# ehsan886/DBA_mod

Hardware: AMD Instinct MI355X
Metric: FL rounds/sec + backdoor ASR & main-task acc, ResNet-18 CIFAR-10 100 clients (higher is better)
Workload: dtype fp32

## Files before the change

csrc/kernels/xaux.hip:

```cpp
#include "common.hpp"
#include "xmfma.hpp"
#include <algorithm>

namespace {

__device__ __forceinline__ void xsplit_w_body(const float* __restrict__ w, long long sstride, long long per,
                                              const int* __restrict__ amax, int ld, uint16_t* __restrict__ out,
                                              int sl, long long e0, long long e1, long long step) {
  const int sb = hexp(amax_read(amax, ld, sl));
  const float mb = __uint_as_float((uint32_t)(sb + 127) << 23);
  const float* __restrict__ src = w + (long long)sl * sstride;
  uint16_t* __restrict__ oh = out + (long long)sl * 2 * per;
  uint16_t* __restrict__ ol = oh + per;
  for (long long e = e0 + threadIdx.x * 4LL; e < e1; e += step) {
    float v[4];
#pragma unroll
    for (int i = 0; i < 4; ++i) v[i] = e + i < per ? src[e + i] : 0.f;
    uint2 sp[2];
    split4h(v[0], v[1], v[2], v[3], mb, sp);
    const uint16_t* h = (const uint16_t*)&sp[0];
    const uint16_t* l = (const uint16_t*)&sp[1];
#pragma unroll
    for (int i = 0; i < 4; ++i)
      if (e + i < per) { oh[e + i] = h[i]; ol[e + i] = l[i]; }
  }
}
__global__ __launch_bounds__(256) void xsplit_w_kernel(const float* __restrict__ w, long long sstride, long long per,
                                                       const int* __restrict__ amax, int ld,
                                                       uint16_t* __restrict__ out) {
  xsplit_w_body(w, sstride, per, amax, ld, out, blockIdx.y, blockIdx.x * 1024LL, per, (long long)gridDim.x * 1024);
}
struct XSDesc {
  long long w, sstride, per, amax, ld, out, boff;
};
constexpr int kXSBatch = 24, kXSChunk = 4096;
struct XSBatch {
  XSDesc d[kXSBatch];
  int n;
};
__global__ __launch_bounds__(256) void xsplit_w_batch_kernel(const XSBatch b) {
  int i = 0;
  while (i + 1 < b.n && (long long)blockIdx.x >= b.d[i + 1].boff) ++i;
  const XSDesc& d = b.d[i];
  const long long e0 = ((long long)blockIdx.x - d.boff) * kXSChunk;
  const long long e1 = e0 + kXSChunk < d.per ? e0 + kXSChunk : d.per;
  xsplit_w_body((const float*)d.w, d.sstride, d.per, (const int*)d.amax, (int)d.ld, (uint16_t*)d.out, blockIdx.y, e0,
                e1, 1024);
}

struct XFDesc {
  long long planes, out, ncol, cs, boff;
};
struct XFBatch {
  XFDesc d[kXSBatch];
  int n;
};
__global__ __launch_bounds__(256) void xfrag_w_kernel(const XFBatch b) {
  int i = 0;
  while (i + 1 < b.n && (long long)blockIdx.x >= b.d[i + 1].boff) ++i;
  const XFDesc& d = b.d[i];
  const int Cs = (int)d.cs, K = 9 * Cs, NK = K / 32;
  const long long per = d.ncol * K;
  const long long idx = ((long long)blockIdx.x - d.boff) * 256 + threadIdx.x;
  if (idx >= per / 4) return;
  const int l = (int)(idx & 63), f = (int)(idx >> 6) & 3, p = f & 1, kk = f >> 1;
  const long long tt = idx >> 8;
  const int t = (int)(tt % NK), nt = (int)(tt / NK), cc = t / 9, tap = t - cc * 9;
  const long long e = (long long)(nt * 32 + (l & 31)) * K + tap * Cs + cc * 32 + (kk * 2 + (l >> 5)) * 8;
  const uint16_t* __restrict__ src = (const uint16_t*)d.planes + ((long long)blockIdx.y * 2 + p) * per;
  uint16_t* __restrict__ dst = (uint16_t*)d.out + (long long)blockIdx.y * 2 * per;
  ((uint4*)dst)[idx] = *(const uint4*)(src + e);
}

constexpr int kAmaxSegs = 64, kAmaxChunk = 4096;
struct AmaxSegs {
  long long off[kAmaxSegs];
  int len[kAmaxSegs];
  int start[kAmaxSegs + 1];
  int n;
};
__global__ __launch_bounds__(256) void amax_segments_kernel(const float* __restrict__ base, long long gstride,
                                                            const AmaxSegs segs, int ld, int* __restrict__ out) {
  const int c = blockIdx.x, g = blockIdx.y;
  int sg = 0;
  while (sg + 1 < segs.n && segs.start[sg + 1] <= c) ++sg;
  const float* __restrict__ p = base + (long long)g * gstride + segs.off[sg];
  const int n = segs.len[sg], e0 = (c - segs.start[sg]) * kAmaxChunk;
  const bool v4 = ((segs.off[sg] | gstride) & 3) == 0 && ((uintptr_t)base & 15) == 0;
  float m = 0.f;
  float4 v[4];
#pragma unroll
  for (int k = 0; k < 4; ++k) {
    const int e = e0 + (k * 256 + threadIdx.x) * 4;
    if (v4 && e + 3 < n) {
      v[k] = *(const float4*)(p + e);
    } else {
      v[k].x = e < n ? p[e] : 0.f;
      v[k].y = e + 1 < n ? p[e + 1] : 0.f;
      v[k].z = e + 2 < n ? p[e + 2] : 0.f;
      v[k].w = e + 3 < n ? p[e + 3] : 0.f;
    }
  }
#pragma unroll
  for (int k = 0; k < 4; ++k) m = fmaxf(m, fmaxf(fmaxf(fabsf(v[k].x), fabsf(v[k].y)), fmaxf(fabsf(v[k].z), fabsf(v[k].w))));
  amax_fold(out + (long long)sg * kAmaxSub * ld, ld, g, m);
}

__global__ __launch_bounds__(256) void amax_kernel(const float* __restrict__ x, long long gstride, long long n_per_g,
                                                   const int* __restrict__ nvalid, long long per_item, int vec,
                                                   int* __restrict__ out, int ld) {
  const int g = blockIdx.y;
  const long long n = nvalid ? (long long)nvalid[g] * per_item : n_per_g;
  const float* __restrict__ p = x + (long long)g * gstride;
  float m = 0.f;
  if (vec) {
    const long long n4 = n >> 2;
    for (long long e = blockIdx.x * 256LL + threadIdx.x; e < n4; e += (long long)gridDim.x * 256) {
      const float4 v = ((const float4*)p)[e];
      m = fmaxf(m, fmaxf(fmaxf(fabsf(v.x), fabsf(v.y)), fmaxf(fabsf(v.z), fabsf(v.w))));
    }
    for (long long e = n4 * 4 + blockIdx.x * 256LL + threadIdx.x; e < n; e += (long long)gridDim.x * 256)
      m = fmaxf(m, fabsf(p[e]));
  } else {
    for (long long e = blockIdx.x * 256LL + threadIdx.x; e < n; e += (long long)gridDim.x * 256) m = fmaxf(m, fabsf(p[e]));
  }
  amax_fold(out, ld, g, m);
}

}

DBA_EXPORT int dba_xsplit_w(const float* w, long long sstride, long long per, int slots, const int* amax, int ld,
                            uint16_t* out, void* stream) {
  const dim3 grid((unsigned)std::max(1LL, std::min(1024LL, (per + 1023) / 1024)), slots);
  hipLaunchKernelGGL(xsplit_w_kernel, grid, dim3(256), 0, (hipStream_t)stream, w, sstride, per, amax, ld, out);
  DBA_LAUNCH_CHECK();
}


DBA_EXPORT int dba_xsplit_w_batch(const void* desc, int n, int slots, void* stream) {
  const XSDesc* ds = (const XSDesc*)desc;
  for (int i0 = 0; i0 < n; i0 += kXSBatch) {
    XSBatch b{};
    b.n = std::min(kXSBatch, n - i0);
    long long nb = 0;
    for (int i = 0; i < b.n; ++i) {
      b.d[i] = ds[i0 + i];
      b.d[i].boff = nb;
      nb += (b.d[i].per + kXSChunk - 1) / kXSChunk;
    }
    hipLaunchKernelGGL(xsplit_w_batch_kernel, dim3((unsigned)nb, slots), dim3(256), 0, (hipStream_t)stream, b);
    const int rc = (int)hipGetLastError();
    if (rc != 0) return rc;
  }
  return 0;
}


DBA_EXPORT int dba_xfrag_w_batch(const void* desc, int n, int slots, void* stream) {
  const XFDesc* ds = (const XFDesc*)desc;
  for (int i0 = 0; i0 < n; i0 += kXSBatch) {
    XFBatch b{};
    b.n = std::min(kXSBatch, n - i0);
    long long nb = 0;
    for (int i = 0; i < b.n; ++i) {
      b.d[i] = ds[i0 + i];
      if (b.d[i].ncol <= 0 || b.d[i].cs <= 0 || b.d[i].ncol % 32 || b.d[i].cs % 32 || ((b.d[i].planes | b.d[i].out) & 15))
        return -105;
      b.d[i].boff = nb;
      nb += b.d[i].ncol * 9 * b.d[i].cs / 1024;
    }
    hipLaunchKernelGGL(xfrag_w_kernel, dim3((unsigned)nb, slots), dim3(256), 0, (hipStream_t)stream, b);
    const int rc = (int)hipGetLastError();
    if (rc != 0) return rc;
  }
  return 0;
}


DBA_EXPORT int dba_amax_segments(const float* base, long long gstride, const long long* segs, int n, int G, int* out,
                                 int ld, void* stream) {
  if (n > kAmaxSegs || n < 1) return -105;
  AmaxSegs a{};
  a.n = n;
  for (int i = 0; i < n; ++i) {
    a.off[i] = segs[2 * i];
    a.len[i] = (int)segs[2 * i + 1];
    a.start[i + 1] = a.start[i] + std::max(1, ceil_div(a.len[i], kAmaxChunk));
  }
  const dim3 grid((unsigned)a.start[n], G);
  hipLaunchKernelGGL(amax_segments_kernel, grid, dim3(256), 0, (hipStream_t)stream, base, gstride, a, ld, out);
  DBA_LAUNCH_CHECK();
}


DBA_EXPORT int dba_amax(const float* x, long long gstride, long long n_per_g, const int* nvalid, long long per_item,
                        int G, int* out, int ld, void* stream) {
  hipStream_t st = (hipStream_t)stream;
  const int vec = aligned16(x) && gstride % 4 == 0;
  const long long per = nvalid ? per_item * (n_per_g / std::max(1LL, per_item)) : n_per_g;
  const dim3 grid((unsigned)std::max(1LL, std::min(256LL, (per + 4095) / 4096)), G);
  hipLaunchKernelGGL(amax_kernel, grid, dim3(256), 0, st, x, gstride, n_per_g, nvalid, per_item, vec, out, ld);
  DBA_LAUNCH_CHECK();
}
```

csrc/kernels/xconv_fwd.hip:

```cpp
#include "xhalo.hpp"

namespace xg {
SplitPolicy& split_policy() {
  static SplitPolicy p;
  return p;
}
int& xstage_mode() {
  static int mode = 1;
  return mode;
}
}

namespace {

template <int W, int IMGS, int BN, int WM, int WN, bool PRE>
__global__ __launch_bounds__(256) void ximg_kernel(const XArgs a) {
  constexpr int P = 2, NT = 256;
  constexpr int PW = W + 2, PI = PW * PW, PP = IMGS * PI;
  constexpr int CC = 32, CH = CC / 8, Q4 = CC / 4;
  constexpr int PATCH = PP * CH;
  constexpr int BM = IMGS * W * W;
  constexpr int TM = BM / WM, TN = BN / WN, MI = TM / 32, NJ = TN / 32;
  static_assert(WM * WN == NT / 64 && MI >= 1 && NJ >= 1 && BM == 128, "tiling");
  constexpr int RPT = NT / 8;
  static_assert(BN % RPT == 0, "weight rows");
  constexpr int RB = BN / RPT, BPL = BN * 4;
  __shared__ __attribute__((aligned(16))) uint4 patch[P * PATCH];
  __shared__ __attribute__((aligned(16))) uint4 bring[2 * P * BPL];

  const int g = blockIdx.y;
  const int tn = blockIdx.x % a.tiles_n, tm = blockIdx.x / a.tiles_n;
  const int img0 = tm * IMGS, n0 = tn * BN;
  const int nv = min(valid_rows(a.nvalid, g, a.N), a.N);
  if (img0 >= nv) return;
  const int slot = a.wsel ? a.wsel[g] : g;
  const int Cs = a.Cs, K = 9 * Cs, NC = Cs / CC, NK = 9 * NC;
  const float* __restrict__ src = a.src + (long long)g * a.src_gstride;
  const int tid = threadIdx.x, lane = tid & 63, wid = tid >> 6;
  const int wm = wid / WN, wn = wid % WN;
  const int kq = tid & 7, r0 = tid >> 3;
  const int fr = lane & 31, hf = lane >> 5;

  constexpr int NE = (PP * Q4 + NT - 1) / NT;
  float4 pv[NE];
  const __amdgpu_buffer_rsrc_t rA = rsrc(src, (long long)a.N * W * W * Cs * 4);
  auto pload = [&](int cc) __attribute__((always_inline)) {
#pragma unroll
    for (int u = 0; u < NE; ++u) {
      const int e = tid + NT * u;
      const int pp = e / Q4, q = e - pp * Q4;
      const int im = pp / PI, rem = pp - im * PI;
      const int h = rem / PW - 1, w = rem % PW - 1, img = img0 + im;
      const bool ok = e < PP * Q4 && img < nv && (unsigned)h < (unsigned)W && (unsigned)w < (unsigned)W;
      pv[u] = bload4(rA, ok ? (((img * W + h) * W + w) * Cs + cc * CC + q * 4) * 4 : kOOB);
    }
  };
  HScale hs;
  auto ppiece = [&](int u, float m) __attribute__((always_inline)) {
    const int e = tid + NT * u;
    if (e >= PP * Q4) return;
    const int pp = e / Q4, q = e - pp * Q4;
    const int prow = (pp % PI) / PW;
    uint2 sp[P];
    split4h(pv[u].x, pv[u].y, pv[u].z, pv[u].w, m, sp);
    const int o = pp * CH + ((q >> 1) ^ (prow & 3));
#pragma unroll
    for (int p = 0; p < P; ++p) ((uint2*)&patch[p * PATCH + o])[q & 1] = sp[p];
  };

  int bn_[RB];
#pragma unroll
  for (int j = 0; j < RB; ++j) {
    const int n = n0 + r0 + RPT * j;
    bn_[j] = n < a.Ncol ? n : -1;
  }
  const uint16_t* Bh = PRE ? a.wp + (long long)slot * a.wp_sstride : nullptr;
  const __amdgpu_buffer_rsrc_t rBh = rsrc(Bh, (long long)a.Ncol * K * 2);
  const __amdgpu_buffer_rsrc_t rBl = rsrc(PRE ? Bh + (a.wp_sstride >> 1) : nullptr, (long long)a.Ncol * K * 2);
  const __amdgpu_buffer_rsrc_t rB = rsrc(a.w + (long long)slot * a.w_sstride, (long long)a.Ncol * K * 4);
  uint4 rb[2][RB];
  auto gq = [&](int t, int st, int j) __attribute__((always_inline)) {
    const bool ok = bn_[j] >= 0 && t < NK;
    const int cc = t / 9, tap = t - cc * 9;
    const int kb = bn_[j] * K + tap * Cs + cc * CC + kq * 4;
    if constexpr (PRE) {
      const uint2 h = bload8(rBh, ok ? kb * 2 : kOOB), l = bload8(rBl, ok ? kb * 2 : kOOB);
      rb[st][j] = make_uint4(h.x, h.y, l.x, l.y);
    } else {
      rb[st][j] = __builtin_bit_cast(uint4, bload4(rB, ok ? kb * 4 : kOOB));
    }
  };
  auto lput_q = [&](int buf, int st, int q) __attribute__((always_inline)) {
    uint2 sp[P];
    if constexpr (PRE) {
      sp[0] = make_uint2(rb[st][q].x, rb[st][q].y);
      sp[1] = make_uint2(rb[st][q].z, rb[st][q].w);
    } else {
      const float4 v = __builtin_bit_cast(float4, rb[st][q]);
      split4h(v.x, v.y, v.z, v.w, hs.mb, sp);
    }
    lds_put<P, false, BN>(bring + buf * P * BPL, BPL, 0, r0 + RPT * q, kq, sp);
  };

  f32x16_t acc[MI][NJ];
#pragma unroll
  for (int i = 0; i < MI; ++i)
#pragma unroll
    for (int j = 0; j < NJ; ++j)
#pragma unroll
      for (int r = 0; r < 16; ++r) acc[i][j][r] = 0.f;

  int apix[MI], arow[MI];
#pragma unroll
  for (int i = 0; i < MI; ++i) {
    const int m = wm * TM + i * 32 + fr;
    const int im = m / (W * W), rem = m - im * (W * W);
    apix[i] = im * PI + (rem / W) * PW + rem % W;
    arow[i] = rem / W;
  }
  auto mma = [&](int t, int buf, int stn) __attribute__((always_inline)) {
    const int tap = t % 9, ti = tap / 3, tj = tap - ti * 3;
    const int toff = ti * PW + tj;
    const uint4* L = bring + buf * P * BPL;
    sfor<2>([&](auto KK) __attribute__((always_inline)) {
      const int ch = decltype(KK)::value * 2 + hf;
      uint4 af[P][MI], bfr[P][NJ];
#pragma unroll
      for (int i = 0; i < MI; ++i) {
        const int pp = apix[i] + toff;
        const int o = pp * CH + (ch ^ ((arow[i] + ti) & 3));
#pragma unroll
        for (int p = 0; p < P; ++p) af[p][i] = patch[p * PATCH + o];
      }
#pragma unroll
      for (int j = 0; j < NJ; ++j) {
        const int n = wn * TN + j * 32 + fr;
        const int o = n * 4 + (ch ^ ((n >> 2) & 3));
#pragma unroll
        for (int p = 0; p < P; ++p) bfr[p][j] = L[p * BPL + o];
      }
      mma_half<MI, NJ, P, true, RB, decltype(KK)::value>(af, bfr, acc, [&](int q) __attribute__((always_inline)) {
        lput_q(buf ^ 1, stn, q);
        gq(t + 3, stn, q);
      });
    });
  };
  auto step = [&](int t, int buf, int stn) __attribute__((always_inline)) {
    const int c = t / 9;
    mma(t, buf, stn);
    __syncthreads();
    if (t - 9 * c == 8 && c + 1 < NC) {
#pragma unroll
      for (int u = 0; u < NE; ++u) ppiece(u, hs.ma);
      if (c + 2 < NC) pload(c + 2);
      __syncthreads();
    }
  };

  hs.init(amax_read(a.amax_src, a.amax_src_ld, g), amax_read(a.amax_w, a.amax_w_ld, slot));
#pragma unroll
  for (int q = 0; q < RB; ++q) {
    gq(0, 0, q);
    gq(1, 1, q);
  }
  pload(0);
#pragma unroll
  for (int u = 0; u < NE; ++u) ppiece(u, hs.ma);
  if (NC > 1) pload(1);
#pragma unroll
  for (int q = 0; q < RB; ++q) {
    lput_q(0, 0, q);
    gq(2, 0, q);
  }
  __syncthreads();
  int t = 0;
  for (; t + 1 < NK; t += 2) {
    step(t, 0, 1);
    step(t + 1, 1, 0);
  }
  if (t < NK) step(t, 0, 1);
  hs.finish(acc);

  float* out = a.out + (long long)g * a.out_gstride;
  const float* bias = a.bias ? a.bias + (long long)slot * a.b_sstride : nullptr;
  const float* res = a.res ? a.res + (long long)g * a.out_gstride : nullptr;
  float vmax = 0.f;
#pragma unroll
  for (int j = 0; j < NJ; ++j) {
    const int n = n0 + wn * TN + j * 32 + fr;
    if (n >= a.Ncol) continue;
    const float bv = bias ? bias[n] : 0.f;
#pragma unroll
    for (int i = 0; i < MI; ++i)
#pragma unroll
      for (int r = 0; r < 16; ++r) {
        const int m = wm * TM + i * 32 + (r & 3) + 8 * (r >> 2) + 4 * hf;
        if (img0 + m / (W * W) >= nv) continue;
        const long long o = (long long)(img0 * W * W + m) * a.Ncol + n;
        float v = acc[i][j][r];
        if (bias) v += bv;
        if (res) v += res[o];
        if (a.relu) v = fmaxf(v, 0.f);
        vmax = fmaxf(vmax, fabsf(v));
        out[o] = v;
      }
  }
  if (a.amax_out) amax_fold(a.amax_out, a.amax_out_ld, g, vmax);
}

template <int W, int IMGS, int BN>
__global__ __launch_bounds__(256) void ximg2_kernel(const XArgs a) {
  constexpr int P = 2, NT = 256;
  constexpr int PW = W + 2, PI = PW * PW, PP = IMGS * PI;
  constexpr int CC = 32, CH = CC / 8, Q4 = CC / 4;
  constexpr int PATCH = PP * CH;
  constexpr int BM = IMGS * W * W;
  constexpr int WN = BN / 32, WM = (NT / 64) / WN, TM = BM / WM, MI = TM / 32;
  static_assert(WM * WN == NT / 64 && MI >= 1 && BM == 128, "tiling");
  extern __shared__ __attribute__((aligned(16))) uint4 ximg2_patch[];

  const int g = blockIdx.y;
  const int tn = blockIdx.x % a.tiles_n, tm = blockIdx.x / a.tiles_n;
  const int img0 = tm * IMGS, n0 = tn * BN;
  const int nv = min(valid_rows(a.nvalid, g, a.N), a.N);
  if (img0 >= nv) return;
  const int slot = a.wsel ? a.wsel[g] : g;
  const int Cs = a.Cs, NC = Cs / CC, NK = 9 * NC;
  const float* __restrict__ src = a.src + (long long)g * a.src_gstride;
  const int tid = threadIdx.x, lane = tid & 63, wid = tid >> 6;
  const int wm = wid / WN, wn = wid % WN;
  const int fr = lane & 31, hf = lane >> 5;

  constexpr int NE = (PP * Q4 + NT - 1) / NT;
  static_assert(NE <= 9, "one patch piece per k-step");
  float4 pv[NE];
  const __amdgpu_buffer_rsrc_t rA = rsrc(src, (long long)a.N * W * W * Cs * 4);
  auto pload1 = [&](int u, int cc) __attribute__((always_inline)) {
    const int e = tid + NT * u;
    const int pp = e / Q4, q = e - pp * Q4;
    const int im = pp / PI, rem = pp - im * PI;
    const int h = rem / PW - 1, w = rem % PW - 1, img = img0 + im;
    const bool ok = e < PP * Q4 && cc < NC && img < nv && (unsigned)h < (unsigned)W && (unsigned)w < (unsigned)W;
    pv[u] = bload4(rA, ok ? (((img * W + h) * W + w) * Cs + cc * CC + q * 4) * 4 : kOOB);
  };
  HScale hs;
  auto ppiece = [&](int u, int buf) __attribute__((always_inline)) {
    const int e = tid + NT * u;
    if (NT * (u + 1) > PP * Q4 && e >= PP * Q4) return;
    const int pp = e / Q4, q = e - pp * Q4;
    const int prow = (pp % PI) / PW;
    uint2 sp[P];
    split4h(pv[u].x, pv[u].y, pv[u].z, pv[u].w, hs.ma, sp);
    const int o = pp * CH + ((q >> 1) ^ (prow & 3));
#pragma unroll
    for (int p = 0; p < P; ++p) ((uint2*)&ximg2_patch[(buf * P + p) * PATCH + o])[q & 1] = sp[p];
  };

  const __amdgpu_buffer_rsrc_t rF = rsrc(a.wf + (long long)slot * a.wf_sstride, (long long)a.Ncol * 9 * Cs * 4);
  const int wbase = ((n0 >> 5) + wn) * NK * 4096 + lane * 16;
  uint4 wb[3][4];
  auto gw = [&](int t, int s, int f) __attribute__((always_inline)) {
    wb[s][f] = __builtin_bit_cast(uint4, bload4(rF, t < NK ? wbase + t * 4096 + f * 1024 : kOOB));
  };

  f32x16_t acc[MI][1];
#pragma unroll
  for (int i = 0; i < MI; ++i)
#pragma unroll
    for (int r = 0; r < 16; ++r) acc[i][0][r] = 0.f;

  int apix[MI], arow[MI];
#pragma unroll
  for (int i = 0; i < MI; ++i) {
    const int m = wm * TM + i * 32 + fr;
    const int im = m / (W * W), rem = m - im * (W * W);
    apix[i] = im * PI + (rem / W) * PW + rem % W;
    arow[i] = rem / W;
  }

  hs.init(amax_read(a.amax_src, a.amax_src_ld, g), amax_read(a.amax_w, a.amax_w_ld, slot));
#pragma unroll
  for (int f = 0; f < 4; ++f) {
    gw(0, 0, f);
    gw(1, 1, f);
  }
#pragma unroll
  for (int u = 0; u < NE; ++u) pload1(u, 0);
#pragma unroll
  for (int u = 0; u < NE; ++u) {
    ppiece(u, 0);
    pload1(u, 1);
  }
  __syncthreads();
  for (int c = 0; c < NC; ++c) {
    const uint4* L = ximg2_patch + (c & 1) * P * PATCH;
    const bool more = c + 1 < NC;
    sfor<9>([&](auto TAP) __attribute__((always_inline)) {
      constexpr int tap = decltype(TAP)::value, ti = tap / 3, tj = tap - ti * 3;
      constexpr int toff = ti * PW + tj, s = tap % 3, s2 = (tap + 2) % 3;
      constexpr int u = tap - (9 - NE);
      constexpr int NQ = u >= 0 ? 5 : 4;
      const int t = c * 9 + tap;
      __builtin_amdgcn_sched_barrier(0x786);
      sfor<2>([&](auto KK) __attribute__((always_inline)) {
        constexpr int kk = decltype(KK)::value;
        const int ch = kk * 2 + hf;
        uint4 af[P][MI], bfr[P][1];
#pragma unroll
        for (int i = 0; i < MI; ++i) {
          const int o = (apix[i] + toff) * CH + (ch ^ ((arow[i] + ti) & 3));
#pragma unroll
          for (int p = 0; p < P; ++p) af[p][i] = L[p * PATCH + o];
        }
#pragma unroll
        for (int p = 0; p < P; ++p) bfr[p][0] = wb[s][kk * 2 + p];
        mma_half<MI, 1, P, true, NQ, kk>(af, bfr, acc, [&](int q) __attribute__((always_inline)) {
          if (q < 4) {
            gw(t + 2, s2, q);
          } else if constexpr (u >= 0) {
            if (more) ppiece(u, (c + 1) & 1);
            pload1(u, c + 2);
          }
        });
      });
    });
    __syncthreads();
  }
  hs.finish(acc);

  float* out = a.out + (long long)g * a.out_gstride;
  const float* bias = a.bias ? a.bias + (long long)slot * a.b_sstride : nullptr;
  const float* res = a.res ? a.res + (long long)g * a.out_gstride : nullptr;
  float vmax = 0.f;
  const int n = n0 + wn * 32 + fr;
  if (n < a.Ncol) {
    const float bv = bias ? bias[n] : 0.f;
#pragma unroll
    for (int i = 0; i < MI; ++i)
#pragma unroll
      for (int r = 0; r < 16; ++r) {
        const int m = wm * TM + i * 32 + (r & 3) + 8 * (r >> 2) + 4 * hf;
        if (img0 + m / (W * W) >= nv) continue;
        const long long o = (long long)(img0 * W * W + m) * a.Ncol + n;
        float v = acc[i][0][r];
        if (bias) v += bv;
        if (res) v += res[o];
        if (a.relu) v = fmaxf(v, 0.f);
        vmax = fmaxf(vmax, fabsf(v));
        out[o] = v;
      }
  }
  if (a.amax_out) amax_fold(a.amax_out, a.amax_out_ld, g, vmax);
}

template <int W, int IMGS, int BN, int WM, int WN>
int ximg_go(const XArgs& a, int G, hipStream_t st) {
  XArgs b = a;
  b.tiles_n = ceil_div(a.Ncol, BN);
  const dim3 grid((unsigned)(ceil_div(a.N, IMGS) * b.tiles_n), G, 1);
  if (a.wp) hipLaunchKernelGGL((ximg_kernel<W, IMGS, BN, WM, WN, true>), grid, dim3(256), 0, st, b);
  else hipLaunchKernelGGL((ximg_kernel<W, IMGS, BN, WM, WN, false>), grid, dim3(256), 0, st, b);
  DBA_LAUNCH_CHECK();
}
template <int W, int IMGS, int BN>
int ximg2_go(const XArgs& a, int G, hipStream_t st) {
  constexpr int PATCH = IMGS * (W + 2) * (W + 2) * 4;
  constexpr int LDS = 2 * 2 * PATCH * (int)sizeof(uint4);
  static unsigned long long attr_set = 0ull;
  int dev = 0;
  if (hipGetDevice(&dev) != hipSuccess || dev < 0 || dev >= 64) return -100;
  if (!(attr_set >> dev & 1ull)) {
    if (hipFuncSetAttribute((const void*)ximg2_kernel<W, IMGS, BN>, hipFuncAttributeMaxDynamicSharedMemorySize,
                            LDS) != hipSuccess)
      return -100;
    attr_set |= 1ull << dev;
  }
  XArgs b = a;
  b.tiles_n = ceil_div(a.Ncol, BN);
  const dim3 grid((unsigned)(ceil_div(a.N, IMGS) * b.tiles_n), G, 1);
  hipLaunchKernelGGL((ximg2_kernel<W, IMGS, BN>), grid, dim3(256), LDS, st, b);
  DBA_LAUNCH_CHECK();
}
__global__ __launch_bounds__(256) void xstage16_kernel(const XArgs a) {
  constexpr int P = 2, W = 16, CS = 64, BM = 128, BN = 64, WN = 2;
  constexpr int TR = BM / W, PW = W + 2, PR = TR + 2, PP = PR * PW;
  constexpr int CH = CS / 8, PATCH = PP * CH;
  constexpr int TM = 64, TN = 32, MI = TM / 32;
  constexpr int CB = CS / 32;
  constexpr int STG = (BN / 32) * CB * 4 * 64;
  static_assert(BM * BN <= P * PATCH * 4, "epilogue tile fits the patch");
  __shared__ __attribute__((aligned(16))) uint4 lds[P * PATCH + 2 * STG];
  __shared__ long long orow[BM];
  uint4* const patch = lds;
  uint4* const bring = lds + P * PATCH;

  const int g = blockIdx.y;
  const int HT = a.Ho / TR;
  const int tm = blockIdx.x;
  const int img = tm / HT, h0 = (tm - img * HT) * TR;
  if (img >= valid_rows(a.nvalid, g, a.N)) return;
  const int slot = a.wsel ? a.wsel[g] : g;
  const float* __restrict__ src = a.src + (long long)g * a.src_gstride;
  const int tid = threadIdx.x, lane = tid & 63, wid = tid >> 6;
  const int wm = wid / WN, wn = wid % WN;
  const int fr = lane & 31, hf = lane >> 5;

  const uint16_t* F = a.wf + (long long)slot * a.wf_sstride + ((wid >> 1) * (CB * 9) + (wid & 1) * 9) * 2048 + lane * 8;
  auto fill = [&](int tap) __attribute__((always_inline)) {
    const uint32_t dst = __builtin_amdgcn_readfirstlane(
        (uint32_t)(uintptr_t)(__attribute__((address_space(3))) void*)(bring + (tap & 1) * STG + wid * 256));
#pragma unroll
    for (int f = 0; f < 4; ++f) {
      uint32_t keep;
      asm volatile("s_mov_b32 %0, m0\n\ts_mov_b32 m0, %2\n\ts_nop 0\n\tglobal_load_lds_dwordx4 %1, off\n\ts_mov_b32 m0, %0"
                   : "=&s"(keep)
                   : "v"(F + tap * 2048 + f * 512), "s"(dst + f * 1024)
                   : "memory");
    }
  };
  auto gl_sync = [&]() __attribute__((always_inline)) {
    asm volatile("s_waitcnt vmcnt(0)" ::: "memory");
    __syncthreads();
  };
  fill(0);

  if (tid < BM)
    orow[tid] = (((long long)img * a.Ho + h0 + tid / W) * a.Wo + tid % W) * a.Ncol;

  constexpr int Q4 = CS / 4;
  constexpr int NE = (PP * Q4 + 255) / 256;
  float4 pv[NE];
  {
    const __amdgpu_buffer_rsrc_t rA = rsrc(src, (long long)a.N * a.Hs * a.Ws * CS * 4);
#pragma unroll
    for (int u = 0; u < NE; ++u) {
      const int e = tid + 256 * u;
      const int pp = e / Q4, q = e - pp * Q4;
      const int pr = pp / PW, pc = pp - pr * PW;
      const int h = h0 - 1 + pr, w = pc - 1;
      const bool ok = e < PP * Q4 && (unsigned)h < (unsigned)a.Hs && (unsigned)w < (unsigned)a.Ws;
      pv[u] = bload4(rA, ok ? (((img * a.Hs + h) * a.Ws + w) * CS + q * 4) * 4 : kOOB);
    }
  }
  HScale hs;
  hs.init(amax_read(a.amax_src, a.amax_src_ld, g), amax_read(a.amax_w, a.amax_w_ld, slot));
#pragma unroll
  for (int u = 0; u < NE; ++u) {
    const int e = tid + 256 * u;
    if (e >= PP * Q4) break;
    const int pp = e / Q4, q = e - pp * Q4;
    uint2 sp[P];
    split4h(pv[u].x, pv[u].y, pv[u].z, pv[u].w, hs.ma, sp);
    const int o = pp * CH + ((q >> 1) ^ hswz<W, CS>(pp, pp % PW));
#pragma unroll
    for (int p = 0; p < P; ++p) ((uint2*)&patch[p * PATCH + o])[q & 1] = sp[p];
  }

  f32x16_t acc[MI][1];
#pragma unroll
  for (int i = 0; i < MI; ++i)
#pragma unroll
    for (int r = 0; r < 16; ++r) acc[i][0][r] = 0.f;
  int apix[MI], acol[MI];
#pragma unroll
  for (int i = 0; i < MI; ++i) {
    const int m = wm * TM + i * 32 + fr;
    apix[i] = (m / W) * PW + (m % W);
    acol[i] = m % W;
  }

  auto stage = [&](int tap) __attribute__((always_inline)) {
    const int ti = tap / 3, tj = tap - ti * 3;
    const int toff = ti * PW + tj;
    const uint4* L = bring + (tap & 1) * STG + wn * (CB * 4 * 64) + lane;
    uint4 af[2][P][MI], bfr[2][P][1];
    auto frags = [&](auto Hc) __attribute__((always_inline)) {
      constexpr int h = decltype(Hc)::value, cb = h / 2, kk = h % 2, st = h & 1;
      const int ch = kk * 2 + hf;
#pragma unroll
      for (int i = 0; i < MI; ++i) {
        const int pp = apix[i] + toff;
        const int o = pp * CH + ((cb * 4 + ch) ^ hswz<W, CS>(pp, acol[i] + tj));
#pragma unroll
        for (int p = 0; p < P; ++p) af[st][p][i] = patch[p * PATCH + o];
      }
#pragma unroll
      for (int p = 0; p < P; ++p) bfr[st][p][0] = L[(cb * 4 + kk * 2 + p) * 64];
    };
    frags(std::integral_constant<int, 0>{});
    sfor<2 * CB>([&](auto Hc) __attribute__((always_inline)) {
      constexpr int h = decltype(Hc)::value;
      if constexpr (h + 1 < 2 * CB) frags(std::integral_constant<int, h + 1>{});
      __builtin_amdgcn_sched_barrier(0);
      mma_half<MI, 1, P, true, 0, h % 2>(af[h & 1], bfr[h & 1], acc, [](int) {});
      __builtin_amdgcn_sched_barrier(0);
    });
  };

  gl_sync();
  for (int tap = 0; tap < 9; ++tap) {
    if (tap + 1 < 9) fill(tap + 1);
    stage(tap);
    gl_sync();
  }
  hs.finish(acc);

  float* Ct = reinterpret_cast<float*>(patch);
#pragma unroll
  for (int i = 0; i < MI; ++i)
#pragma unroll
    for (int r = 0; r < 16; ++r)
      Ct[(wm * TM + i * 32 + (r & 3) + 8 * (r >> 2) + 4 * hf) * BN + wn * TN + fr] = acc[i][0][r];
  __syncthreads();
  float* out = a.out + (long long)g * a.out_gstride;
  const float* bias = a.bias ? a.bias + (long long)slot * a.b_sstride : nullptr;
  const float* res = a.res ? a.res + (long long)g * a.out_gstride : nullptr;
  constexpr int C4 = BN / 4;
  float vmax = 0.f;
  for (int e = tid; e < BM * C4; e += 256) {
    const int row = e / C4, n = (e - row * C4) * 4;
    const long long o = orow[row];
    float4 v = *(const float4*)&Ct[row * BN + n];
    if (bias) { v.x += bias[n]; v.y += bias[n + 1]; v.z += bias[n + 2]; v.w += bias[n + 3]; }
    if (res) {
      const float4 rv = *(const float4*)(res + o + n);
      v.x += rv.x; v.y += rv.y; v.z += rv.z; v.w += rv.w;
    }
    if (a.relu) { v.x = fmaxf(v.x, 0.f); v.y = fmaxf(v.y, 0.f); v.z = fmaxf(v.z, 0.f); v.w = fmaxf(v.w, 0.f); }
    vmax = fmaxf(vmax, fmaxf(fmaxf(fabsf(v.x), fabsf(v.y)), fmaxf(fabsf(v.z), fabsf(v.w))));
    *(float4*)(out + o + n) = v;
  }
  if (a.amax_out) amax_fold(a.amax_out, a.amax_out_ld, g, vmax);
}

constexpr bool kXStage16Default = true;

int xstage16_try(const XArgs& a, int G, int KH, int KW, hipStream_t st) {
  const XClass& c = a.cls[0];
  const int mode = xg::xstage_mode();
  if (!(mode == 3 || (mode == 1 && kXStage16Default))) return -100;
  if (KH != 3 || KW != 3 || a.sp != 1 || a.os != 1 || a.dsg != 1 || a.splitk != 1 || c.nI != 3 || c.nJ != 3 ||
      c.bh != -1 || c.bw != -1)
    return -100;
  if (a.Hs != 16 || a.Ws != 16 || a.Ho != 16 || a.Wo != 16 || a.Cs != 64 || a.Ncol != 64) return -100;
  if (a.bf.mode || a.lz_coef || a.sc_src) return -100;
  if (!aligned16(a.src) || !aligned16(a.w) || a.src_gstride % 4 || a.w_sstride % 4) return -100;
  if (!a.wp || !a.wf || ((uintptr_t)a.wf & 15) || a.wf_sstride % 8 || a.wf_sstride < 2 * 64 * 576) return -100;
  hipLaunchKernelGGL(xstage16_kernel, dim3((unsigned)(a.N * (a.Ho / 8)), G, 1), dim3(256), 0, st, a);
  DBA_LAUNCH_CHECK();
}

int& ximg_on() {
  static int on = 1;
  return on;
}
int ximg_try(const XArgs& a, int G, int KH, int KW, hipStream_t st) {
  const XClass& c = a.cls[0];
  if (!ximg_on() || KH != 3 || KW != 3 || a.sp != 1 || a.os != 1 || a.dsg != 1 || a.splitk != 1 || c.nI != 3 ||
      c.nJ != 3 || c.bh != -1 || c.bw != -1)
    return -100;
  if (a.Hs != a.Ho || a.Ws != a.Wo || a.Ho != a.Wo || a.Cs % 32 != 0 || a.Ncol % 32 != 0) return -100;
  if (a.bf.mode || a.lz_coef) return -100;
  if (!aligned16(a.src) || a.src_gstride % 4 || !aligned16(a.w) || a.w_sstride % 4) return -100;
  if (a.wp && (((uintptr_t)a.wp & 15) || a.wp_sstride % 8)) return -100;
  if (a.sc_src) return -100;
  if (ximg_on() == 1 && a.wp && a.wf && !((uintptr_t)a.wf & 15) && a.wf_sstride % 8 == 0) {
    int rc = -100;
    if (a.Wo == 8) rc = a.Ncol >= 128 ? ximg2_go<8, 2, 128>(a, G, st) : ximg2_go<8, 2, 64>(a, G, st);
    if (a.Wo == 4) rc = a.Ncol >= 128 ? ximg2_go<4, 8, 128>(a, G, st) : ximg2_go<4, 8, 64>(a, G, st);
    if (rc != -100) return rc;
  }
  if (a.Wo == 8) return a.Ncol >= 128 ? ximg_go<8, 2, 128, 2, 2>(a, G, st) : ximg_go<8, 2, 64, 2, 2>(a, G, st);
  if (a.Wo == 4) return a.Ncol >= 128 ? ximg_go<4, 8, 128, 2, 2>(a, G, st) : ximg_go<4, 8, 64, 2, 2>(a, G, st);
  return -100;
}

}

DBA_EXPORT int dba_xsplit_policy(int target, int min_k, int max_s, int kslab_max, int dgrad_ks) {
  SplitPolicy& p = split_policy();
  if (dgrad_ks >= 0) p.dgrad_ks = dgrad_ks;
  if (target > 0) p.target = target;
  if (min_k > 0) p.min_k = min_k;
  if (max_s > 0) p.max_s = std::min(max_s, kSkMax);
  if (kslab_max > 0) p.kslab_max = kslab_max;
  return 0;
}

DBA_EXPORT int dba_ximg_set(int on) {
  const int prev = ximg_on();
  if (on >= 0) ximg_on() = on;
  return prev;
}

DBA_EXPORT int dba_xstage_set(int on) {
  const int prev = xg::xstage_mode();
  if (on >= 1 && on <= 3) xg::xstage_mode() = on;
  return prev;
}


DBA_EXPORT long long dba_xconv_ws_floats(int G, int N, int Ho, int Wo, int Cin, int Cout, int KH, int KW) {
  const long long M = (long long)N * Ho * Wo;
  const int s = xsplitk(M, G, Cout, KH * KW * Cin);
  return s > 1 ? (long long)s * G * M * Cout : 0;
}


DBA_EXPORT long long dba_xconv_sk_ints(int G, int N, int Ho, int Wo, int Cin, int Cout, int KH, int KW) {
  const long long M = (long long)N * Ho * Wo;
  const int s = xsplitk(M, G, Cout, KH * KW * Cin);
  const long long n = s > 1 ? xconv_sk_count(M, Cout, G, 1, s) : 0;
  return (n > 0 && sk_ok((const int*)1, n, M, Cout, G, 1, s)) ? n : 0;
}


DBA_EXPORT int dba_xconv_fwd(const float* x, long long x_gstride, const float* w, long long w_sstride,
                             const int* wsel, const float* bias, long long b_sstride, const float* res, float* out,
                             long long out_gstride, const int* nvalid, int G, int N, int H, int W, int Cin, int Ho,
                             int Wo, int Cout, int KH, int KW, int stride, int pad, int relu, const int* amax_x,
                             int amax_x_ld, const int* amax_w, int amax_w_ld, int* amax_out, int amax_out_ld,
                             const uint16_t* wp, long long wp_sstride, const uint16_t* wf, long long wf_sstride,
                             float* ws, long long ws_floats, int* sk_cnt,
                             long long sk_cnt_n, const void* bnf, const float* lz_coef, int lz_relu,
                             void* stream) {
  hipStream_t st = (hipStream_t)stream;
  if ((long long)N * H * W * Cin >= (1LL << 29)) return -103;
  const long long M = (long long)N * Ho * Wo;
  const int K = KH * KW * Cin;
  const int vec = (Cin % 4 == 0 && aligned16(x) && aligned16(w) && x_gstride % 4 == 0 && w_sstride % 4 == 0) ? 4 : 1;
  XArgs a{};
  a.src = x; a.src_gstride = x_gstride; a.w = w; a.w_sstride = w_sstride; a.wsel = wsel;
  a.bias = bias; a.b_sstride = b_sstride; a.res = res; a.out = out; a.out_gstride = out_gstride;
  a.nvalid = nvalid; a.N = N; a.Hs = H; a.Ws = W; a.Cs = Cin; a.Ncol = Cout; a.Ho = Ho; a.Wo = Wo;
  a.sp = stride; a.os = 1; a.dsg = 1; a.relu = relu; a.splitk = 1;
  a.amax_src = amax_x; a.amax_w = amax_w; a.amax_out = amax_out;
  a.amax_src_ld = amax_x_ld; a.amax_w_ld = amax_w_ld; a.amax_out_ld = amax_out_ld;
  a.wp = wp; a.wp_sstride = wp_sstride; a.wf = wf; a.wf_sstride = wf_sstride;
  a.cls[0] = XClass{KH, KW, -pad, -pad, 0, 0, Ho, Wo, 0};
  if (!amax_x || !amax_w) return -109;
  if (bnf) {
    a.bf = *(const BnFuse*)bnf;
    if (a.bf.mode != 1 || bias || res || relu || (Cout & 3) || a.bf.C != Cout) return -108;
  }
  if (lz_coef) {
    if (wp || vec < 4 || Cin > 512) return -108;
    a.lz_coef = lz_coef; a.lz_relu = lz_relu;
  }
  auto fin = [&](int rc) { return (rc == 0 && a.bf.mode) ? bnx_finalize_go(a.bf, nvalid, G, N, Ho * Wo, st) : rc; };
  if (stride == 1) {
    int rc = ximg_try(a, G, KH, KW, st);
    if (rc == -100) rc = xstage16_try(a, G, KH, KW, st);
    if (rc == -100) rc = xhalo_try(a, G, KH, KW, st);
    if (rc != -100) return fin(rc);
  }
  const int s = xsplitk(M, G, Cout, K);
  const bool ws_ok = s > 1 && ws != nullptr && ws_floats >= (long long)s * G * M * Cout;
  if (s > 1 && !(ws_ok && sk_ok(sk_cnt, sk_cnt_n, M, Cout, G, 1, s))) {
    XArgs b = a;
    b.kslab = s;
    const int rc = xconv_ks(b, M, G, vec, st);
    if (rc != -100) return fin(rc);
  }
  if (ws_ok && sk_ok(sk_cnt, sk_cnt_n, M, Cout, G, 1, s)) {
    XArgs b = a;
    b.splitk = s;
    b.zstride = (long long)G * M * Cout;
    b.sk_ws = ws; b.sk_gstride = M * Cout; b.sk_cnt = sk_cnt;
    return fin(xconv_dispatch(b, M, G, 1, vec, st));
  }
  if (ws_ok) {
    XArgs b = a;
    b.splitk = s;
    b.out = ws;
    b.out_gstride = M * Cout;
    b.zstride = (long long)G * M * Cout;
    const int rc = xconv_dispatch(b, M, G, 1, vec, st);
    if (rc != 0) return rc;
    if (a.bf.mode)
      return bnx_tile_go(a.bf, nullptr, out, out_gstride, nvalid, G, N, Ho * Wo, nullptr, 0.f, ws, s, b.zstride,
                         nullptr, st);
    const long long per = M * Cout;
    const dim3 grid((unsigned)std::max(1LL, std::min(1024LL, (per + 255) / 256)), G);
    hipLaunchKernelGGL(xsplitk_reduce_kernel, grid, dim3(256), 0, st, (const float*)ws, s, b.zstride, per, nvalid, N,
                       Ho * Wo, Cout, bias, b_sstride, wsel, res, relu, out, amax_out, amax_out_ld);
    DBA_LAUNCH_CHECK();
  }
  return fin(xconv_dispatch(a, M, G, 1, vec, st));
}


DBA_EXPORT int dba_xdown_fwd(const float* a_, long long a_gstride, const float* w2, long long w2_sstride,
                             const uint16_t* w2p, long long w2p_sstride, const int* wsel, const float* b2,
                             long long b_sstride, const float* x2, long long x2_gstride, const uint16_t* wscp,
                             long long wscp_sstride, const float* bsc, long long bsc_sstride, float* out,
                             long long out_gstride, const int* nvalid, int G, int N, int Ho, int Wo, int C, int H2,
                             int W2, int C2, const int* amax_a, int amax_a_ld, const int* amax_w2, int amax_w2_ld,
                             const int* amax_x2, int amax_x2_ld, const int* amax_wsc, int amax_wsc_ld, int* amax_out,
                             int amax_out_ld, void* stream) {
  if (!amax_a || !amax_w2 || !amax_x2 || !amax_wsc || !w2p || !wscp) return -109;
  if ((H2 - 1) / 2 + 1 != Ho || (W2 - 1) / 2 + 1 != Wo || (long long)N * H2 * W2 * C2 >= (1LL << 29) ||
      (long long)N * Ho * Wo * C >= (1LL << 29))
    return -103;
  XArgs a{};
  a.src = a_; a.src_gstride = a_gstride; a.w = w2; a.w_sstride = w2_sstride; a.wsel = wsel;
  a.bias = b2; a.b_sstride = b_sstride; a.res = nullptr; a.out = out; a.out_gstride = out_gstride;
  a.nvalid = nvalid; a.N = N; a.Hs = Ho; a.Ws = Wo; a.Cs = C; a.Ncol = C; a.Ho = Ho; a.Wo = Wo;
  a.sp = 1; a.os = 1; a.dsg = 1; a.relu = 1; a.splitk = 1;
  a.amax_src = amax_a; a.amax_w = amax_w2; a.amax_out = amax_out;
  a.amax_src_ld = amax_a_ld; a.amax_w_ld = amax_w2_ld; a.amax_out_ld = amax_out_ld;
  a.wp = w2p; a.wp_sstride = w2p_sstride;
  a.sc_src = x2; a.sc_gstride = x2_gstride; a.sc_H = H2; a.sc_W = W2; a.sc_C = C2;
  a.sc_wp = wscp; a.sc_wp_sstride = wscp_sstride;
  a.sc_amax_src = amax_x2; a.sc_amax_src_ld = amax_x2_ld; a.sc_amax_w = amax_wsc; a.sc_amax_w_ld = amax_wsc_ld;
  a.sc_bias = bsc; a.sc_b_sstride = bsc_sstride;
  a.cls[0] = XClass{3, 3, -1, -1, 0, 0, Ho, Wo, 0};
  return xhalo_try(a, G, 3, 3, (hipStream_t)stream);
}
```

dba_mod_amd/models/program.py:

```python
from __future__ import annotations

from typing import Callable, Dict, List, Optional, Tuple

import torch

from .. import ops
from ..ops import bnstate as bs
from .mirror import CIFAR_RESNETS
from .spec import ModelSpec

Tensor = torch.Tensor
BN_EPS = 1e-5
BN_MOMENTUM = 0.1


class Tape:

    def __init__(self) -> None:
        self.nodes: List[Tuple[Tuple[Tensor, ...], Tuple[Optional[Tensor], ...], Callable]] = []
        self._produced: set = set()
        self._grads: Optional[Dict[int, Tensor]] = None
        self._uses: Dict[int, int] = {}
        self.nvalid: Optional[Tensor] = None
        self.on_begin: Optional[Callable[[], None]] = None
        self.on_end: Optional[Callable[[], None]] = None

    def record(self, outputs: Tuple[Tensor, ...], inputs: Tuple[Optional[Tensor], ...], bwd: Callable) -> None:
        self.nodes.append((outputs, inputs, bwd))
        for o in outputs:
            self._produced.add(id(o))
        for i in inputs:
            if i is not None:
                self._uses[id(i)] = self._uses.get(id(i), 0) + 1

    def is_last(self, t) -> bool:
        return self._uses.get(id(t), 0) == 1

    @staticmethod
    def finish_spec(t) -> Optional[bs.Finish]:
        if isinstance(t, bs.LazyBN):
            return bs.Finish(ya=t.y, sa=t.stat, lazy=t.relu)
        return getattr(t, "_dba_finish", None)

    def needs_grad(self, t: Optional[Tensor]) -> bool:
        return t is not None and id(t) in self._produced

    def pop_grad(self, t: Tensor) -> Optional[Tensor]:
        return self._grads.pop(id(t), None) if self._grads is not None else None

    def backward(self, out: Tensor, grad: Tensor) -> None:
        if self.on_begin is not None:
            self.on_begin()
        grads: Dict[int, Tensor] = {id(out): grad}
        self._grads = grads
        for outputs, inputs, bwd in reversed(self.nodes):
            gouts = [grads.pop(id(o), None) for o in outputs]
            if all(g is None for g in gouts):
                for i in inputs:
                    if i is not None:
                        self._uses[id(i)] -= 1
                continue
            gouts = [ops.bn_finish(g, self.finish_spec(o), self.nvalid)
                     if isinstance(g, Tensor) and self.finish_spec(o) is not None else g
                     for o, g in zip(outputs, gouts)]
            gins = bwd(*gouts)
            for inp, gi in zip(inputs, gins):
                if inp is not None:
                    self._uses[id(inp)] -= 1
                if gi is None or inp is None or not self.needs_grad(inp):
                    continue
                k = id(inp)
                if k in grads:
                    if not (isinstance(grads[k], Tensor) and isinstance(gi, Tensor)):
                        raise RuntimeError("a finished BN gradient cannot take further contributions")
                    grads[k] = grads[k] + gi
                else:
                    grads[k] = gi
        self.nodes.clear()
        self._produced.clear()
        self._uses.clear()
        self._grads = None
        if self.on_end is not None:
            self.on_end()


class Ctx:

    def __init__(self, spec: ModelSpec, state: Tensor, wcomp: Tensor, wsel: Optional[Tensor],
                 train: bool, grads: Optional[Tensor] = None, nvalid: Optional[Tensor] = None,
                 folded: Optional[Dict[str, Tuple[Tensor, Tensor]]] = None,
                 dropout_seed: Optional[Tensor] = None,
                 act_dtype: torch.dtype = torch.float32) -> None:
        self.spec, self.state, self.wcomp, self.wsel = spec, state, wcomp, wsel
        self.train, self.grads, self.nvalid, self.folded = train, grads, nvalid, folded
        self.tape = Tape() if train else None
        self._dgrad_items: List[tuple] = []
        self._wt: Dict[int, Tensor] = {}
        self._wdefer: List[tuple] = []
        if self.tape is not None:
            self.tape.on_begin = self._prepare_dgrad
            self.tape.on_end = self._end_backward
            self.tape.nvalid = nvalid
        self.dropout_seed = dropout_seed
        self._drop_ctr = 0
        self.head: Optional[dict] = None
        self.head_out: Optional[Tuple[Tensor, Tensor]] = None
        self.act_dtype = act_dtype
        self._wamax = self._weight_scales() if train else None

    def _weight_scales(self) -> Optional[Dict[str, Tensor]]:
        wc = self.wcomp
        if wc is None or not wc.is_cuda or wc.dtype != torch.float32 or ops.backend_name(wc.device) != "hip":
            return None
        names = [e.name for e in self.spec.params if e.kind in ("conv_w", "lin_w")]
        slots = ops.hip_module().weight_amax(wc, [(self.spec.by_name[n].offset, self.spec.by_name[n].numel)
                                                  for n in names])
        return dict(zip(names, slots))

    def _want_dgrad(self, w: Tensor, stride: int, pad: int, in_hw: Tuple[int, int], G: int) -> int:
        self._dgrad_items.append((w, self.wsel, stride, pad, in_hw, self.nvalid, G))
        return len(self._dgrad_items) - 1

    def _end_backward(self) -> None:
        if self._wdefer:
            ops.backend_for(self.state).wgrad_flush(self._wdefer)

    def _prepare_dgrad(self) -> None:
        if self._dgrad_items:
            self._wt = ops.prepare_dgrad_weights(self._dgrad_items[0][0], self._dgrad_items)
        self._dgrad_items = []

    def w(self, name: str) -> Tensor:
        v = self.spec.view(self.wcomp, name)
        if self._wamax is not None and name in self._wamax:
            v._dba_amax = self._wamax[name]
        return v

    def m(self, name: str) -> Tensor:
        return self.spec.view(self.state, name)

    def g(self, name: str) -> Tensor:
        assert self.grads is not None
        return self.spec.view(self.grads, name)

    def conv_bn(self, x: Tensor, conv: str, bn: str, stride: int, pad: int, relu: bool,
                residual: Optional[Tensor] = None) -> Tensor:
        if self.train:
            raise RuntimeError("conv_bn is the evaluation form; training uses bn_conv / bn_out")
        wf, bf = self.folded[conv]
        return ops.conv2d(x, wf, self.wsel, stride, pad, bias=bf, residual=residual, relu=relu, nvalid=self.nvalid)

    def basic_block(self, x: Tensor, pre: str) -> Tensor:
        w1, b1 = self.folded[pre + "conv1.weight"]
        w2, b2 = self.folded[pre + "conv2.weight"]
        if ops.basic_block_ok(x, w1, w2):
            return ops.basic_block_eval(x, w1, b1, w2, b2, self.wsel, self.nvalid)
        a = ops.conv2d(x, w1, self.wsel, 1, 1, bias=b1, relu=True, nvalid=self.nvalid)
        return ops.conv2d(a, w2, self.wsel, 1, 1, bias=b2, residual=x, relu=True, nvalid=self.nvalid)

    def down_block(self, a: Tensor, x: Tensor, pre: str, sc: str) -> Tensor:
        w2, b2 = self.folded[pre + "conv2.weight"]
        wsc, bsc = self.folded[sc + ".0.weight"]
        if ops.down_block_ok(a, w2, x, wsc):
            return ops.down_block_eval(a, w2, b2, x, wsc, bsc, self.wsel, self.nvalid)
        r = ops.conv2d(x, wsc, self.wsel, 2, 0, bias=bsc, nvalid=self.nvalid)
        return ops.conv2d(a, w2, self.wsel, 1, 1, bias=b2, residual=r, relu=True, nvalid=self.nvalid)

    def stem_block(self, x: Tensor, stem: str, pre: str) -> Optional[Tensor]:
        w0, b0 = self.folded[stem]
        w1, b1 = self.folded[pre + "conv1.weight"]
        w2, b2 = self.folded[pre + "conv2.weight"]
        if not ops.stem_block_ok(x, w0, w1, w2):
            return None
        return ops.stem_block_eval(x, w0, b0, w1, b1, w2, b2, self.wsel, self.nvalid)

    def _bnp(self, bn: str) -> bs.BnParams:
        return bs.BnParams(self.m(bn + ".weight"), self.m(bn + ".bias"), self.m(bn + ".running_mean"),
                           self.m(bn + ".running_var"), self.g(bn + ".weight"), self.g(bn + ".bias"),
                           BN_MOMENTUM, BN_EPS)

    def bn_conv(self, x, conv: str, bn: str, stride: int, pad: int, relu: bool):
        if not self.train:
            return self.conv_bn(x, conv, bn, stride, pad, relu)
        w = self.w(conv)
        y, st = ops.conv_bn_stats(x, w, self.wsel, stride, pad, self.nvalid, self._bnp(bn), relu)
        a = bs.LazyBN(y, st, relu)
        self.tape.record((a,), (x,), self._bn_conv_bwd(x, w, y, st, conv, stride, pad))
        return a

    def _bn_conv_bwd(self, x, w, y, st, conv: str, stride: int, pad: int):
        in_hw = (x.shape[2], x.shape[3])
        kh, kw = w.shape[2], w.shape[3]
        need_dx = self.tape.needs_grad(x)
        k = self._want_dgrad(w, stride, pad, in_hw, x.shape[0]) if need_dx else -1

        def bwd(ga: bs.Fin):
            dy = ops.conv2d_wgrad(bs.LazyGrad(ga.for_stat(st).d, y, st), x, stride, pad, kh, kw, self.g(conv),
                                  nvalid=self.nvalid, defer=self._wdefer)
            if not need_dx:
                return (None,)
            if dy is None:
                raise RuntimeError(f"{conv}: the weight gradient did not store dy for the data gradient")
            acc = self.tape.pop_grad(x)
            fin = self.tape.finish_spec(x) if self.tape.is_last(x) else None
            return (ops.conv2d_dgrad(dy, w, self.wsel, stride, pad, in_hw, nvalid=self.nvalid, accum=acc,
                                     wt=self._wt.get(k), finish=fin),)
        return bwd

    def bn_out(self, a, residual=None, relu: bool = True) -> Tensor:
        out = ops.bn_apply(a, residual, relu, self.nvalid)
        branch = isinstance(residual, bs.LazyBN) and not residual.relu
        out._dba_finish = bs.Finish(ya=a.y, sa=a.stat, mask_out=out if relu else None,
                                    yb=residual.y if branch else None, sb=residual.stat if branch else None)

        def bwd(gout: bs.Fin):
            gr = None
            if branch:
                gr = gout.for_stat(residual.stat)
            elif residual is not None:
                gr = gout.d
            return gout.for_stat(a.stat), gr

        self.tape.record((out,), (a, residual), bwd)
        return out

    def conv(self, x: Tensor, name: str, stride: int, pad: int, bias: Optional[str], relu: bool) -> Tensor:
        if not self.train and self.folded is not None and name in self.folded:
            w, b = self.folded[name]
        else:
            w, b = self.w(name), (self.m(bias) if bias is not None else None)
        y = ops.conv2d(x, w, self.wsel, stride, pad, bias=b, relu=relu, nvalid=self.nvalid)
        if not self.train:
            return y
        in_hw = (x.shape[2], x.shape[3])
        kh, kw = w.shape[2], w.shape[3]
        need_dx = self.tape.needs_grad(x)
        k = self._want_dgrad(w, stride, pad, in_hw, x.shape[0]) if need_dx else -1

        def bwd(dout: Tensor):
            d = ops.relu_mask_bwd(dout, y) if relu else dout
            ops.conv2d_wgrad(d, x, stride, pad, kh, kw, self.g(name), self.g(bias) if bias is not None else None,
                             nvalid=self.nvalid, defer=self._wdefer)
            return (ops.conv2d_dgrad(d, w, self.wsel, stride, pad, in_hw, nvalid=self.nvalid, wt=self._wt.get(k))
                    if need_dx else None,)

        self.tape.record((y,), (x,), bwd)
        return y

    def linear(self, x: Tensor, name: str, bias: str, relu: bool, final: bool = False) -> Tensor:
        G, N, Fd = x.shape
        x4 = self.reshape(x, (G, N, 1, 1, Fd))
        y4 = self._lin_conv(x4, name, bias, relu, torch.float32 if final else None)
        return self.reshape(y4, (G, N, y4.shape[-1]))

    def _lin_conv(self, x4: Tensor, name: str, bias: str, relu: bool,
                  out_dtype: Optional[torch.dtype] = None) -> Tensor:
        if not self.train and self.folded is not None and name in self.folded:
            w, b = self.folded[name]
        else:
            wv = self.w(name)
            w = wv.reshape(wv.shape[0], wv.shape[1], 1, 1, wv.shape[2])
            if hasattr(wv, "_dba_amax"):
                w._dba_amax = wv._dba_amax
            b = self.m(bias)
        y = ops.conv2d(x4, w, self.wsel, 1, 0, bias=b, relu=relu, nvalid=self.nvalid, out_dtype=out_dtype)
        if not self.train:
            return y
        need_dx = self.tape.needs_grad(x4)
        gv = self.g(name)
        k = self._want_dgrad(w, 1, 0, (1, 1), x4.shape[0]) if need_dx else -1

        def bwd(dout: Tensor):
            d = ops.relu_mask_bwd(dout, y) if relu else dout
            ops.conv2d_wgrad(d, x4, 1, 0, 1, 1, gv.reshape(gv.shape[0], gv.shape[1], 1, 1, gv.shape[2]),
                             self.g(bias), nvalid=self.nvalid, defer=self._wdefer)
            return (ops.conv2d_dgrad(d, w, self.wsel, 1, 0, (1, 1), nvalid=self.nvalid, wt=self._wt.get(k))
                    if need_dx else None,)

        self.tape.record((y,), (x4,), bwd)
        return y

    def reshape(self, x: Tensor, shape: Tuple[int, ...]) -> Tensor:
        y = x.reshape(shape)
        if self.train and y is not x:
            in_shape = x.shape
            self.tape.record((y,), (x,), lambda d: (d.reshape(in_shape),))
        return y

    def maxpool(self, x: Tensor, k: int, s: int, p: int) -> Tensor:
        if not self.train:
            return ops.maxpool2d(x, k, s, p, want_ind=False)[0]
        y, ind = ops.maxpool2d(x, k, s, p)
        if self.train:
            shp = tuple(x.shape)
            self.tape.record((y,), (x,), lambda d: (ops.maxpool2d_bwd(d, ind, shp, k, s, p),))
        return y

    def gap(self, x: Tensor) -> Tensor:
        y = ops.avgpool_global(x)
        if self.train:
            hw = (x.shape[2], x.shape[3])

            def bwd(d):
                fin = self.tape.finish_spec(x) if self.tape.is_last(x) else None
                if fin is not None:
                    return (ops.bn_finish(None, fin, self.nvalid, pool=d, hw=hw),)
                return (ops.avgpool_global_bwd(d, hw),)

            self.tape.record((y,), (x,), bwd)
        return y

    def head_ok(self, x, wname: str) -> bool:
        if not (self.train and self.head is not None and isinstance(x, Tensor) and x.is_cuda):
            return False
        be = ops.backend_for(x)
        return hasattr(be, "head_ok") and be.head_ok(x, self.w(wname))

    def fused_head(self, x: Tensor, wname: str, bname: str) -> Tensor:
        be = ops.backend_for(x)
        h = self.head
        hw = (x.shape[2], x.shape[3])
        loss, correct, dpool = be.head_train(x, self.w(wname), self.m(bname), h["labels"], self.nvalid,
                                             self.g(wname), self.g(bname), h.get("stats"), h.get("slot"))
        self.head_out = (loss, correct)

        def bwd(_seed):
            fin = self.tape.finish_spec(x) if self.tape.is_last(x) else None
            if fin is not None:
                return (ops.bn_finish(None, fin, self.nvalid, pool=dpool, hw=hw),)
            return (ops.avgpool_global_bwd(dpool, hw),)

        self.tape.record((loss,), (x,), bwd)
        return loss

    def dropout(self, x: Tensor, p: float) -> Tensor:
        if not self.train:
            return x
        seeds, salt = self.dropout_seed, self._drop_ctr
        self._drop_ctr += 1
        y = ops.dropout(x, p, seeds, salt)
        self.tape.record((y,), (x,), lambda d: (ops.dropout_bwd(d, p, seeds, salt),))
        return y


def _block_out(ctx: Ctx, a, conv: str, bn: str, pad: int, residual):
    if not ctx.train:
        return ctx.conv_bn(a, conv, bn, 1, pad, relu=True, residual=residual)
    return ctx.bn_out(ctx.bn_conv(a, conv, bn, 1, pad, relu=False), residual, relu=True)


def _resnet_cifar(ctx: Ctx, x: Tensor) -> Tensor:
    bottleneck, blocks = CIFAR_RESNETS[ctx.spec.arch]
    exp = 4 if bottleneck else 1
    out = None if (ctx.train or bottleneck) else ctx.stem_block(x, "conv1.weight", "layer1.0.")
    done = 0 if out is None else 1
    if out is None:
        out = ctx.bn_conv(x, "conv1.weight", "bn1", 1, 1, relu=True)
    cin = 32
    for li, w in enumerate((32, 64, 128, 256)):
        for bi in range(done if li == 0 else 0, blocks[li]):
            stride = 2 if (li > 0 and bi == 0) else 1
            pre = f"layer{li + 1}.{bi}."
            if not ctx.train and not bottleneck and stride == 1 and cin == w:
                out = ctx.basic_block(out, pre)
                cin = w
                continue
            if bottleneck:
                a = ctx.bn_conv(out, pre + "conv1.weight", pre + "bn1", 1, 0, relu=True)
                a = ctx.bn_conv(a, pre + "conv2.weight", pre + "bn2", stride, 1, relu=True)
                last, p = "3", 0
            else:
                a = ctx.bn_conv(out, pre + "conv1.weight", pre + "bn1", stride, 1, relu=True)
                last, p = "2", 1
                if not ctx.train and stride == 2 and cin != w:
                    out, cin = ctx.down_block(a, out, pre, pre + "shortcut"), w
                    continue
            if stride != 1 or cin != w * exp:
                sc = ctx.bn_conv(out, pre + "shortcut.0.weight", pre + "shortcut.1", stride, 0, relu=False)
            else:
                sc = out
            out = _block_out(ctx, a, pre + f"conv{last}.weight", pre + f"bn{last}", p, sc)
            cin = w * exp
    if ctx.head_ok(out, "linear.weight"):
        return ctx.fused_head(out, "linear.weight", "linear.bias")
    out = ctx.gap(out)
    G, N = out.shape[:2]
    return ctx.linear(ctx.reshape(out, (G, N, out.shape[-1])), "linear.weight", "linear.bias", relu=False, final=True)


def _resnet_tiny(ctx: Ctx, x: Tensor) -> Tensor:
    if ctx.train:
        out = ctx.bn_out(ctx.bn_conv(x, "conv1.weight", "bn1", 2, 3, relu=False), None, relu=True)
    else:
        out = ctx.conv_bn(x, "conv1.weight", "bn1", 2, 3, relu=True)
    out = ctx.maxpool(out, 3, 2, 1)
    cin = 64
    for li, w in enumerate((64, 128, 256, 512)):
        for bi in range(2):
            stride = 2 if (li > 0 and bi == 0) else 1
            pre = f"layer{li + 1}.{bi}."
            if not ctx.train and stride == 2 and cin != w:
                a = ctx.bn_conv(out, pre + "conv1.weight", pre + "bn1", stride, 1, relu=True)
                out, cin = ctx.down_block(a, out, pre, pre + "downsample"), w
                continue
            if stride != 1 or cin != w:
                sc = ctx.bn_conv(out, pre + "downsample.0.weight", pre + "downsample.1", stride, 0, relu=False)
            else:
                sc = out
            a = ctx.bn_conv(out, pre + "conv1.weight", pre + "bn1", stride, 1, relu=True)
            out = _block_out(ctx, a, pre + "conv2.weight", pre + "bn2", 1, sc)
            cin = w
    out = ctx.gap(out)
    G, N = out.shape[:2]
    return ctx.linear(ctx.reshape(out, (G, N, out.shape[-1])), "fc.weight", "fc.bias", relu=False, final=True)


def _mnist(ctx: Ctx, x: Tensor) -> Tensor:
    a = ctx.conv(x, "conv1.weight", 1, 0, "conv1.bias", relu=True)
    a = ctx.maxpool(a, 2, 2, 0)
    b = ctx.conv(a, "conv2.weight", 1, 0, "conv2.bias", relu=True)
    b = ctx.maxpool(b, 2, 2, 0)
    G, N = b.shape[:2]
    f = ctx.reshape(b, (G, N, -1))
    h = ctx.linear(f, "fc1.weight", "fc1.bias", relu=True)
    return ctx.linear(h, "fc2.weight", "fc2.bias", relu=False, final=True)


def _loan(ctx: Ctx, x: Tensor) -> Tensor:
    h = ctx.linear(x, "layer1.0.weight", "layer1.0.bias", relu=True)
    h = ctx.dropout(h, 0.5)
    h = ctx.linear(h, "layer2.0.weight", "layer2.0.bias", relu=True)
    h = ctx.dropout(h, 0.5)
    return ctx.linear(h, "layer3.0.weight", "layer3.0.bias", relu=False, final=True)


FORWARDS: Dict[str, Callable[[Ctx, Tensor], Tensor]] = {
    "resnet18_tiny": _resnet_tiny, "mnist": _mnist, "loan": _loan,
    **{arch: _resnet_cifar for arch in CIFAR_RESNETS},
}


def forward(ctx: Ctx, x: Tensor) -> Tensor:
    return FORWARDS[ctx.spec.arch](ctx, x)


def _conv_bn_pairs(spec: ModelSpec) -> List[Tuple[str, str]]:
    pairs = []
    for e in spec.params:
        if e.kind != "conv_w":
            continue
        n = e.name
        if n.endswith("shortcut.0.weight"):
            pairs.append((n, n.replace("shortcut.0.weight", "shortcut.1")))
        elif n.endswith("downsample.0.weight"):
            pairs.append((n, n.replace("downsample.0.weight", "downsample.1")))
        else:
            bn = n.replace("conv", "bn").replace(".weight", "")
            if bn + ".weight" in spec.by_name:
                pairs.append((n, bn))
    return pairs


def fold_bank(spec: ModelSpec, state: Tensor, dtype: torch.dtype) -> Dict[str, Tuple[Tensor, Tensor]]:
    out: Dict[str, Tuple[Tensor, Tensor]] = {}
    pairs = list(_conv_bn_pairs(spec))
    slots = (ops.hip_module().amax_slots(len(pairs), state.shape[0], state.device)
             if state.is_cuda and ops.backend_name(state.device) == "hip" and dtype == torch.float32 else None)
    H = ops.hip_module() if slots is not None else None
    if H is not None and (ops.bn_fold is H.bn_fold or getattr(ops.bn_fold, "__module__", "") == ops.__name__):
        folded = H.bn_fold_batch([(spec.view(state, conv), spec.view(state, bn + ".weight"),
                                   spec.view(state, bn + ".bias"), spec.view(state, bn + ".running_mean"),
                                   spec.view(state, bn + ".running_var"), slots[i])
                                  for i, (conv, bn) in enumerate(pairs)], BN_EPS)
        for (conv, _), wb in zip(pairs, folded):
            out[conv] = wb
        H.split_weights_batch([(wf, wf[0].numel(), wf[0].numel(), wf._dba_amax) for wf, _ in folded])
    else:
        for conv, bn in pairs:
            out[conv] = ops.bn_fold(spec.view(state, conv), None, spec.view(state, bn + ".weight"),
                                    spec.view(state, bn + ".bias"), spec.view(state, bn + ".running_mean"),
                                    spec.view(state, bn + ".running_var"), BN_EPS, dtype)
    for e in spec.params:
        if e.name in out or e.kind not in ("conv_w", "lin_w"):
            continue
        bias = e.name.replace(".weight", ".bias")
        w = spec.view(state, e.name)
        if w.dim() == 3:
            w = w.reshape(w.shape[0], w.shape[1], 1, 1, w.shape[2])
        b = spec.view(state, bias) if bias in spec.by_name else None
        out[e.name] = (w.to(dtype), b)
    return out
```

dba_mod_amd/ops/__init__.py:

```python
from __future__ import annotations

import contextlib
import os
from typing import Any

import torch

from . import reference as _ref

_FORCE_REF = os.environ.get("DBA_OPS", "").lower() == "reference"
_hip_mod = None


def hip_module():
    global _hip_mod
    if _hip_mod is None:
        from . import hip as _h
        _hip_mod = _h
    return _hip_mod


def backend_for(t: torch.Tensor):
    if t.is_cuda and not _FORCE_REF:
        return hip_module()
    return _ref


def backend_name(device: torch.device) -> str:
    return "hip" if (device.type == "cuda" and not _FORCE_REF) else "reference"


def _dispatch(name: str):
    def fn(*args: Any, **kw: Any):
        first = next(a for a in list(args) + list(kw.values()) if isinstance(a, torch.Tensor))
        return getattr(backend_for(first), name)(*args, **kw)
    fn.__name__ = name
    fn.__doc__ = getattr(_ref, name).__doc__
    return fn


_OPS = ["gather_images", "gather_rows", "conv2d", "conv2d_dgrad", "conv2d_wgrad", "relu_mask_bwd", "bn_fold", "maxpool2d", "maxpool2d_bwd", "avgpool_global",
        "avgpool_global_bwd", "dropout", "dropout_bwd", "softmax_xent", "sgd_step", "dist_loss_grad",
        "scale_from_base", "add_noise_scaled", "delta_sum", "sq_dists", "weighted_sum", "weighted_sum_fixed", "delta_stats", "clipped_delta_sum_fixed",
        "clipped_delta_sum", "pairwise_sq_dists", "trimmed_delta_sum", "delta_sum_votes",
        "vote_agreement", "rlr_apply", "gram", "prepare_dgrad_weights", "wgrad_flush",
        "wgrad_prepare", "conv_bn_stats", "bn_apply", "bn_finish", "basic_block_ok", "basic_block_eval",
        "stem_block_ok", "stem_block_eval", "down_block_ok", "down_block_eval"]

for _n in _OPS:
    globals()[_n] = _dispatch(_n)


def amax_arena(G: int, device: torch.device, counters: int = 0):
    if backend_name(device) == "hip":
        return hip_module().amax_arena(G, device, counters=counters)
    return contextlib.nullcontext()


__all__ = list(_OPS) + ["backend_for", "backend_name", "hip_module", "amax_arena"]

from . import library
```

dba_mod_amd/ops/branches.py:

```python
from __future__ import annotations

import torch

TIE_TOL = 1e-4


class BranchReplay:

    def __init__(self, nval, tol: float = TIE_TOL):
        self.nval, self.rec, self.replay, self.i = nval, [], False, 0
        self.tol = tol
        self.flips = self.hard = self.elements = 0

    def start_replay(self) -> None:
        self.replay, self.i = True, 0
        self.flips = self.hard = self.elements = 0

    def wrap(self, mod):
        o_conv, o_mp = mod.conv2d, mod.maxpool2d
        o_cbs, o_apply = mod.conv_bn_stats, mod.bn_apply

        def conv_bn_stats(x, w, wsel, stride, pad, nvalid, p, relu):
            y, st = o_cbs(x, w, wsel, stride, pad, nvalid, p, relu)
            if relu:
                C = y.shape[-1]
                sh = (y.shape[0],) + (1,) * (y.dim() - 2) + (C,)
                pre = (y.double() * st.coef[:, 2].reshape(sh).double() + st.coef[:, 3].reshape(sh).double())
                if not self.replay:
                    self.rec.append((pre > 0).cpu())
                else:
                    st.relu_mask = self._decide(pre.to(y.dtype) if y.dtype == torch.float64 else pre)
            return y, st

        def bn_apply(a, residual, relu, nvalid=None):
            if not (relu and self.replay):
                out = o_apply(a, residual, relu, nvalid)
                return self._record(out) if relu else out
            return self._relu(o_apply(a, residual, False, nvalid))

        def conv2d(*a, **k):
            relu = k.get("relu", a[7] if len(a) > 7 else False)
            if not (relu and self.replay):
                y = o_conv(*a, **k)
                return self._record(y) if relu else y
            if len(a) > 7:
                a = a[:7] + (False,) + a[8:]
            else:
                k = dict(k, relu=False)
            return self._relu(o_conv(*a, **k))

        def maxpool2d(x, kk, st, p, want_ind=True):
            y, ind = o_mp(x, kk, st, p)
            y, ind = self._pool(x, y, ind)
            return y, (ind if want_ind else None)

        def basic_block_ok(x, w1, w2):
            return False
        return {"conv2d": conv2d, "maxpool2d": maxpool2d, "conv_bn_stats": conv_bn_stats, "bn_apply": bn_apply,
                "basic_block_ok": basic_block_ok, "stem_block_ok": lambda x, w0, w1, w2: False,
                "down_block_ok": lambda a, w2, x2, wsc: False}

    def _valid(self, t):
        v = torch.zeros(t.shape[:2], dtype=torch.bool)
        for g in range(t.shape[0]):
            v[g, :int(self.nval[g])] = True
        return v.view(*t.shape[:2], *([1] * (t.dim() - 2))).to(t.device)

    def _rms(self, t):
        keep = self._valid(t).expand_as(t)
        sq = torch.where(keep, t.double() ** 2, torch.zeros((), dtype=torch.float64, device=t.device))
        n = keep.reshape(t.shape[0], -1).sum(1).clamp(min=1)
        r = (sq.reshape(t.shape[0], -1).sum(1) / n).sqrt()
        return r.view(-1, *([1] * (t.dim() - 1))).to(t.dtype)

    def _record(self, out):
        self.rec.append((out > 0).cpu())
        return out

    def _decide(self, pre):
        m = self.rec[self.i].to(pre.device)
        self.i += 1
        keep = self._valid(pre).expand_as(pre)
        pos = pre > 0
        tie = pre.abs() <= self.tol * self._rms(pre)
        differ = keep & (m != pos)
        take = differ & tie
        self.flips += int(take.sum())
        self.hard += int((differ & ~tie).sum())
        self.elements += int(keep.sum())
        return torch.where(take, m, pos)

    def _relu(self, pre):
        m = self.rec[self.i].to(pre.device)
        self.i += 1
        keep = self._valid(pre).expand_as(pre)
        pos = pre > 0
        tie = pre.abs() <= self.tol * self._rms(pre)
        differ = keep & (m != pos)
        take = differ & tie
        self.flips += int(take.sum())
        self.hard += int((differ & ~tie).sum())
        self.elements += int(keep.sum())
        out = torch.where(pos, pre, torch.zeros_like(pre))
        out = torch.where(take & m, torch.full_like(pre, 1e-300 if pre.dtype == torch.float64 else 1e-30), out)
        return torch.where(take & ~m, torch.zeros_like(pre), out)

    def _pool(self, x, y, ind):
        if not self.replay:
            self.rec.append(ind.cpu())
            return y, ind
        rec = self.rec[self.i].to(ind.device).to(ind.dtype)
        self.i += 1
        G, N, Hh, Ww, C = x.shape
        xf = x.reshape(G, N, Hh * Ww, C)
        y_rec = xf.gather(2, rec.reshape(G, N, -1, C).long()).reshape(y.shape)
        keep = self._valid(ind).expand_as(ind)
        differ = keep & (rec != ind)
        tie = y_rec >= y - self.tol * self._rms(x).reshape(G, 1, 1, 1, 1)
        take = differ & tie
        self.flips += int(take.sum())
        self.hard += int((differ & ~tie).sum())
        self.elements += int(keep.sum())
        hind = torch.where(take, rec, ind)
        yy = xf.gather(2, hind.reshape(G, N, -1, C).long()).reshape(y.shape)
        return yy.to(y.dtype), hind
```

dba_mod_amd/ops/build.py:

```python
from __future__ import annotations

import glob
import os
import subprocess
import sys
import time
from concurrent.futures import ThreadPoolExecutor
from typing import List

ROOT = os.path.dirname(os.path.dirname(os.path.dirname(os.path.abspath(__file__))))
LIBDIR = os.path.join(ROOT, "dba_mod_amd", "_lib")
CSRC = os.path.join(ROOT, "csrc")
ARCH = os.environ.get("DBA_OFFLOAD_ARCH", "gfx950")


def kernels_path() -> str:
    return os.environ.get("DBA_KERNELS_LIB") or os.path.join(LIBDIR, "libdba_kernels.so")


def runtime_path() -> str:
    return os.path.join(LIBDIR, "libdba_runtime.so")


def _srcs(sub: str, ext: str) -> List[str]:
    return sorted(glob.glob(os.path.join(CSRC, sub, f"*{ext}")))


def _newest(paths: List[str]) -> float:
    return max([os.path.getmtime(p) for p in paths] or [0.0])


def runtime_stale() -> bool:
    p = runtime_path()
    return (not os.path.exists(p)) or _newest(_srcs("runtime", ".cpp")) > os.path.getmtime(p)


def kernels_stale() -> bool:
    p = kernels_path()
    deps = _srcs("kernels", ".hip") + _srcs("kernels", ".hpp")
    return (not os.path.exists(p)) or _newest(deps) > os.path.getmtime(p)


def _run(cmd: List[str]) -> None:
    r = subprocess.run(cmd, stdout=subprocess.PIPE, stderr=subprocess.STDOUT, text=True)
    if r.returncode != 0:
        raise RuntimeError(f"build failed: {' '.join(cmd)}\n{r.stdout}")


def build_runtime(verbose: bool = False) -> str:
    os.makedirs(LIBDIR, exist_ok=True)
    out = runtime_path()
    tmp = out + f".tmp{os.getpid()}"
    _run(["g++", "-O3", "-std=c++17", "-shared", "-fPIC", "-o", tmp] + _srcs("runtime", ".cpp"))
    os.replace(tmp, out)
    if verbose:
        print(f"built {out}")
    return out


_EXTRA = {n: ["-fno-slp-vectorize"] for n in ("xconv_fwd.hip", "xconv_dgrad.hip", "xwgrad.hip", "xaux.hip", "xbn.hip")}
_THIS_MTIME = os.path.getmtime(os.path.abspath(__file__))


def build_kernels(verbose: bool = False, jobs: int = 8) -> str:
    os.makedirs(LIBDIR, exist_ok=True)
    objdir = os.path.join(LIBDIR, "obj")
    os.makedirs(objdir, exist_ok=True)
    hipcc = os.environ.get("HIPCC", "/opt/rocm/bin/hipcc")
    srcs = _srcs("kernels", ".hip")
    hdr_time = _newest(_srcs("kernels", ".hpp"))
    flags = ["-O3", "-std=c++17", "-fPIC", f"--offload-arch={ARCH}", "-munsafe-fp-atomics",
             "-I", os.path.join(CSRC, "kernels")]

    def one(src: str) -> str:
        obj = os.path.join(objdir, os.path.basename(src) + ".o")
        if os.path.exists(obj) and os.path.getmtime(obj) >= max(os.path.getmtime(src), hdr_time, _THIS_MTIME):
            return obj
        t0 = time.time()
        _run([hipcc] + flags + _EXTRA.get(os.path.basename(src), []) + ["-c", src, "-o", obj + ".tmp"])
        os.replace(obj + ".tmp", obj)
        if verbose:
            print(f"  {os.path.basename(src)}: {time.time() - t0:.1f}s")
        return obj

    with ThreadPoolExecutor(max_workers=max(1, min(jobs, len(srcs)))) as ex:
        objs = list(ex.map(one, srcs))
    out = kernels_path()
    tmp = out + f".tmp{os.getpid()}"
    _run([hipcc, "-shared", "-fPIC", f"--offload-arch={ARCH}", "-o", tmp] + objs)
    os.replace(tmp, out)
    if verbose:
        print(f"built {out}")
    return out


def build_all(verbose: bool = True) -> None:
    build_runtime(verbose)
    build_kernels(verbose)


if __name__ == "__main__":
    build_all(verbose=True)
    sys.exit(0)
```

dba_mod_amd/ops/hip.py:

```python
from __future__ import annotations

import contextlib
import ctypes
import os
from typing import Optional, Sequence, Tuple

import torch

from . import bnstate as bs
from . import build
from . import reference as _ref

Tensor = torch.Tensor
_F32 = torch.float32

if not os.path.exists(build.kernels_path()):
    raise ImportError(f"HIP kernel library missing: {build.kernels_path()} — run "
                      f"`python -m dba_mod_amd.ops.build` (or __graft_entry__.build())")
_L = ctypes.CDLL(build.kernels_path())

_P = ctypes.c_void_p
_I = ctypes.c_int
_LL = ctypes.c_longlong
_F = ctypes.c_float
_U = ctypes.c_uint
_D = ctypes.c_double

_SIGS = {
    "dba_gather_images": [_P, _P, _P, _P, _P, _P, _I, _P, _P, _I, _P, _I, _I, _I, _I, _I, _P],
    "dba_gather_rows": [_P, _P, _P, _P, _P, _I, _P, _P, _I, _P, _I, _P, _I, _I, _I, _P],
    "dba_xcolsum": [_P, _LL, _I, _P, _I, _I, _I, _P, _LL, _P, _P],
    "dba_xcolsum_part_doubles": [_I, _I, _I, _I],
    "dba_amax_segments": [_P, _LL, _P, _I, _I, _P, _I, _P],
    "dba_bn_fold": [_P, _LL, _P, _P, _P, _P, _P, _LL, _F, _P, _P, _I, _I, _I, _I, _P, _I, _P],
    "dba_relu_mask_bwd": [_P, _P, _P, _LL, _I, _P],
    "dba_maxpool": [_P, _P, _P, _LL, _I, _I, _I, _I, _I, _I, _I, _I, _I, _P],
    "dba_maxpool_bwd": [_P, _P, _P, _LL, _I, _I, _I, _I, _I, _I, _I, _I, _I, _P],
    "dba_avgpool": [_P, _P, _LL, _I, _I, _I, _P],
    "dba_avgpool_bwd": [_P, _P, _LL, _I, _I, _I, _P],
    "dba_dropout": [_P, _P, _I, _P, _U, _F, _LL, _I, _P],
    "dba_softmax_xent": [_P, _P, _I, _I, _I, _I, _P, _P, _P, _P, _LL, _P, _I, _P, _I, _P, _P, _P],
    "dba_softmax_xent_part_doubles": [_I, _I],
    "dba_xent_r5_set": [_I],
    "dba_head_train": [_P, _LL, _I, _I, _I, _I, _P, _LL, _P, _LL, _I, _P, _P, _P, _P, _P, _P, _LL, _P, _LL, _P, _P,
                       _P, _P, _LL, _P, _I, _I, _P],
    "dba_head_part_doubles": [_I, _I],
    "dba_sgd_step": [_P, _LL, _P, _P, _P, _P, _P, _F, _F, _P, _I, _I, _P],
    "dba_scale_from_base": [_P, _P, _F, _P, _LL, _P],
    "dba_add_noise_scaled": [_P, _P, _LL, _F, _F, _U, _I, _I, _P],
    "dba_delta_sum": [_P, _LL, _I, _P, _LL, _P, _P],
    "dba_sqdist_blocks": [_LL],
    "dba_gram_chunks": [_I],
    "dba_sq_dists": [_P, _LL, _P, _I, _LL, _P, _P, _P],
    "dba_weighted_sum": [_P, _LL, _P, _I, _P, _LL, _I, _P],
    "dba_weighted_sum_fixed": [_P, _LL, _P, _I, _P, _LL, _D, _P],
    "dba_gram": [_P, _LL, _I, _I, _P, _P, _P],
    "dba_delta_stats_blocks": [_LL],
    "dba_delta_stats": [_P, _LL, _I, _P, _LL, _P, _P, _P, _P, _P],
    "dba_clipped_delta_sum_fixed": [_P, _LL, _I, _P, _P, _P, _LL, _D, _P],
    "dba_clipped_delta_sum": [_P, _LL, _I, _P, _P, _P, _LL, _P],
    "dba_pairwise_sqdist_blocks": [_LL],
    "dba_pairwise_sqdist": [_P, _LL, _P, _I, _LL, _P, _P, _P],
    "dba_coord_trim_blocks": [_LL],
    "dba_coord_trim": [_P, _LL, _P, _I, _P, _I, _LL, _P, _P, _P, _P],
    "dba_vote_agreement_blocks": [_LL],
    "dba_rlr_apply_blocks": [_LL],
    "dba_delta_sum_votes": [_P, _LL, _I, _P, _LL, _P, _P, _P],
    "dba_vote_agreement": [_P, _LL, _I, _P, _P, _I, _LL, _P, _P, _P],
    "dba_rlr_apply": [_P, _P, _P, _I, _LL, _F, _F, _U, _I, _P, _P, _P],
    "dba_dist_loss_grad": [_P, _LL, _P, _LL, _P, _LL, _I, _P, _P, _F, _P, _P, _P],
    "dba_ximg_set": [_I],
    "dba_xwgrad_halo_set": [_I],
    "dba_xconv_ws_floats": [_I] * 8,
    "dba_xconv_fwd": [_P, _LL, _P, _LL, _P, _P, _LL, _P, _P, _LL, _P] + [_I] * 13 + [_P, _I] * 3 + [_P, _LL] * 3
    + [_P, _LL, _P, _P, _I, _P],
    "dba_xconv_sk_ints": [_I] * 8,
    "dba_xconv_dgrad": [_P, _LL, _P, _LL, _P, _P, _P, _LL, _P] + [_I] * 12 + [_P, _I] * 2 + [_P, _LL] * 3 + [_P, _P],
    "dba_xsplit_w": [_P, _LL, _LL, _I, _P, _I, _P, _P],
    "dba_amax": [_P, _LL, _LL, _P, _LL, _I, _P, _I, _P],
    "dba_xtranspose": [_P, _I, _I, _LL, _P, _P],
    "dba_xwgrad_ws_floats": [_I] * 8 + [_P],
    "dba_xwgrad_stem_ws_floats": [_I] * 6,
    "dba_xsplit_policy": [_I] * 5,
    "dba_xsplit_w_batch": [_P, _I, _I, _P],
    "dba_xfrag_w_batch": [_P, _I, _I, _P],
    "dba_bn_fold_batch": [_P, _I, _I, _F, _P],
    "dba_xwgrad": [_P, _LL, _P, _LL, _P, _LL, _P] + [_I] * 12 + [_P, _I] * 2 + [_P, _LL, _I] + [_P, _I, _P],
    "dba_bnx_rows": [_P, _P, _P, _LL, _P, _I, _I, _I, _P, _F, _P],
    "dba_bnx_apply": [_P, _P, _P, _P, _P, _I, _I, _P, _LL, _P, _I, _I, _I, _I, _P, _I, _P],
    "dba_bnfuse_size": [],
    "dba_xwgrad_stem": [_P, _LL, _P, _P, _P, _LL, _P, _P, _I, _I, _I, _I, _P],
    "dba_bnx_dy": [_P, _P, _P, _P, _LL, _P, _I, _I, _I, _I, _P, _I, _P],
    "dba_xwgrad_reduce_batch": [_P, _I, _I, _LL, _P],
    "dba_xstage_set": [_I],
    "dba_xblock_fwd": [_P, _LL, _P, _LL, _P, _P, _P, _LL, _P, _P, _LL, _P, _P, _LL, _P] + [_I] * 6
    + [_P, _I, _P, _P, _I, _P, _I, _P],
    "dba_xblock_stem_fwd": [_P, _LL, _P, _LL, _P, _P, _LL, _P, _LL, _P, _P, _LL, _P, _P, _LL, _P, _P, _LL, _P]
    + [_I] * 6 + [_P, _P, _P, _I, _P, _I, _P],
    "dba_mlp_train": [_P, _I, _I, _I, _I, _I, _P, _LL, _P, _P, _I, _P, _I, _I, _I, _I, _P, _P, _P, _P, _I, _I,
                      _P, _LL, _I, _P, _F, _F, _P, _P],
    "dba_xdown_fwd": [_P, _LL, _P, _LL, _P, _LL, _P, _P, _LL, _P, _LL, _P, _LL, _P, _LL, _P, _LL, _P] + [_I] * 8
    + [_P, _I] * 5 + [_P],
    "dba_xstem_fwd": [_P, _LL, _P, _LL, _P, _P, _LL, _P, _P, _LL, _P] + [_I] * 13 + [_P, _I, _P, _P],
}
for _name, _args in _SIGS.items():
    _fn = getattr(_L, _name)
    _fn.argtypes = _args
    _fn.restype = ctypes.c_int
_L.dba_xconv_ws_floats.restype = ctypes.c_longlong
_L.dba_xconv_sk_ints.restype = ctypes.c_longlong
_L.dba_xwgrad_ws_floats.restype = ctypes.c_longlong
_L.dba_xwgrad_stem_ws_floats.restype = ctypes.c_longlong
_L.dba_xcolsum_part_doubles.restype = ctypes.c_longlong
_L.dba_softmax_xent_part_doubles.restype = ctypes.c_longlong
_L.dba_head_part_doubles.restype = ctypes.c_longlong


class _BnFuse(ctypes.Structure):
    _fields_ = [("mode", _I), ("C", _I), ("ngrp", _I),
                ("rec0", _P),
                ("coef_a", _P), ("gamma_a", _P), ("beta_a", _P), ("rm_a", _P), ("rv_a", _P),
                ("p_gstride", _LL), ("momentum", _F), ("eps", _F), ("relu", _I),
                ("amax_a", _P), ("amax_ld", _I),
                ("ya", _P), ("yb", _P), ("y_gstride", _LL),
                ("coef_b", _P), ("gamma_b", _P), ("amax_b", _P),
                ("dgamma_a", _P), ("dbeta_a", _P), ("dgamma_b", _P), ("dbeta_b", _P), ("gr_gstride", _LL),
                ("mask_out", _P), ("mask_lazy", _I)]


assert ctypes.sizeof(_BnFuse) == int(_L.dba_bnfuse_size()), "BnFuse layout mismatch (rebuild the kernels)"


NOT_HANDLED = -100
F16_PAIR = 16


def _call(name: str, *args) -> int:
    rc = getattr(_L, name)(*args)
    if rc != 0 and rc != NOT_HANDLED:
        raise RuntimeError(f"{name}: HIP error {rc}")
    return rc


def _ptr(t: Optional[Tensor]):
    return None if t is None else t.data_ptr()


def _stream():
    return torch.cuda.current_stream().cuda_stream


def _i32(t: Optional[Tensor]) -> Optional[Tensor]:
    if t is None:
        return None
    return t if (t.dtype == torch.int32 and t.is_contiguous()) else t.to(torch.int32).contiguous()


def _inner_contig(t: Tensor) -> bool:
    exp = 1
    for d in range(t.dim() - 1, 0, -1):
        if t.shape[d] != 1 and t.stride(d) != exp:
            return False
        exp *= t.shape[d]
    return True


def _rowview(t: Tensor) -> Tuple[Tensor, int]:
    if not _inner_contig(t):
        t = t.contiguous()
    return t, (t.stride(0) if t.shape[0] > 1 else int(torch.tensor(t.shape[1:]).prod()))


def _act(t: Tensor, dt: Optional[torch.dtype] = None, what: str = "activation") -> Tensor:
    if t.dtype != _F32:
        raise TypeError(f"{what}: unsupported dtype {t.dtype} (fp32 only)")
    if dt is not None and t.dtype != dt:
        raise TypeError(f"{what}: dtype {t.dtype} does not match the op's {dt} operands "
                        f"(no silent precision conversion)")
    return t.contiguous()


def _f32(t: Tensor) -> int:
    return int(t.dtype == _F32)


_UNIT_AMAX = {}


def _unit_amax(G: int, device):
    key = (G, device)
    if key not in _UNIT_AMAX:
        a = torch.zeros(AMAX_SUB, _amax_ld(G), dtype=torch.int32, device=device)
        a[0, :G] = 0x3F800000
        _UNIT_AMAX[key] = a
    return _UNIT_AMAX[key]


def gather_images(src, labels, idx, trig_masks, trig_id, poison_n, target, flip_seeds, out_dtype):
    G, B = idx.shape
    _, H, W, C = src.shape
    x = torch.empty(G, B, H, W, C, dtype=out_dtype, device=src.device)
    y = torch.empty(G, B, dtype=torch.int32, device=src.device)
    idx, trig_id, poison_n, fs = _i32(idx), _i32(trig_id), _i32(poison_n), _i32(flip_seeds)
    _call("dba_gather_images", src.data_ptr(), _i32(labels).data_ptr(), idx.data_ptr(),
          trig_masks.contiguous().data_ptr(), trig_id.data_ptr(), poison_n.data_ptr(), int(target), _ptr(fs),
          x.data_ptr(), int(out_dtype == torch.float32), y.data_ptr(), G, B, H, W, C, _stream())
    if out_dtype == _F32:
        x._dba_amax = _unit_amax(G, x.device)
    return x, y


def gather_rows(src, labels, idx, trig_cols, trig_vals, trig_id, poison_n, target, out_dtype):
    G, B = idx.shape
    Fd = src.shape[1]
    x = torch.empty(G, B, Fd, dtype=out_dtype, device=src.device)
    y = torch.empty(G, B, dtype=torch.int32, device=src.device)
    tc = _i32(trig_cols)
    _call("dba_gather_rows", src.contiguous().data_ptr(), _i32(labels).data_ptr(), _i32(idx).data_ptr(),
          tc.data_ptr(), trig_vals.float().contiguous().data_ptr(), int(tc.shape[1]), _i32(trig_id).data_ptr(),
          _i32(poison_n).data_ptr(), int(target), x.data_ptr(), int(out_dtype == torch.float32), y.data_ptr(),
          G, B, Fd, _stream())
    return x, y


_MLP_LAYERS = ("layer1.0.weight", "layer1.0.bias", "layer2.0.weight", "layer2.0.bias", "layer3.0.weight",
               "layer3.0.bias")


def mlp_train(spec, sched, t0, t1, B, state, mom, fg, rows, labels, trig_cols, trig_vals, target, stats,
              max_slots, nan_flag, momentum, wd, prof=None) -> int:
    G = state.shape[0]
    es = [spec.by_name[n] for n in _MLP_LAYERS]
    offs = torch.tensor([e.offset for e in es], dtype=torch.int32)
    (H1, F), (H2, _), (C, _) = es[0].k_shape[:2], es[2].k_shape[:2], es[4].k_shape[:2]
    assert sched.dtype == torch.int32 and sched.is_contiguous() and state.stride(1) == 1
    tc = _i32(trig_cols)
    return _call("dba_mlp_train", sched.data_ptr(), sched.shape[1], int(t0), int(t1), G, B, state.data_ptr(),
                 state.stride(0), mom.data_ptr(), _ptr(fg), spec.P, offs.data_ptr(), F, H1, H2, C,
                 rows.contiguous().data_ptr(), _i32(labels).data_ptr(), tc.data_ptr(),
                 trig_vals.float().contiguous().data_ptr(), int(tc.shape[1]), int(target), stats.data_ptr(),
                 stats.shape[1], max_slots, nan_flag.data_ptr(), float(momentum), float(wd), _ptr(prof), _stream())


def _check_w(w: Tensor, dt: torch.dtype = _F32) -> Tuple[Tensor, int]:
    if w.dtype != dt:
        raise TypeError(f"conv weights: dtype {w.dtype} does not match the {dt} activations "
                        f"(no silent precision conversion)")
    return _rowview(w)


def set_ximg(on: int) -> int:
    return int(_L.dba_ximg_set(int(on)))


def set_xstage(on: int) -> int:
    return int(_L.dba_xstage_set(int(on)))


def set_wgrad_halo(on: int) -> int:
    return int(_L.dba_xwgrad_halo_set(int(on)))


def set_split_policy(target: int = -1, min_k: int = -1, max_s: int = -1, kslab_max: int = -1,
                     dgrad_ks: int = -1) -> None:
    _call("dba_xsplit_policy", int(target), int(min_k), int(max_s), int(kslab_max), int(dgrad_ks))


_STEM_WGRAD = True


def set_stem_wgrad(on: int) -> int:
    global _STEM_WGRAD
    prev = int(_STEM_WGRAD)
    if on >= 0:
        _STEM_WGRAD = bool(on)
    return prev


def fp32_mode() -> int:
    return F16_PAIR


AMAX_SUB = 16


def _amax_ld(G: int) -> int:
    return max(32, (G + 31) // 32 * 32)


class _AmaxArena:

    def __init__(self, G: int, device, n: int, counters: int = 0) -> None:
        self.G, self.ld, self.next = G, _amax_ld(G), 0
        slots = n * AMAX_SUB * self.ld
        flat = torch.zeros(slots + counters, dtype=torch.int32, device=device)
        self.buf = flat[:slots].view(n, AMAX_SUB, self.ld)
        self.cnt, self.cnt_next = flat[slots:], 0

    def counters(self, n: int, device):
        if n <= 0 or device != self.cnt.device or self.cnt_next + n > self.cnt.numel():
            return None
        self.cnt_next += n
        return self.cnt[self.cnt_next - n:self.cnt_next]

    def take(self, G: int, device):
        if G != self.G or self.next >= self.buf.shape[0] or device != self.buf.device:
            return None
        self.next += 1
        return self.buf[self.next - 1]


_ARENA: list = []


@contextlib.contextmanager
def amax_arena(G: int, device, n: int = 256, counters: int = 0):
    _ARENA.append(_AmaxArena(G, device, n, counters))
    try:
        yield
    finally:
        _ARENA.pop()


def amax_slots(n: int, G: int, device):
    return torch.zeros(n, AMAX_SUB, _amax_ld(G), dtype=torch.int32, device=device)


def _amax_new(G: int, device):
    a = _ARENA[-1].take(G, device) if _ARENA else None
    return a if a is not None else torch.zeros(AMAX_SUB, _amax_ld(G), dtype=torch.int32, device=device)


def _sk_counters(n: int, device):
    if n <= 0 or not _ARENA:
        return None
    return _ARENA[-1].counters(n, device)


def _aptr(a):
    return (None, 0) if a is None else (a.data_ptr(), a.shape[-1])


def _amax(t, gstride, n_per_g, nvalid=None, per_item=0):
    G = t.shape[0]
    out = _amax_new(G, t.device)
    _call("dba_amax", t.data_ptr(), gstride, n_per_g, _ptr(_i32(nvalid)), per_item, G, out.data_ptr(), out.shape[1],
          _stream())
    return out


def _amax_out(t):
    if t.dtype != _F32:
        return None
    a = _amax_new(t.shape[0], t.device)
    t._dba_amax = a
    return a


def weight_amax(flat, segments):
    G, n = flat.shape[0], len(segments)
    ar = _ARENA[-1] if _ARENA else None
    if ar is not None and ar.G == G and ar.buf.device == flat.device and ar.next + n <= ar.buf.shape[0]:
        buf, ar.next = ar.buf[ar.next:ar.next + n], ar.next + n
    else:
        buf = torch.zeros(n, AMAX_SUB, _amax_ld(G), dtype=torch.int32, device=flat.device)
    slots, base = list(buf), buf.data_ptr()
    d = torch.tensor(segments, dtype=torch.int64)
    _call("dba_amax_segments", flat.data_ptr(), flat.stride(0), d.data_ptr(), len(segments), G, base,
          slots[0].shape[1], _stream())
    return slots


def split_weights(w, sstride: int, per: int, amax):
    slots = w.shape[0]
    out = torch.empty(slots, 2, per, dtype=torch.int16, device=w.device)
    _call("dba_xsplit_w", w.data_ptr(), sstride, per, slots, amax.data_ptr(), amax.shape[1], out.data_ptr(), _stream())
    w._dba_planes = out
    frag_weights_batch([w])
    return out


def split_weights_batch(items) -> None:
    if not items:
        return
    slots = items[0][0].shape[0]
    desc, outs = [], []
    for w, sstride, per, amax in items:
        assert w.shape[0] == slots and w.dtype == torch.float32
        out = torch.empty(slots, 2, per, dtype=torch.int16, device=w.device)
        desc.append([w.data_ptr(), sstride, per, amax.data_ptr(), amax.shape[1], out.data_ptr(), 0])
        outs.append(out)
    d = torch.tensor(desc, dtype=torch.int64)
    _call("dba_xsplit_w_batch", d.data_ptr(), len(items), slots, _stream())
    for (w, *_), out in zip(items, outs):
        w._dba_planes = out
    frag_weights_batch([w for w, *_ in items])


def frag_weights_batch(ws) -> None:
    desc, outs = [], []
    for w in ws:
        p = getattr(w, "_dba_planes", None)
        if (p is None or w.dim() != 5 or tuple(w.shape[2:4]) != (3, 3) or w.shape[1] % 32 or w.shape[4] % 32
                or not p.is_contiguous() or p.shape[2] != w[0].numel()):
            continue
        out = torch.empty(p.shape[0], 2 * p.shape[2], dtype=torch.int16, device=p.device)
        desc.append([p.data_ptr(), out.data_ptr(), w.shape[1], w.shape[4], 0])
        outs.append((w, out))
    if not desc:
        return
    d = torch.tensor(desc, dtype=torch.int64)
    _call("dba_xfrag_w_batch", d.data_ptr(), len(desc), outs[0][1].shape[0], _stream())
    for w, out in outs:
        w._dba_fplanes = out


def _wplanes(w):
    p = getattr(w, "_dba_planes", None)
    return (None, 0) if p is None else (p.data_ptr(), p.stride(0))


def _wfplanes(w):
    p = getattr(w, "_dba_fplanes", None)
    return (None, 0) if p is None else (p.data_ptr(), p.stride(0))


def _wfplanes2(w1, w2):
    (f1, s1), (f2, s2) = _wfplanes(w1), _wfplanes(w2)
    return (f1, f2, s1) if f1 is not None and f2 is not None and s1 == s2 else (None, None, 0)


def _amax_w(w, gstride, n):
    a = getattr(w, "_dba_amax", None)
    if a is None:
        a = _amax(w, gstride, n)
        w._dba_amax = a
    return a


def _amax_act(t, nvalid):
    a = getattr(t, "_dba_amax", None)
    if a is not None:
        return a
    per_item = t[0, 0].numel()
    a = _amax(t, t.stride(0), t.shape[1] * per_item, nvalid, per_item)
    t._dba_amax = a
    return a


_EVAL_STEM_MFMA = os.environ.get("DBA_EVAL_STEM7_MFMA", "1") != "0"
_EVAL_STEM_PAD = True


def _xconv_fwd(x, w, wsel, stride, pad, bias, residual, relu, nvalid, out_dtype, bnf=None, lz=None):
    if out_dtype not in (None, _F32):
        raise TypeError(f"fp32 conv cannot emit {out_dtype} (no silent precision conversion)")
    G, N, H, W, Cin = x.shape
    attrs = {k: getattr(w, k) for k in ("_dba_amax", "_dba_planes", "_dba_fplanes") if hasattr(w, k)}
    w, ws = _check_w(w, _F32)
    for k, v in attrs.items():
        setattr(w, k, v)
    Cout, KH, KW = w.shape[1], w.shape[2], w.shape[3]
    assert w.shape[4] == Cin, (w.shape, x.shape)
    Ho = (H + 2 * pad - KH) // stride + 1
    Wo = (W + 2 * pad - KW) // stride + 1
    y = torch.empty(G, N, Ho, Wo, Cout, dtype=_F32, device=x.device)
    bs = 0
    if bias is not None:
        if bias.dtype != _F32:
            raise TypeError(f"conv bias must be fp32 (got {bias.dtype})")
        bias, bs = _rowview(bias)
    res = _act(residual, _F32, "residual") if residual is not None else None
    ay = _amax_out(y) if bnf is None else None
    bnf_p = ctypes.byref(bnf) if bnf is not None else None
    eval_mfma = (_EVAL_STEM_MFMA and "_dba_planes" in attrs and bnf is None and KH * KW * Cin > 64)
    if eval_mfma and Cin % 4 and _EVAL_STEM_PAD and lz is None:
        cp = 4 - Cin % 4
        x4 = torch.nn.functional.pad(x, (0, cp))
        x4._dba_amax = _amax_act(x, nvalid)
        w4 = torch.nn.functional.pad(w, (0, cp)).contiguous()
        per4 = w4[0].numel()
        a4 = attrs.get("_dba_amax")
        split_weights(w4, per4, per4, a4 if a4 is not None else _amax_w(w4, per4, per4))
        if a4 is not None:
            w4._dba_amax = a4
        return _xconv_fwd(x4, w4, wsel, stride, pad, bias, residual, relu, nvalid, out_dtype)
    if Cin <= 4 and not eval_mfma:
        rc = _call("dba_xstem_fwd", x.data_ptr(), N * H * W * Cin, w.data_ptr(), ws, _ptr(_i32(wsel)), _ptr(bias), bs,
                   _ptr(res), y.data_ptr(), N * Ho * Wo * Cout, _ptr(_i32(nvalid)), G, N, H, W, Cin, Ho, Wo, Cout,
                   KH, KW, stride, pad, int(relu), *_aptr(ay), bnf_p, _stream())
        if rc != NOT_HANDLED:
            return y
    n = int(_L.dba_xconv_ws_floats(G, N, Ho, Wo, Cin, Cout, KH, KW))
    wsb = torch.empty(n, dtype=_F32, device=x.device) if n > 0 else None
    ncnt = int(_L.dba_xconv_sk_ints(G, N, Ho, Wo, Cin, Cout, KH, KW)) if n > 0 else 0
    cnt = _sk_counters(ncnt, x.device)
    ax = lz[2] if lz is not None else _amax_act(x, nvalid)
    aw = _amax_w(w, ws, Cout * KH * KW * Cin)
    lz_coef, lz_relu = (lz[0].data_ptr(), int(lz[1])) if lz is not None else (None, 0)
    _call("dba_xconv_fwd", x.data_ptr(), N * H * W * Cin, w.data_ptr(), ws, _ptr(_i32(wsel)), _ptr(bias), bs,
          _ptr(res), y.data_ptr(), N * Ho * Wo * Cout, _ptr(_i32(nvalid)), G, N, H, W, Cin, Ho, Wo, Cout, KH, KW,
          stride, pad, int(relu), *_aptr(ax), *_aptr(aw), *_aptr(ay), *_wplanes(w), *_wfplanes(w), _ptr(wsb), n,
          _ptr(cnt), 0 if cnt is None else cnt.numel(), bnf_p, lz_coef, lz_relu, _stream())
    return y


_EVAL_BLOCK = os.environ.get("DBA_EVAL_BLOCK", "1") != "0"
_BLOCK_SHAPES = {(32, 32)}


def basic_block_ok(x, w1, w2) -> bool:
    if not (_EVAL_BLOCK and x.dtype == _F32 and x.dim() == 5):
        return False
    H, W, C = x.shape[2:]
    return (H == W and (W, C) in _BLOCK_SHAPES
            and all(w.dtype == _F32 and tuple(w.shape[1:]) == (C, 3, 3, C)
                    and getattr(w, "_dba_planes", None) is not None for w in (w1, w2)))


def basic_block_eval(x, w1, b1, w2, b2, wsel=None, nvalid=None):
    x = _act(x, _F32, "conv input")
    G, N, _, W, C = x.shape
    per = C * 9 * C
    (w1c, ws1), (w2c, ws2) = _check_w(w1), _check_w(w2)
    aw1, aw2 = _amax_w(w1, ws1, per), _amax_w(w2, ws2, per)
    p1, p2 = w1._dba_planes, w2._dba_planes
    assert p1.stride(0) == p2.stride(0) and aw1.shape[1] == aw2.shape[1]
    (b1c, bs1), (b2c, bs2) = _rowview(b1), _rowview(b2)
    assert bs1 == bs2 and b1c.dtype == b2c.dtype == _F32
    ax = _amax_act(x, nvalid)
    y = torch.empty_like(x)
    ay = _amax_out(y)
    rc = _call("dba_xblock_fwd", x.data_ptr(), x.stride(0), y.data_ptr(), y.stride(0), _ptr(_i32(wsel)),
               p1.data_ptr(), p2.data_ptr(), p1.stride(0), *_wfplanes2(w1, w2), b1c.data_ptr(), b2c.data_ptr(), bs1,
               _ptr(_i32(nvalid)), G, N, W, W, C, C, *_aptr(ax), aw1.data_ptr(), aw2.data_ptr(), aw1.shape[1], *_aptr(ay), _stream())
    if rc == NOT_HANDLED:
        raise RuntimeError("xblock_fwd declined a shape basic_block_ok accepted")
    return y


_EVAL_STEM = os.environ.get("DBA_EVAL_STEM", "1") != "0"


def stem_block_ok(x, w0, w1, w2) -> bool:
    if not (_EVAL_STEM and _EVAL_BLOCK and x.dtype == _F32 and x.dim() == 5 and tuple(x.shape[2:]) == (32, 32, 3)):
        return False
    return (w0.dtype == _F32 and tuple(w0.shape[1:]) == (32, 3, 3, 3) and getattr(w0, "_dba_planes", None) is not None
            and all(w.dtype == _F32 and tuple(w.shape[1:]) == (32, 3, 3, 32)
                    and getattr(w, "_dba_planes", None) is not None for w in (w1, w2)))


def stem_block_eval(x, w0, b0, w1, b1, w2, b2, wsel=None, nvalid=None):
    x = _act(x, _F32, "image")
    G, N, _, W, Ci = x.shape
    C = w1.shape[1]
    per = C * 9 * C
    (w0c, ws0), (w1c, ws1), (w2c, ws2) = _check_w(w0), _check_w(w1), _check_w(w2)
    aw0 = _amax_w(w0, ws0, C * 9 * Ci)
    aw1, aw2 = _amax_w(w1, ws1, per), _amax_w(w2, ws2, per)
    p0, p1, p2 = w0._dba_planes, w1._dba_planes, w2._dba_planes
    assert p1.stride(0) == p2.stride(0) and aw0.shape[1] == aw1.shape[1] == aw2.shape[1]
    (b0c, bs0), (b1c, bs1), (b2c, bs2) = _rowview(b0), _rowview(b1), _rowview(b2)
    assert bs1 == bs2 and b0c.dtype == b1c.dtype == b2c.dtype == _F32
    y = torch.empty(G, N, W, W, C, dtype=_F32, device=x.device)
    ay = _amax_out(y)
    rc = _call("dba_xblock_stem_fwd", x.data_ptr(), x.stride(0), y.data_ptr(), y.stride(0), _ptr(_i32(wsel)),
               p0.data_ptr(), p0.stride(0), b0c.data_ptr(), bs0, p1.data_ptr(), p2.data_ptr(), p1.stride(0),
               *_wfplanes2(w1, w2), b1c.data_ptr(), b2c.data_ptr(), bs1, _ptr(_i32(nvalid)), G, N, W, W, Ci, C, aw0.data_ptr(),
               aw1.data_ptr(), aw2.data_ptr(), aw1.shape[1], *_aptr(ay), _stream())
    if rc == NOT_HANDLED:
        raise RuntimeError("xblock_stem_fwd declined a shape stem_block_ok accepted")
    return y


def down_block_ok(a, w2, x2, wsc) -> bool:
    if not (_EVAL_DOWN and a.dtype == _F32 and x2.dtype == _F32 and a.dim() == 5 and x2.dim() == 5):
        return False
    H, W, C = a.shape[2:]
    H2, W2, C2 = x2.shape[2:]
    if H != W or (H2 - 1) // 2 + 1 != H or (W2 - 1) // 2 + 1 != W or a.shape[:2] != x2.shape[:2]:
        return False
    if any(getattr(t, "_dba_planes", None) is None for t in (w2, wsc)):
        return False
    if tuple(w2.shape[1:]) != (C, 3, 3, C) or tuple(wsc.shape[1:]) != (C, 1, 1, C2):
        return False
    return W == 16 and C == 64 and C2 == 32


def down_block_eval(a, w2, b2, x2, wsc, bsc, wsel=None, nvalid=None):
    a = _act(a, _F32, "conv input")
    x2 = _act(x2, _F32, "shortcut input")
    G, N, Ho, Wo, C = a.shape
    _, _, H2, W2, C2 = x2.shape
    (w2c, ws2), (wscc, wss) = _check_w(w2), _check_w(wsc)
    aw2, awsc = _amax_w(w2, ws2, C * 9 * C), _amax_w(wsc, wss, C * C2)
    p2, psc = w2._dba_planes, wsc._dba_planes
    (b2c, bs2), (bscc, bss) = _rowview(b2), _rowview(bsc)
    aa, ax2 = _amax_act(a, nvalid), _amax_act(x2, nvalid)
    y = torch.empty_like(a)
    ay = _amax_out(y)
    rc = _call("dba_xdown_fwd", a.data_ptr(), a.stride(0), w2c.data_ptr(), ws2, p2.data_ptr(), p2.stride(0),
               _ptr(_i32(wsel)), b2c.data_ptr(), bs2, x2.data_ptr(), x2.stride(0), psc.data_ptr(), psc.stride(0),
               bscc.data_ptr(), bss, y.data_ptr(), y.stride(0), _ptr(_i32(nvalid)), G, N, Ho, Wo, C, H2, W2, C2,
               *_aptr(aa), *_aptr(aw2), *_aptr(ax2), *_aptr(awsc), *_aptr(ay), _stream())
    if rc == NOT_HANDLED:
        raise RuntimeError("xdown_fwd declined a shape down_block_ok accepted")
    return y


_EVAL_DOWN = os.environ.get("DBA_EVAL_DOWN", "1") != "0"


def conv2d(x, w, wsel, stride, pad, bias=None, residual=None, relu=False, nvalid=None, out_dtype=None,
           bn_stats=False):
    return _xconv_fwd(_act(x, _F32, "conv input"), w, wsel, stride, pad, bias, residual, relu, nvalid, out_dtype)


def _xtranspose(items) -> list:
    outs, desc, max_per, nv = [], [], 0, None
    slots = items[0][0].shape[0]
    for w, stride, pad, nvalid in items:
        wv, ws = _check_w(w, _F32)
        _, Cout, KH, KW, Cin = wv.shape
        per = Cout * KH * KW * Cin
        wt = torch.empty(slots, per, dtype=_F32, device=wv.device)
        outs.append(wt)
        desc.append([wv.data_ptr(), wt.data_ptr(), ws, Cout, KH, KW, Cin, stride, pad, 0])
        max_per = max(max_per, per)
        nv = nvalid
    d = torch.tensor(desc, dtype=torch.int64)
    _call("dba_xtranspose", d.data_ptr(), len(desc), slots, max_per, _ptr(_i32(nv)), _stream())
    return outs


def prepare_dgrad_weights(ref, items):
    if not items:
        return {}
    slots = items[0][0].shape[0]
    sel = [k for k, it in enumerate(items) if it[0].shape[0] == slots]
    it0 = items[sel[0]]
    nv = it0[5] if (it0[1] is None and it0[5] is not None and slots == it0[6]) else None
    wts = _xtranspose([(items[k][0], items[k][2], items[k][3], nv) for k in sel])
    return dict(zip(sel, wts))


def _xconv_dgrad(dy, w, wsel, stride, pad, in_hw, nvalid, out_dtype, accum, wt, finish=None):
    if out_dtype not in (None, _F32):
        raise TypeError(f"fp32 dgrad cannot emit {out_dtype} (no silent precision conversion)")
    G, N, Ho, Wo, Cout = dy.shape
    wv, _ = _check_w(w, _F32)
    slots, _, KH, KW, Cin = wv.shape
    H, W = in_hw
    if wt is None:
        nv = nvalid if (wsel is None and nvalid is not None and slots == G) else None
        wt = _xtranspose([(wv, stride, pad, nv)])[0]
    per = Cout * KH * KW * Cin
    assert wt.dtype == _F32 and wt.is_contiguous() and wt.numel() == slots * per
    dx = torch.empty(G, N, H, W, Cin, dtype=_F32, device=dy.device)
    acc = _act(accum, _F32, "dgrad accum") if accum is not None else None
    if acc is not None:
        assert acc.shape == dx.shape
    n = int(_L.dba_xconv_ws_floats(G, N, H, W, Cout, Cin, KH, KW)) if stride == 1 else 0
    wsb = torch.empty(n, dtype=_F32, device=dy.device) if n > 0 else None
    cnt = _sk_counters(int(_L.dba_xconv_sk_ints(G, N, H, W, Cout, Cin, KH, KW)) if n > 0 else 0, dy.device)
    a0 = getattr(w, "_dba_amax", None)
    ad, aw = _amax_act(dy, nvalid), (a0 if a0 is not None else _amax(wt, per, per))
    bnf = _bnf_bwd(finish, G, N * H * W, dx.device) if (finish is not None and stride == 1) else None
    _call("dba_xconv_dgrad", dy.data_ptr(), N * Ho * Wo * Cout, wt.data_ptr(), per, _ptr(_i32(wsel)), _ptr(acc),
          dx.data_ptr(), N * H * W * Cin, _ptr(_i32(nvalid)), G, N, H, W, Cin, Ho, Wo, Cout, KH, KW, stride, pad,
          *_aptr(ad), *_aptr(aw), *_wplanes(wt), _ptr(wsb), n, _ptr(cnt), 0 if cnt is None else cnt.numel(),
          ctypes.byref(bnf) if bnf is not None else None, _stream())
    if finish is None:
        return dx
    if bnf is not None:
        return bs.Fin(dx, finish.stats())
    return bn_finish(dx, finish, nvalid)


def conv2d_dgrad(dy, w, wsel, stride, pad, in_hw, nvalid=None, out_dtype=None, accum=None, wt=None, finish=None):
    return _xconv_dgrad(_act(dy, _F32, "dgrad dy"), w, wsel, stride, pad, in_hw, nvalid, out_dtype, accum, wt, finish)


def conv2d_wgrad(dy, x, stride, pad, kh, kw, dw, dbias=None, nvalid=None, defer=None):
    if _stem_wgrad_ok(dy, x, stride, pad, kh, kw, dbias):
        return _stem_wgrad(dy, x, dw, nvalid, defer)
    if isinstance(dy, bs.LazyGrad):
        dy = _bnx_dy(dy, nvalid)
        conv2d_wgrad(dy, x, stride, pad, kh, kw, dw, dbias, nvalid, defer)
        return dy
    lx = x if isinstance(x, bs.LazyBN) else None
    dy = _act(dy, _F32, "wgrad dy")
    x = _act(lx.y if lx is not None else x, _F32, "wgrad x")
    G, N, Ho, Wo, Cout = dy.shape
    _, _, H, W, Cin = x.shape
    assert dw.dtype == torch.float32 and _inner_contig(dw)
    mchunk = ctypes.c_int(0)
    n = int(_L.dba_xwgrad_ws_floats(G, N, Ho, Wo, Cin, Cout, kh, kw, ctypes.byref(mchunk)))
    wsb = torch.empty(n, dtype=_F32, device=dy.device) if n > 0 else None
    nv = _i32(nvalid)
    ad = _amax_act(dy, nvalid)
    ax = lx.stat.bound if lx is not None else _amax_act(x, nvalid)
    _call("dba_xwgrad", dy.data_ptr(), N * Ho * Wo * Cout, x.data_ptr(), N * H * W * Cin, dw.data_ptr(),
          dw.stride(0), _ptr(nv), G, N, H, W, Cin, Ho, Wo, Cout, kh, kw, stride, pad, *_aptr(ad), *_aptr(ax),
          _ptr(wsb), n, int(defer is not None and n > 0),
          _ptr(lx.stat.coef) if lx is not None else None, int(lx.relu) if lx is not None else 0, _stream())
    if defer is not None and n > 0:
        per = Cout * kh * kw * Cin
        defer.append(([wsb.data_ptr(), dw.data_ptr(), dw.stride(0), per, _ptr(nv) or 0, N, Ho * Wo,
                       mchunk.value, G, 0], wsb, nv))
    if dbias is not None:
        assert dbias.dtype == torch.float32 and dbias.stride(1) == 1
        part = torch.empty(int(_L.dba_xcolsum_part_doubles(G, N, Ho * Wo, Cout)), dtype=torch.float64,
                           device=dy.device)
        _call("dba_xcolsum", dy.data_ptr(), N * Ho * Wo * Cout, Ho * Wo, _ptr(_i32(nvalid)), G, N, Cout,
              dbias.data_ptr(), dbias.stride(0), part.data_ptr(), _stream())
    return None


_STEM_PER = 32 * 27


def _stem_wgrad_ok(dy, x, stride, pad, kh, kw, dbias) -> bool:
    if not _STEM_WGRAD or dbias is not None or isinstance(x, bs.LazyBN) or (stride, pad, kh, kw) != (1, 1, 3, 3):
        return False
    d = dy.d if isinstance(dy, bs.LazyGrad) else dy
    if x.dim() != 5 or x.shape[-1] != 3 or x.dtype != _F32 or d.dtype != _F32 or d.shape[-1] != 32:
        return False
    G, N, H, W, _ = x.shape
    return tuple(d.shape) == (G, N, H, W, 32) and int(_L.dba_xwgrad_stem_ws_floats(G, N, H, W, 3, 32)) > 0


def _stem_wgrad(dy, x, dw, nvalid, defer):
    lg = dy if isinstance(dy, bs.LazyGrad) else None
    d = _act(lg.d if lg is not None else dy, _F32, "wgrad dy")
    y = None
    if lg is not None:
        y = _act(lg.y, _F32, "BN input")
        assert y.shape == d.shape and y.stride(0) == d.stride(0)
    x = _act(x, _F32, "wgrad x")
    assert dw.dtype == torch.float32 and _inner_contig(dw) and dw[0].numel() == _STEM_PER
    G, N, H, W, _ = x.shape
    wsb = torch.empty(int(_L.dba_xwgrad_stem_ws_floats(G, N, H, W, 3, 32)), dtype=_F32, device=x.device)
    nv = _i32(nvalid)
    _call("dba_xwgrad_stem", d.data_ptr(), d.stride(0), _ptr(y), _ptr(lg.stat.coef) if lg is not None else None,
          x.data_ptr(), x.stride(0), wsb.data_ptr(), _ptr(nv), G, N, H, W, _stream())
    entry = ([wsb.data_ptr(), dw.data_ptr(), dw.stride(0), _STEM_PER, _ptr(nv) or 0, N, H * W, 256, G, 0], wsb, nv)
    if defer is not None:
        defer.append(entry)
    else:
        wgrad_flush([entry])
    return None


def _bnf_common(mode: int, G: int, M: int, C: int, device):
    ngrp = (M + 31) // 32
    rec0 = torch.empty(G * C * ngrp * 4, dtype=torch.float64, device=device)
    f = _BnFuse()
    f.mode, f.C, f.ngrp, f.rec0 = mode, C, ngrp, rec0.data_ptr()
    f._keep = (rec0,)
    return f


def _bnf_fwd(p: "bs.BnParams", relu: bool, G: int, M: int, C: int, device):
    coef = torch.empty(G, bs.ROWS, C, dtype=_F32, device=device)
    bound = _amax_new(G, device)
    st = bs.BnStat(coef, p, bound)
    f = _bnf_common(1, G, M, C, device)
    ps = _same_stride(p.gamma, p.beta, p.rmean, p.rvar)
    f.coef_a, f.gamma_a, f.beta_a = coef.data_ptr(), p.gamma.data_ptr(), p.beta.data_ptr()
    f.rm_a, f.rv_a, f.p_gstride = p.rmean.data_ptr(), p.rvar.data_ptr(), ps
    f.momentum, f.eps, f.relu = float(p.momentum), float(p.eps), int(relu)
    f.amax_a, f.amax_ld = bound.data_ptr(), bound.shape[1]
    return f, st


def _bnf_bwd(fin: "bs.Finish", G: int, M: int, device):
    sa, sb = fin.sa, fin.sb
    C = sa.C
    f = _bnf_common(2, G, M, C, device)
    ya = _act(fin.ya, _F32, "BN input")
    pa = sa.params
    f.coef_a, f.gamma_a, f.p_gstride = sa.coef.data_ptr(), pa.gamma.data_ptr(), _same_stride(pa.gamma)
    f.ya, f.y_gstride = ya.data_ptr(), ya.stride(0)
    f.dgamma_a, f.dbeta_a, f.gr_gstride = pa.dgamma.data_ptr(), pa.dbeta.data_ptr(), _same_stride(pa.dgamma, pa.dbeta)
    sa.dbound = _amax_new(G, device)
    f.amax_a, f.amax_ld = sa.dbound.data_ptr(), sa.dbound.shape[1]
    keep = [ya]
    if sb is not None:
        yb = _act(fin.yb, _F32, "BN input")
        assert yb.stride(0) == ya.stride(0) and sb.C == C
        pb = sb.params
        assert _same_stride(pb.gamma) == f.p_gstride and _same_stride(pb.dgamma, pb.dbeta) == f.gr_gstride
        f.yb, f.coef_b, f.gamma_b = yb.data_ptr(), sb.coef.data_ptr(), pb.gamma.data_ptr()
        f.dgamma_b, f.dbeta_b = pb.dgamma.data_ptr(), pb.dbeta.data_ptr()
        sb.dbound = _amax_new(G, device)
        f.amax_b = sb.dbound.data_ptr()
        keep.append(yb)
    if fin.mask_out is not None:
        mo = _act(fin.mask_out, _F32, "BN output")
        assert mo.stride(0) == ya.stride(0)
        f.mask_out = mo.data_ptr()
        keep.append(mo)
    f.mask_lazy = int(bool(fin.lazy))
    f._keep = f._keep + tuple(keep)
    return f


def _bnx_dy(lg, nvalid):
    d = _act(lg.d, _F32, "BN output gradient")
    y = _act(lg.y, _F32, "BN input")
    G, N, H, W, C = d.shape
    assert y.shape == d.shape
    dy = torch.empty_like(d)
    am = lg.stat.dbound
    _call("dba_bnx_dy", d.data_ptr(), y.data_ptr(), lg.stat.coef.data_ptr(), dy.data_ptr(), d.stride(0),
          _ptr(_i32(nvalid)), G, N, H * W, C, *_aptr(None), _stream())
    dy._dba_amax = am
    return dy


def conv_bn_stats(x, w, wsel, stride, pad, nvalid, p, relu):
    lz = None
    if isinstance(x, bs.LazyBN):
        if x.stat.bound is None:
            raise RuntimeError("lazy BN operand without its bound slot")
        lz = (x.stat.coef, x.relu, x.stat.bound)
        x = x.y
    x = _act(x, _F32, "conv input")
    G, N, H, W, Cin = x.shape
    Cout, KH, KW = w.shape[1], w.shape[2], w.shape[3]
    Ho = (H + 2 * pad - KH) // stride + 1
    Wo = (W + 2 * pad - KW) // stride + 1
    f, st = _bnf_fwd(p, relu, G, N * Ho * Wo, Cout, x.device)
    y = _xconv_fwd(x, w, wsel, stride, pad, None, None, False, nvalid, None, bnf=f, lz=lz)
    return y, st


def bn_apply(a, residual, relu, nvalid=None):
    y = _act(a.y, _F32, "BN input")
    G, N, H, W, C = y.shape
    out = torch.empty_like(y)
    am = _amax_out(out)
    res = yb = cb = None
    relu_b = 0
    if isinstance(residual, bs.LazyBN):
        yb, cb, relu_b = _act(residual.y, _F32, "BN input"), residual.stat.coef, int(residual.relu)
        assert yb.shape == y.shape
    elif residual is not None:
        res = _act(residual, _F32, "residual")
        assert res.shape == y.shape
    _call("dba_bnx_apply", y.data_ptr(), a.stat.coef.data_ptr(), _ptr(res), _ptr(yb), _ptr(cb), relu_b, int(relu),
          out.data_ptr(), y.stride(0), _ptr(_i32(nvalid)), G, N, H * W, C, *_aptr(am), _stream())
    return out


def bn_finish(g, fin, nvalid=None, pool=None, hw=None):
    ya = _act(fin.ya, _F32, "BN input")
    G, N, H, W, C = ya.shape
    f = _bnf_bwd(fin, G, N * H * W, ya.device)
    d = torch.empty_like(ya)
    src = None
    if pool is not None:
        pool = _act(pool, _F32, "pooled gradient").reshape(G, N, C)
        assert hw == (H, W)
    else:
        src = _act(g, _F32, "BN output gradient")
        assert src.shape == ya.shape
    inv_hw = float(torch.tensor(1.0, dtype=torch.float32) / torch.tensor(float(H * W), dtype=torch.float32))
    _call("dba_bnx_rows", ctypes.byref(f), _ptr(src), d.data_ptr(), ya.stride(0), _ptr(_i32(nvalid)), G, N, H * W,
          _ptr(pool), inv_hw, _stream())
    return bs.Fin(d, fin.stats())


def wgrad_prepare(dy, x, nvalid=None):
    if dy.dtype == _F32:
        _amax_act(_act(dy, None, "wgrad dy"), nvalid)
        _amax_act(_act(x, _F32, "wgrad x"), nvalid)


def wgrad_flush(defer):
    if not defer:
        return
    d = torch.tensor([e[0] for e in defer], dtype=torch.int64)
    Gmax = max(e[0][8] for e in defer)
    max_per = max(e[0][3] for e in defer)
    _call("dba_xwgrad_reduce_batch", d.data_ptr(), len(defer), Gmax, max_per, _stream())
    defer.clear()


def _same_stride(*ts: Tensor) -> int:
    s = ts[0].stride(0)
    for t in ts:
        assert t.dtype == torch.float32 and t.stride(-1) == 1 and (t.shape[0] == 1 or t.stride(0) == s)
    return s


def relu_mask_bwd(dout, out):
    dout = _act(dout, None, "relu dout")
    out = _act(out, dout.dtype, "relu output")
    din = torch.empty_like(dout)
    _call("dba_relu_mask_bwd", dout.data_ptr(), out.data_ptr(), din.data_ptr(), dout.numel(), _f32(dout), _stream())
    return din


def bn_fold(w, conv_bias, gamma, beta, rmean, rvar, eps, out_dtype, amax_slot=None, split=True):
    assert w.dtype == torch.float32 and _inner_contig(w)
    if out_dtype != _F32:
        raise TypeError(f"bn_fold: fp32 weights only (got {out_dtype})")
    slots, Cout = w.shape[0], w.shape[1]
    K = int(torch.tensor(w.shape[2:]).prod())
    ss = _same_stride(gamma, beta, rmean, rvar)
    wf = torch.empty(w.shape, dtype=out_dtype, device=w.device)
    bf = torch.empty(slots, Cout, dtype=torch.float32, device=w.device)
    cb = None
    if conv_bias is not None:
        cb = conv_bias
        assert _same_stride(cb) == ss
    am = amax_slot if amax_slot is not None else _amax_new(slots, w.device)
    assert am.shape[0] == AMAX_SUB and am.shape[1] >= slots
    _call("dba_bn_fold", w.data_ptr(), w.stride(0), _ptr(cb), gamma.data_ptr(), beta.data_ptr(), rmean.data_ptr(),
          rvar.data_ptr(), ss, float(eps), wf.data_ptr(), bf.data_ptr(), slots, Cout, K, int(out_dtype == _F32),
          am.data_ptr(), am.shape[1], _stream())
    wf._dba_amax = am
    if split:
        split_weights(wf, Cout * K, Cout * K, wf._dba_amax)
    return wf, bf


def bn_fold_batch(items, eps: float):
    if not items:
        return []
    slots = items[0][0].shape[0]
    desc, outs = [], []
    for w, gamma, beta, rmean, rvar, am in items:
        assert w.dtype == torch.float32 and _inner_contig(w) and w.shape[0] == slots
        Cout = w.shape[1]
        K = int(torch.tensor(w.shape[2:]).prod())
        ss = _same_stride(gamma, beta, rmean, rvar)
        assert am.shape[0] == AMAX_SUB and am.shape[1] >= slots
        wf = torch.empty(w.shape, dtype=_F32, device=w.device)
        bf = torch.empty(slots, Cout, dtype=torch.float32, device=w.device)
        desc.append([w.data_ptr(), w.stride(0), gamma.data_ptr(), beta.data_ptr(), rmean.data_ptr(), rvar.data_ptr(),
                     ss, wf.data_ptr(), bf.data_ptr(), Cout, K, am.data_ptr(), am.shape[1], 0])
        wf._dba_amax = am
        outs.append((wf, bf))
    d = torch.tensor(desc, dtype=torch.int64)
    _call("dba_bn_fold_batch", d.data_ptr(), len(items), slots, float(eps), _stream())
    return outs


def maxpool2d(x, k, s, p, want_ind=True):
    x = _act(x, None, "maxpool input")
    G, N, H, W, C = x.shape
    Ho = (H + 2 * p - k) // s + 1
    Wo = (W + 2 * p - k) // s + 1
    y = torch.empty(G, N, Ho, Wo, C, dtype=x.dtype, device=x.device)
    ind = torch.empty(G, N, Ho, Wo, C, dtype=torch.int32, device=x.device) if want_ind else None
    _call("dba_maxpool", x.data_ptr(), y.data_ptr(), _ptr(ind), G * N, H, W, C, Ho, Wo, k, s, p, _f32(x),
          _stream())
    return y, ind


def maxpool2d_bwd(dy, ind, in_shape, k, s, p):
    dy = _act(dy, None, "maxpool dy")
    G, N, H, W, C = in_shape
    Ho, Wo = dy.shape[2], dy.shape[3]
    dx = torch.empty(G, N, H, W, C, dtype=dy.dtype, device=dy.device)
    _call("dba_maxpool_bwd", dy.data_ptr(), ind.data_ptr(), dx.data_ptr(), G * N, H, W, C, Ho, Wo, k, s, p, _f32(dy),
          _stream())
    return dx


def avgpool_global(x):
    x = _act(x, None, "avgpool input")
    G, N, H, W, C = x.shape
    y = torch.empty(G, N, 1, 1, C, dtype=x.dtype, device=x.device)
    _call("dba_avgpool", x.data_ptr(), y.data_ptr(), G * N, H * W, C, _f32(x), _stream())
    return y


def avgpool_global_bwd(dy, hw):
    dy = _act(dy, None, "avgpool dy")
    G, N = dy.shape[:2]
    C = dy.shape[-1]
    H, W = hw
    dx = torch.empty(G, N, H, W, C, dtype=dy.dtype, device=dy.device)
    _call("dba_avgpool_bwd", dy.data_ptr(), dx.data_ptr(), G * N, H * W, C, _f32(dy), _stream())
    return dx


def dropout(x, p, seeds, salt):
    x = _act(x, None, "dropout input")
    y = torch.empty_like(x)
    G = x.shape[0]
    _call("dba_dropout", x.data_ptr(), y.data_ptr(), _f32(x), _i32(seeds).data_ptr(),
          int(salt) & 0xFFFFFFFF, float(p), x.numel() // G, G, _stream())
    return y


def dropout_bwd(dy, p, seeds, salt):
    return dropout(dy, p, seeds, salt)


def softmax_xent(logits, labels, mean, want_grad, stats=None, slot=None, nvalid=None, grad_dtype=None,
                 loss_dtype=None):
    if logits.dtype != _F32:
        raise TypeError("softmax_xent: logits must be fp32 (the final layer emits fp32)")
    lf = logits.contiguous()
    G, B, C = lf.shape
    gdt = grad_dtype or _F32
    if gdt != _F32:
        raise TypeError(f"softmax_xent: unsupported grad dtype {gdt}")
    loss = torch.empty(G, dtype=torch.float32, device=lf.device)
    loss64 = torch.empty(G, dtype=torch.float64, device=lf.device) if loss_dtype == torch.float64 else None
    correct = torch.empty(G, dtype=torch.float32, device=lf.device)
    dl = torch.empty(G, B, C, dtype=gdt, device=lf.device) if want_grad else None
    sp, ss, slp, ms, nvp = None, 0, None, 0, None
    if stats is not None:
        assert stats.dtype == torch.float32 and stats.is_contiguous() and stats.shape[0] == 3
        ms = stats.shape[1] // G
        assert ms * G == stats.shape[1]
        slot_, nv_ = _i32(slot), _i32(nvalid)
        sp, ss, slp, nvp = stats.data_ptr(), stats.shape[1], slot_.data_ptr(), nv_.data_ptr()
    npart = int(_L.dba_softmax_xent_part_doubles(G, B))
    part = torch.empty(npart, dtype=torch.float64, device=lf.device) if npart > 0 else None
    _call("dba_softmax_xent", lf.data_ptr(), _i32(labels).data_ptr(), G, B, C, int(bool(mean)), _ptr(dl),
          loss.data_ptr(), correct.data_ptr(), sp, ss, slp, ms, nvp, int(gdt == _F32), _ptr(loss64), _ptr(part),
          _stream())
    return (loss64 if loss64 is not None else loss), correct, dl


_FUSED_HEAD = os.environ.get("DBA_FUSED_HEAD", "0") == "1"


def head_ok(x, w) -> bool:
    return (_FUSED_HEAD and x.dtype == _F32 and x.dim() == 5 and x.shape[-1] <= 512 and x.shape[-1] % 4 == 0 and x.shape[1] <= 256
            and x.shape[2] * x.shape[3] <= 64
            and w.dim() == 3 and w.shape[1] <= 16 and w.shape[2] == x.shape[-1] and w.dtype == _F32
            and w.stride(2) == 1 and w.stride(1) == w.shape[2])


def head_train(x, w, b, labels, nvalid, dw, db, stats=None, slot=None, mean=True):
    x = _act(x, _F32, "head input")
    G, N, H, W_, C = x.shape
    K = w.shape[1]
    assert head_ok(x, w) and b.stride(-1) == 1 and dw.stride(-1) == 1 and db.stride(-1) == 1
    pooled = torch.empty(G, N, C, dtype=_F32, device=x.device)
    dlog = torch.empty(G, N, 16, dtype=_F32, device=x.device)
    part = torch.empty(int(_L.dba_head_part_doubles(G, N)), dtype=torch.float64, device=x.device)
    dpool = torch.empty(G, N, 1, 1, C, dtype=_F32, device=x.device)
    loss = torch.empty(G, dtype=_F32, device=x.device)
    correct = torch.empty(G, dtype=_F32, device=x.device)
    sp, ss, slp, ms = None, 0, None, 0
    if stats is not None:
        ms = stats.shape[1] // G
        sp, ss, slp = stats.data_ptr(), stats.shape[1], _i32(slot).data_ptr()
    rc = _call("dba_head_train", x.data_ptr(), x.stride(0), G, N, H * W_, C, w.data_ptr(), w.stride(0), b.data_ptr(),
               b.stride(0), K, _i32(labels).data_ptr(), _ptr(_i32(nvalid)), pooled.data_ptr(), dlog.data_ptr(),
               part.data_ptr(), dw.data_ptr(),
               dw.stride(0), db.data_ptr(), db.stride(0), dpool.data_ptr(), loss.data_ptr(), correct.data_ptr(), sp, ss,
               slp, ms, int(bool(mean)), _stream())
    if rc == NOT_HANDLED:
        raise RuntimeError("head_train declined a shape head_ok accepted")
    return loss, correct, dpool


def sgd_step(params, grads, mom, lr, first, active, momentum, wd, fg_accum=None):
    G, P = grads.shape
    assert params.dtype == torch.float32 and params.stride(1) == 1 and params.stride(0) % 4 == 0
    assert grads.is_contiguous() and mom.is_contiguous() and P % 4 == 0
    _call("dba_sgd_step", params.data_ptr(), params.stride(0), grads.data_ptr(), mom.data_ptr(),
          lr.float().contiguous().data_ptr(), _i32(first).data_ptr(), _i32(active).data_ptr(), float(momentum),
          float(wd), _ptr(fg_accum), G, P, _stream())


def dist_loss_grad(w, base, grads, trig, active, alpha):
    G, P = grads.shape
    assert w.dtype == torch.float32 and w.stride(1) == 1 and base.stride(1) == 1 and grads.is_contiguous()
    assert w.shape[0] >= G and base.shape[0] >= G and w.shape[1] >= P and base.shape[1] >= P
    nrm2 = torch.zeros(G, dtype=torch.float32, device=grads.device)
    part = torch.empty(G, 256, dtype=torch.float32, device=grads.device)
    _call("dba_dist_loss_grad", w.data_ptr(), w.stride(0), base.data_ptr(), base.stride(0), grads.data_ptr(), P, G,
          _i32(trig).data_ptr(), _i32(active).data_ptr(), float(alpha), nrm2.data_ptr(), part.data_ptr(), _stream())
    return nrm2.sqrt()


def scale_from_base(w, base, gamma):
    w = w.contiguous()
    base = base.contiguous()
    out = torch.empty_like(w)
    _call("dba_scale_from_base", w.data_ptr(), base.data_ptr(), float(gamma), out.data_ptr(), w.numel(), _stream())
    return out


def add_noise_scaled(dst, upd, coef, sigma, seed, noise):
    assert dst.is_contiguous() and dst.dtype == torch.float32
    if upd.dtype not in (torch.float32, torch.float64):
        upd = upd.float()
    upd = upd.contiguous()
    _call("dba_add_noise_scaled", dst.data_ptr(), upd.data_ptr(), dst.numel(), float(coef), float(sigma),
          int(seed) & 0xFFFFFFFF, int(bool(noise)), int(upd.dtype == torch.float64), _stream())


def delta_sum(rows, base):
    assert rows.dtype == torch.float32 and base.dtype == torch.float32
    n = base.numel()
    out = torch.empty(n, dtype=torch.float64, device=base.device)
    if rows.shape[0] == 0:
        out.zero_()
        return out
    assert rows.stride(-1) == 1 and rows.shape[1] >= n
    base = base.contiguous()
    _call("dba_delta_sum", rows.data_ptr(), rows.stride(0), rows.shape[0], base.data_ptr(), n, out.data_ptr(),
          _stream())
    return out


def sq_dists(points, m):
    assert points.stride(1) == 1 and points.dtype == torch.float32
    m = m.float().contiguous()
    n, L = points.shape
    out = torch.empty(n, dtype=torch.float64, device=points.device)
    part = torch.empty(n * int(_L.dba_sqdist_blocks(L)), dtype=torch.float64, device=points.device)
    _call("dba_sq_dists", points.data_ptr(), points.stride(0), m.data_ptr(), n, L, out.data_ptr(), part.data_ptr(),
          _stream())
    return out


def weighted_sum(points, wts, out_dtype=None):
    assert points.stride(1) == 1 and points.dtype == torch.float32
    odt = out_dtype or torch.float32
    n, L = points.shape
    out = torch.empty(L, dtype=odt, device=points.device)
    _call("dba_weighted_sum", points.data_ptr(), points.stride(0), wts.float().contiguous().data_ptr(), n,
          out.data_ptr(), L, int(odt == torch.float64), _stream())
    return out


def weighted_sum_fixed(points, wts, E):
    assert points.stride(1) == 1 and points.dtype == torch.float32
    n, L = points.shape
    out = torch.empty(2, L, dtype=torch.int64, device=points.device)
    _call("dba_weighted_sum_fixed", points.data_ptr(), points.stride(0), wts.float().contiguous().data_ptr(), n,
          out.data_ptr(), L, float(2.0 ** E), _stream())
    return out


def _delta_rows(rows, base):
    assert rows.dtype == torch.float32 and base.dtype == torch.float32
    assert rows.dim() == 2 and rows.shape[1] == base.numel(), (tuple(rows.shape), base.numel())
    assert base.is_cuda and rows.device == base.device
    if rows.shape[1] > 1 and rows.stride(1) != 1:
        rows = rows.contiguous()
    return rows, (rows.stride(0) if rows.shape[0] > 1 else rows.shape[1]), base.contiguous()


def _clip_scale(scale, n, device):
    assert scale.numel() == n
    return scale.to(device=device, dtype=torch.float32).contiguous()


def delta_stats(rows, base):
    rows, rs, base = _delta_rows(rows, base)
    n, L = rows.shape
    if n == 0 or L == 0:
        return (torch.zeros(n, dtype=torch.float64, device=base.device),
                torch.zeros(n, dtype=torch.float32, device=base.device))
    sq = torch.empty(n, dtype=torch.float64, device=base.device)
    mx = torch.empty(n, dtype=torch.float32, device=base.device)
    nb = int(_L.dba_delta_stats_blocks(L))
    part_sq = torch.empty(n * nb, dtype=torch.float64, device=base.device)
    part_mx = torch.empty(n * nb, dtype=torch.float32, device=base.device)
    _call("dba_delta_stats", rows.data_ptr(), rs, n, base.data_ptr(), L, sq.data_ptr(), mx.data_ptr(),
          part_sq.data_ptr(), part_mx.data_ptr(), _stream())
    return sq, mx


def clipped_delta_sum_fixed(rows, base, scale, E):
    rows, rs, base = _delta_rows(rows, base)
    n, L = rows.shape
    if n == 0 or L == 0:
        return torch.zeros(2, L, dtype=torch.int64, device=base.device)
    scale = _clip_scale(scale, n, base.device)
    out = torch.empty(2, L, dtype=torch.int64, device=base.device)
    _call("dba_clipped_delta_sum_fixed", rows.data_ptr(), rs, n, base.data_ptr(), scale.data_ptr(), out.data_ptr(),
          L, float(2.0 ** E), _stream())
    return out


def clipped_delta_sum(rows, base, scale):
    rows, rs, base = _delta_rows(rows, base)
    n, L = rows.shape
    if n == 0 or L == 0:
        return torch.zeros(L, dtype=torch.float64, device=base.device)
    scale = _clip_scale(scale, n, base.device)
    out = torch.empty(L, dtype=torch.float64, device=base.device)
    _call("dba_clipped_delta_sum", rows.data_ptr(), rs, n, base.data_ptr(), scale.data_ptr(), out.data_ptr(), L,
          _stream())
    return out


PAIRWISE_MAX_ROWS = 64


def pairwise_sq_dists(buf, row_idx=None):
    assert buf.dtype == torch.float32 and buf.dim() == 2 and buf.is_cuda
    if buf.shape[1] > 1 and buf.stride(1) != 1:
        buf = buf.contiguous()
    R, L = buf.shape
    idx = None
    if row_idx is not None:
        rows = [int(r) for r in (row_idx.tolist() if isinstance(row_idx, Tensor) else row_idx)]
        if not all(0 <= r < R for r in rows):
            raise ValueError(f"pairwise_sq_dists: row_idx {rows} outside the {R} rows of buf")
        idx = torch.tensor(rows, dtype=torch.int32, device=buf.device)
    n = R if idx is None else idx.numel()
    if n > PAIRWISE_MAX_ROWS:
        return _ref.pairwise_sq_dists(buf, row_idx)
    if n < 2 or L == 0:
        return torch.zeros(n, n, dtype=torch.float64, device=buf.device)
    rs = buf.stride(0) if R > 1 else L
    out = torch.empty(n, n, dtype=torch.float64, device=buf.device)
    nb = int(_L.dba_pairwise_sqdist_blocks(L))
    part = torch.empty(n * (n - 1) // 2 * nb, dtype=torch.float64, device=buf.device)
    _call("dba_pairwise_sqdist", buf.data_ptr(), rs, _ptr(idx), n, L, out.data_ptr(), part.data_ptr(), _stream())
    return out


TRIM_MAX_ROWS = 64


def trimmed_delta_sum(buf, base, k, row_idx=None):
    assert buf.dtype == torch.float32 and buf.dim() == 2 and buf.is_cuda
    assert base.dtype == torch.float32 and base.device == buf.device
    if buf.shape[1] > 1 and buf.stride(1) != 1:
        buf = buf.contiguous()
    R, L = buf.shape
    assert base.numel() == L, (tuple(buf.shape), base.numel())
    idx = None
    if row_idx is not None:
        rows = [int(r) for r in (row_idx.tolist() if isinstance(row_idx, Tensor) else row_idx)]
        if not all(0 <= r < R for r in rows):
            raise ValueError(f"trimmed_delta_sum: row_idx {rows} outside the {R} rows of buf")
        idx = torch.tensor(rows, dtype=torch.int32, device=buf.device)
    n = R if idx is None else idx.numel()
    k = _ref.check_trim(n, k)
    if n > TRIM_MAX_ROWS or L >= 1 << 31:
        return _ref.trimmed_delta_sum(buf, base, k, row_idx)
    if n == 0 or L == 0:
        return (torch.zeros(L, dtype=torch.float64, device=buf.device),
                torch.zeros(n, dtype=torch.int64, device=buf.device),
                torch.zeros(n, dtype=torch.int64, device=buf.device))
    rs = buf.stride(0) if R > 1 else L
    base = base.contiguous()
    total = torch.empty(L, dtype=torch.float64, device=buf.device)
    counts = torch.empty(n, 2, dtype=torch.int64, device=buf.device)
    part = torch.empty(2 * n * int(_L.dba_coord_trim_blocks(L)), dtype=torch.int64, device=buf.device)
    _call("dba_coord_trim", buf.data_ptr(), rs, _ptr(idx), n, base.data_ptr(), k, L, total.data_ptr(),
          counts.data_ptr(), part.data_ptr(), _stream())
    return total, counts[:, 0].contiguous(), counts[:, 1].contiguous()


RLR_MAX_ROWS = 65535


def _rlr_theta(theta) -> int:
    theta = int(theta)
    if not -(1 << 31) <= theta < (1 << 31):
        raise ValueError(f"rlr: theta {theta} does not fit an int32")
    return theta


def delta_sum_votes(rows, base):
    rows, rs, base = _delta_rows(rows, base)
    n, L = rows.shape
    if n == 0 or L == 0:
        return (torch.zeros(L, dtype=torch.float64, device=base.device),
                torch.zeros(L, dtype=torch.int32, device=base.device))
    total = torch.empty(L, dtype=torch.float64, device=base.device)
    votes = torch.empty(L, dtype=torch.int32, device=base.device)
    _call("dba_delta_sum_votes", rows.data_ptr(), rs, n, base.data_ptr(), L, total.data_ptr(), votes.data_ptr(),
          _stream())
    return total, votes


def vote_agreement(rows, base, votes, theta):
    rows, rs, base = _delta_rows(rows, base)
    n, L = rows.shape
    theta = _rlr_theta(theta)
    assert votes.dtype == torch.int32 and votes.numel() == L and votes.device == base.device
    if n == 0 or L == 0:
        return torch.zeros(n, 2, dtype=torch.int64, device=base.device)
    if n > RLR_MAX_ROWS:
        return torch.cat([vote_agreement(rows[i:i + RLR_MAX_ROWS], base, votes, theta)
                          for i in range(0, n, RLR_MAX_ROWS)])
    votes = votes.reshape(-1).contiguous()
    counts = torch.empty(n, 2, dtype=torch.int64, device=base.device)
    part = torch.empty(2 * n * int(_L.dba_vote_agreement_blocks(L)), dtype=torch.int64, device=base.device)
    _call("dba_vote_agreement", rows.data_ptr(), rs, n, base.data_ptr(), votes.data_ptr(), theta, L,
          counts.data_ptr(), part.data_ptr(), _stream())
    return counts


def rlr_apply(dst, total, votes, theta, coef, sigma, seed, noise):
    assert dst.is_contiguous() and dst.dtype == torch.float32 and dst.dim() == 1 and dst.is_cuda
    L = dst.numel()
    theta = _rlr_theta(theta)
    assert total.dtype == torch.float64 and total.numel() == L and total.device == dst.device
    assert votes.dtype == torch.int32 and votes.numel() == L and votes.device == dst.device
    if L == 0:
        return torch.zeros((), dtype=torch.int64, device=dst.device)
    flipped = torch.empty((), dtype=torch.int64, device=dst.device)
    total, votes = total.reshape(-1).contiguous(), votes.reshape(-1).contiguous()
    part = torch.empty(int(_L.dba_rlr_apply_blocks(L)), dtype=torch.int64, device=dst.device)
    _call("dba_rlr_apply", dst.data_ptr(), total.data_ptr(), votes.data_ptr(), theta, L, float(coef), float(sigma),
          int(seed) & 0xFFFFFFFF, int(bool(noise)), flipped.data_ptr(), part.data_ptr(), _stream())
    return flipped


def gram(feats):
    f = feats.float()
    if f.stride(1) != 1:
        f = f.contiguous()
    n, d = f.shape
    out = torch.empty(n, n, dtype=torch.float64, device=f.device)
    slab = torch.empty(int(_L.dba_gram_chunks(d)) * n * n, dtype=torch.float32, device=f.device)
    _call("dba_gram", f.data_ptr(), f.stride(0), n, d, out.data_ptr(), slab.data_ptr(), _stream())
    return out
```

dba_mod_amd/ops/reference.py:

```python
from __future__ import annotations

from typing import Optional, Sequence, Tuple

import torch
import torch.nn.functional as F

from . import bnstate as bs
from . import rng

Tensor = torch.Tensor


def _sel(w: Tensor, wsel: Optional[Tensor], g: int) -> Tensor:
    return w[int(wsel[g])] if wsel is not None else w[g]


def _nchw(x: Tensor) -> Tensor:
    return x.permute(0, 3, 1, 2)


def _nhwc(x: Tensor) -> Tensor:
    return x.permute(0, 2, 3, 1)


COMPUTE_DTYPE = torch.float32


def _cdt() -> torch.dtype:
    return COMPUTE_DTYPE


def _rows_valid(nvalid: Optional[Tensor], g: int, n: int) -> int:
    return n if nvalid is None else int(nvalid[g])


def gather_images(src: Tensor, labels: Tensor, idx: Tensor, trig_masks: Tensor, trig_id: Tensor,
                  poison_n: Tensor, target: int, flip_seeds: Optional[Tensor], out_dtype: torch.dtype
                  ) -> Tuple[Tensor, Tensor]:
    G, B = idx.shape
    _, H, W, C = src.shape
    valid = idx >= 0
    safe = idx.clamp(min=0).long()
    x = src[safe.reshape(-1)].reshape(G, B, H, W, C).to(torch.float32)
    y = labels.long()[safe.reshape(-1)].reshape(G, B)
    if flip_seeds is not None:
        ctr = torch.arange(B, dtype=torch.int64, device=src.device)[None, :].expand(G, B)
        flip = (rng.hash2(flip_seeds.to(torch.int64)[:, None], ctr) & 1).bool()
        x = torch.where(flip[..., None, None, None], x.flip(3), x)
    b_ar = torch.arange(B, device=src.device)[None, :]
    tid = trig_id.long()
    pois = (b_ar < poison_n.long()[:, None]) & (tid[:, None] >= 0) & valid
    if trig_masks.numel() > 0:
        m = trig_masks[tid.clamp(min=0)].bool()
        pm = pois[:, :, None, None] & m[:, None, :, :]
        x = torch.where(pm[..., None], torch.full_like(x, 255.0), x)
    y = torch.where(pois, torch.full_like(y, int(target)), y)
    x = x * (1.0 / 255.0)
    x = torch.where(valid[..., None, None, None], x, torch.zeros_like(x))
    y = torch.where(valid, y, torch.full_like(y, -1))
    return x.to(out_dtype), y.to(torch.int32)


def gather_rows(src: Tensor, labels: Tensor, idx: Tensor, trig_cols: Tensor, trig_vals: Tensor,
                trig_id: Tensor, poison_n: Tensor, target: int, out_dtype: torch.dtype
                ) -> Tuple[Tensor, Tensor]:
    G, B = idx.shape
    Fd = src.shape[1]
    valid = idx >= 0
    safe = idx.clamp(min=0).long()
    x = src[safe.reshape(-1)].reshape(G, B, Fd).to(torch.float32).clone()
    y = labels.long()[safe.reshape(-1)].reshape(G, B)
    b_ar = torch.arange(B, device=src.device)[None, :]
    tid = trig_id.long()
    pois = (b_ar < poison_n.long()[:, None]) & (tid[:, None] >= 0) & valid
    for g in range(G):
        if int(tid[g]) < 0:
            continue
        cols = trig_cols[int(tid[g])]
        vals = trig_vals[int(tid[g])]
        rows = pois[g].nonzero().flatten()
        for k in range(cols.shape[0]):
            c = int(cols[k])
            if c >= 0:
                x[g, rows, c] = float(vals[k])
    y = torch.where(pois, torch.full_like(y, int(target)), y)
    x = torch.where(valid[..., None], x, torch.zeros_like(x))
    y = torch.where(valid, y, torch.full_like(y, -1))
    return x.to(out_dtype), y.to(torch.int32)


def conv2d(x: Tensor, w: Tensor, wsel: Optional[Tensor], stride: int, pad: int,
           bias: Optional[Tensor] = None, residual: Optional[Tensor] = None,
           relu: bool = False, nvalid: Optional[Tensor] = None,
           out_dtype: Optional[torch.dtype] = None, bn_stats: bool = False) -> Tensor:
    G = x.shape[0]
    outs = []
    for g in range(G):
        wg = _sel(w, wsel, g).to(_cdt()).permute(0, 3, 1, 2)
        bg = _sel(bias, wsel, g).to(_cdt()) if bias is not None else None
        yg = F.conv2d(_nchw(x[g].to(_cdt())), wg, bg, stride=stride, padding=pad)
        yg = _nhwc(yg)
        if residual is not None:
            yg = yg + residual[g].to(_cdt())
        if relu:
            yg = torch.relu(yg)
        outs.append(yg)
    if out_dtype == torch.float32 and _cdt() == torch.float64:
        out_dtype = torch.float64
    return torch.stack(outs).to(out_dtype or x.dtype)


def basic_block_ok(x: Tensor, w1: Tensor, w2: Tensor) -> bool:
    return False


def basic_block_eval(x: Tensor, w1: Tensor, b1: Tensor, w2: Tensor, b2: Tensor,
                     wsel: Optional[Tensor] = None, nvalid: Optional[Tensor] = None) -> Tensor:
    h = conv2d(x, w1, wsel, 1, 1, bias=b1, relu=True, nvalid=nvalid)
    return conv2d(h, w2, wsel, 1, 1, bias=b2, residual=x, relu=True, nvalid=nvalid)


def stem_block_ok(x: Tensor, w0: Tensor, w1: Tensor, w2: Tensor) -> bool:
    return False


def stem_block_eval(x: Tensor, w0: Tensor, b0: Tensor, w1: Tensor, b1: Tensor, w2: Tensor, b2: Tensor,
                    wsel: Optional[Tensor] = None, nvalid: Optional[Tensor] = None) -> Tensor:
    s = conv2d(x, w0, wsel, 1, 1, bias=b0, relu=True, nvalid=nvalid)
    return basic_block_eval(s, w1, b1, w2, b2, wsel, nvalid)


def down_block_ok(a: Tensor, w2: Tensor, x2: Tensor, wsc: Tensor) -> bool:
    return False


def down_block_eval(a: Tensor, w2: Tensor, b2: Tensor, x2: Tensor, wsc: Tensor, bsc: Tensor,
                    wsel: Optional[Tensor] = None, nvalid: Optional[Tensor] = None) -> Tensor:
    sc = conv2d(x2, wsc, wsel, 2, 0, bias=bsc, nvalid=nvalid)
    return conv2d(a, w2, wsel, 1, 1, bias=b2, residual=sc, relu=True, nvalid=nvalid)


def _valid_mask(t: Tensor, nvalid: Optional[Tensor]) -> Tensor:
    G, N = t.shape[:2]
    n = torch.full((G,), N, dtype=torch.int64) if nvalid is None else nvalid.long().cpu()
    v = torch.arange(N)[None, :] < n[:, None]
    return v.view(G, N, *([1] * (t.dim() - 2))).to(t.device)


def _coef(st: "bs.BnStat", row: int, t: Tensor) -> Tensor:
    return st.coef[:, row].view(t.shape[0], *([1] * (t.dim() - 2)), t.shape[-1]).to(t.dtype)


def lazy_value(a: "bs.LazyBN", nvalid: Optional[Tensor] = None) -> Tensor:
    v = a.y * _coef(a.stat, bs.SCALE, a.y) + _coef(a.stat, bs.SHIFT, a.y)
    if a.relu:
        m = getattr(a.stat, "relu_mask", None)
        tiny = 1e-300 if v.dtype == torch.float64 else 1e-30
        v = torch.relu(v) if m is None else torch.where(m.to(v.device), v.clamp(min=tiny), torch.zeros_like(v))
    return torch.where(_valid_mask(v, nvalid), v, torch.zeros_like(v))


def lazy_grad_value(lg: "bs.LazyGrad", nvalid: Optional[Tensor] = None) -> Tensor:
    st = lg.stat
    v = _coef(st, bs.A, lg.d) * lg.d + _coef(st, bs.B, lg.y) * lg.y + _coef(st, bs.K, lg.d)
    return torch.where(_valid_mask(v, nvalid), v, torch.zeros_like(v)).to(lg.d.dtype)


def conv_bn_stats(x, w: Tensor, wsel: Optional[Tensor], stride: int, pad: int, nvalid: Optional[Tensor],
                  p: "bs.BnParams", relu: bool):
    xv = lazy_value(x, nvalid) if isinstance(x, bs.LazyBN) else x
    y = conv2d(xv, w, wsel, stride, pad, nvalid=nvalid)
    G, N = y.shape[:2]
    C = y.shape[-1]
    coef = torch.zeros(G, bs.ROWS, C, dtype=_cdt(), device=y.device)
    for g in range(G):
        n = _rows_valid(nvalid, g, N)
        if n == 0:
            continue
        flat = y[g, :n].to(_cdt()).reshape(-1, C)
        cnt = flat.shape[0]
        mean = flat.mean(0)
        var = flat.var(0, unbiased=False)
        invstd = torch.rsqrt(var + p.eps)
        unbiased = var * (cnt / max(cnt - 1, 1))
        p.rmean[g] = (1 - p.momentum) * p.rmean[g] + p.momentum * mean
        p.rvar[g] = (1 - p.momentum) * p.rvar[g] + p.momentum * unbiased
        sc = invstd * p.gamma[g].to(_cdt())
        coef[g, bs.MEAN], coef[g, bs.INV] = mean, invstd
        coef[g, bs.SCALE], coef[g, bs.SHIFT] = sc, p.beta[g].to(_cdt()) - mean * sc
        coef[g, bs.YMAX], coef[g, bs.YMIN] = flat.max(0).values, flat.min(0).values
    return y, bs.BnStat(coef, p)


def bn_apply(a: "bs.LazyBN", residual, relu: bool, nvalid: Optional[Tensor] = None) -> Tensor:
    v = a.y * _coef(a.stat, bs.SCALE, a.y) + _coef(a.stat, bs.SHIFT, a.y)
    if isinstance(residual, bs.LazyBN):
        v = v + lazy_value(residual, nvalid)
    elif residual is not None:
        v = v + residual.to(v.dtype)
    if relu:
        v = torch.relu(v)
    return torch.where(_valid_mask(v, nvalid), v, torch.zeros_like(v)).to(a.y.dtype)


def bn_finish(g: Optional[Tensor], fin: "bs.Finish", nvalid: Optional[Tensor] = None,
              pool: Optional[Tensor] = None, hw: Optional[Tuple[int, int]] = None) -> "bs.Fin":
    if pool is not None:
        g = avgpool_global_bwd(pool, hw)
    ya = fin.ya
    d = g.to(_cdt())
    if fin.mask_out is not None:
        d = d * (fin.mask_out.to(_cdt()) > 0)
    elif fin.lazy:
        m = getattr(fin.sa, "relu_mask", None)
        pre = ya.to(_cdt()) * _coef(fin.sa, bs.SCALE, ya).to(_cdt()) + _coef(fin.sa, bs.SHIFT, ya).to(_cdt())
        d = d * ((pre > 0) if m is None else m.to(d.device))
    d = torch.where(_valid_mask(d, nvalid), d, torch.zeros_like(d))
    G, N = d.shape[:2]
    C = d.shape[-1]
    for y, st in ((ya, fin.sa), (fin.yb, fin.sb)):
        if st is None:
            continue
        p = st.params
        for gg in range(G):
            n = _rows_valid(nvalid, gg, N)
            if n == 0:
                continue
            dg = d[gg, :n].reshape(-1, C)
            mean, inv = st.coef[gg, bs.MEAN].to(_cdt()), st.coef[gg, bs.INV].to(_cdt())
            xhat = (y[gg, :n].to(_cdt()).reshape(-1, C) - mean) * inv
            cnt = dg.shape[0]
            sd, sdx = dg.sum(0), (dg * xhat).sum(0)
            p.dbeta[gg] += sd.to(p.dbeta.dtype)
            p.dgamma[gg] += sdx.to(p.dgamma.dtype)
            A = p.gamma[gg].to(_cdt()) * inv
            B = -A * inv * sdx / cnt
            st.coef[gg, bs.A], st.coef[gg, bs.B] = A, B
            st.coef[gg, bs.K] = -A * sd / cnt - B * mean
    return bs.Fin(d.to(g.dtype), fin.stats())


def wgrad_prepare(dy, x, nvalid=None):
    return None


def wgrad_flush(defer: list) -> None:
    if defer:
        defer.clear()


def prepare_dgrad_weights(ref: Tensor, items: list) -> dict:
    return {}


def conv2d_dgrad(dy: Tensor, w: Tensor, wsel: Optional[Tensor], stride: int, pad: int,
                 in_hw: Tuple[int, int], nvalid: Optional[Tensor] = None,
                 out_dtype: Optional[torch.dtype] = None, accum: Optional[Tensor] = None,
                 wt: Optional[Tensor] = None, finish: Optional["bs.Finish"] = None):
    if finish is not None:
        dx = conv2d_dgrad(dy, w, wsel, stride, pad, in_hw, nvalid, out_dtype, accum, wt)
        return bn_finish(dx, finish, nvalid)
    G, N = dy.shape[:2]
    cin = w.shape[-1]
    outs = []
    for g in range(G):
        wg = _sel(w, wsel, g).to(_cdt()).permute(0, 3, 1, 2)
        dx = torch.nn.grad.conv2d_input((N, cin, in_hw[0], in_hw[1]), wg, _nchw(dy[g].to(_cdt())),
                                        stride=stride, padding=pad)
        outs.append(_nhwc(dx))
    dx = torch.stack(outs)
    if accum is not None:
        dx = dx + accum.to(dx.dtype)
    return dx.to(out_dtype or dy.dtype)


def conv2d_wgrad(dy, x, stride: int, pad: int, kh: int, kw: int,
                 dw: Tensor, dbias: Optional[Tensor] = None, nvalid: Optional[Tensor] = None,
                 defer: Optional[list] = None) -> Optional[Tensor]:
    out = None
    if isinstance(dy, bs.LazyGrad):
        dy = out = lazy_grad_value(dy, nvalid)
    if isinstance(x, bs.LazyBN):
        x = lazy_value(x, nvalid)
    G = dy.shape[0]
    cout = dy.shape[-1]
    cin = x.shape[-1]
    for g in range(G):
        gw = torch.nn.grad.conv2d_weight(_nchw(x[g].to(_cdt())), (cout, cin, kh, kw),
                                         _nchw(dy[g].to(_cdt())), stride=stride, padding=pad)
        dw[g] += gw.permute(0, 2, 3, 1)
        if dbias is not None:
            dbias[g] += dy[g].to(_cdt()).sum(dim=(0, 1, 2))
    return out


def relu_mask_bwd(dout: Tensor, out: Tensor) -> Tensor:
    return (dout.to(_cdt()) * (out.to(_cdt()) > 0)).to(dout.dtype)


def bn_fold(w: Tensor, conv_bias: Optional[Tensor], gamma: Tensor, beta: Tensor,
            rmean: Tensor, rvar: Tensor, eps: float, out_dtype: torch.dtype,
            amax_slot: Optional[Tensor] = None, split: bool = True) -> Tuple[Tensor, Tensor]:
    s = gamma.to(_cdt()) * torch.rsqrt(rvar.to(_cdt()) + eps)
    wf = w.to(_cdt()) * s[:, :, None, None, None]
    b0 = conv_bias.to(_cdt()) if conv_bias is not None else torch.zeros_like(s)
    bf = (b0 - rmean.to(_cdt())) * s + beta.to(_cdt())
    return wf.to(out_dtype), bf.contiguous()


def maxpool2d(x: Tensor, k: int, s: int, p: int, want_ind: bool = True) -> Tuple[Tensor, Optional[Tensor]]:
    G, N, H, W, C = x.shape
    y, ind = F.max_pool2d(_nchw(x.to(_cdt()).reshape(G * N, H, W, C)), k, s, p, return_indices=True)
    return (_nhwc(y).reshape(G, N, y.shape[2], y.shape[3], C).to(x.dtype),
            _nhwc(ind).reshape(G, N, y.shape[2], y.shape[3], C).to(torch.int32))


def maxpool2d_bwd(dy: Tensor, ind: Tensor, in_shape: Sequence[int], k: int, s: int, p: int) -> Tensor:
    G, N, H, W, C = in_shape
    Ho, Wo = dy.shape[2], dy.shape[3]
    dyn = _nchw(dy.to(_cdt()).reshape(G * N, Ho, Wo, C)).contiguous()
    indn = _nchw(ind.long().reshape(G * N, Ho, Wo, C)).contiguous()
    dx = torch.zeros(G * N, C, H * W, dtype=_cdt(), device=dy.device)
    dx.scatter_add_(2, indn.reshape(G * N, C, -1), dyn.reshape(G * N, C, -1))
    return _nhwc(dx.reshape(G * N, C, H, W)).reshape(G, N, H, W, C).to(dy.dtype)


def avgpool_global(x: Tensor) -> Tensor:
    return x.to(_cdt()).mean(dim=(2, 3), keepdim=True).to(x.dtype)


def avgpool_global_bwd(dy: Tensor, hw: Tuple[int, int]) -> Tensor:
    H, W = hw
    return (dy.to(_cdt()).expand(-1, -1, H, W, -1) / (H * W)).to(dy.dtype).contiguous()


def dropout(x: Tensor, p: float, seeds: Tensor, salt: int) -> Tensor:
    G = x.shape[0]
    per = x[0].numel()
    ctr = torch.arange(per, dtype=torch.int64, device=x.device)[None, :].expand(G, per)
    s = rng.salted(seeds.to(torch.int64), salt)[:, None]
    keep = (rng.uniform01(s, ctr) >= p).reshape(x.shape)
    return (x.to(_cdt()) * keep / (1.0 - p)).to(x.dtype)


def dropout_bwd(dy: Tensor, p: float, seeds: Tensor, salt: int) -> Tensor:
    return dropout(dy, p, seeds, salt)


def softmax_xent(logits: Tensor, labels: Tensor, mean: bool, want_grad: bool,
                 stats: Optional[Tensor] = None, slot: Optional[Tensor] = None,
                 nvalid: Optional[Tensor] = None, grad_dtype: Optional[torch.dtype] = None,
                 loss_dtype: Optional[torch.dtype] = None) -> Tuple[Tensor, Tensor, Optional[Tensor]]:
    G, B, C = logits.shape
    lf = logits.to(_cdt())
    lab = labels.long()
    valid = lab >= 0
    logp = torch.log_softmax(lf, dim=-1)
    nll = -logp.gather(-1, lab.clamp(min=0)[..., None]).squeeze(-1)
    nll = torch.where(valid, nll, torch.zeros_like(nll))
    cnt = valid.sum(1).clamp(min=1).to(_cdt())
    if loss_dtype == torch.float64:
        nll = nll.to(torch.float64)
        cnt = cnt.to(torch.float64)
    loss = nll.sum(1) / cnt if mean else nll.sum(1)
    pred = lf.argmax(-1)
    correct = ((pred == lab) & valid).sum(1).to(_cdt())
    dl = None
    if want_grad:
        dl = torch.softmax(lf, -1)
        dl = dl - F.one_hot(lab.clamp(min=0), C).to(_cdt())
        dl = torch.where(valid[..., None], dl, torch.zeros_like(dl))
        if mean:
            dl = dl / cnt[:, None, None]
        dl = dl.to(grad_dtype or logits.dtype)
    if stats is not None:
        accumulate_step_stats(stats, slot, loss, correct, nvalid)
    return loss, correct, dl


def accumulate_step_stats(stats: Tensor, slot: Tensor, loss: Tensor, correct: Tensor, nvalid: Tensor) -> None:
    G = loss.shape[0]
    ms = stats.shape[1] // G
    col = torch.arange(G, device=stats.device, dtype=torch.int64) * ms + slot.long()
    stats[0].index_add_(0, col, loss.to(stats.dtype))
    stats[1].index_add_(0, col, correct.to(stats.dtype))
    stats[2].index_add_(0, col, nvalid.to(stats.dtype))


def sgd_step(params: Tensor, grads: Tensor, mom: Tensor, lr: Tensor, first: Tensor, active: Tensor,
             momentum: float, wd: float, fg_accum: Optional[Tensor] = None) -> None:
    for g in range(params.shape[0]):
        if int(active[g]) == 0:
            continue
        gr = grads[g]
        if fg_accum is not None:
            fg_accum[g] += gr
        dp = gr + wd * params[g]
        if int(first[g]):
            mom[g] = dp
        else:
            mom[g] = momentum * mom[g] + dp
        params[g] -= float(lr[g]) * mom[g]


def dist_loss_grad(w: Tensor, base: Tensor, grads: Tensor, trig: Tensor, active: Tensor,
                   alpha: float) -> Tensor:
    G, P = grads.shape
    out = torch.zeros(G, dtype=torch.float32, device=grads.device)
    for g in range(G):
        if int(trig[g]) < 0 or int(active[g]) == 0:
            continue
        d = w[g, :P] - base[g, :P]
        nr = torch.linalg.vector_norm(d.double()).float()
        out[g] = nr
        c = (1.0 - alpha) / nr if float(nr) > 0 else 0.0
        grads[g] = alpha * grads[g] + c * d
    return out


def scale_from_base(w: Tensor, base: Tensor, gamma: float) -> Tensor:
    return base + (w - base) * gamma


def add_noise_scaled(dst: Tensor, upd: Tensor, coef: float, sigma: float, seed: int,
                     noise: bool) -> None:
    u = (upd * coef).to(dst.dtype)
    if noise:
        ctr = torch.arange(u.numel(), dtype=torch.int64, device=u.device).reshape(u.shape)
        u = u + sigma * rng.normal(seed, ctr)
    dst += u


def delta_sum(rows: Tensor, base: Tensor) -> Tensor:
    n = base.numel()
    if rows.shape[0] == 0:
        return torch.zeros(n, dtype=torch.float64, device=base.device)
    return (rows[:, :n].double() - base.double()[None]).sum(0)


def sq_dists(points: Tensor, m: Tensor) -> Tensor:
    d = points.double() - m.double()[None]
    return (d * d).sum(1)


def weighted_sum(points: Tensor, wts: Tensor, out_dtype: Optional[torch.dtype] = None) -> Tensor:
    return (wts.double()[:, None] * points.double()).sum(0).to(out_dtype or points.dtype)


def weighted_sum_fixed(points: Tensor, wts: Tensor, E: int) -> Tensor:
    q = (wts.float().double()[:, None] * points.double()) * (2.0 ** E)
    hi = torch.floor(q)
    lo = torch.floor((q - hi) * 2.0 ** 53)
    return torch.stack([hi.to(torch.int64).sum(0), lo.to(torch.int64).sum(0)])


def delta_stats(rows: Tensor, base: Tensor) -> Tuple[Tensor, Tensor]:
    n = rows.shape[0]
    sq = torch.zeros(n, dtype=torch.float64, device=base.device)
    mx = torch.zeros(n, dtype=torch.float32, device=base.device)
    if base.numel() == 0:
        return sq, mx
    b = base.double()
    inf = torch.tensor(float("inf"), dtype=torch.float32, device=base.device)
    for i in range(n):
        d = rows[i].double() - b
        sq[i] = (d * d).sum()
        a = d.float().abs()
        mx[i] = torch.where(a.isnan(), inf, a).max()
    return sq, mx


def clipped_delta_sum_fixed(rows: Tensor, base: Tensor, scale: Tensor, E: int) -> Tensor:
    L = base.numel()
    if rows.shape[0] == 0:
        return torch.zeros(2, L, dtype=torch.int64, device=base.device)
    d = rows.double() - base.double()[None]
    q = (scale.float().double()[:, None] * d) * (2.0 ** E)
    hi = torch.floor(q)
    lo = torch.floor((q - hi) * 2.0 ** 53)
    return torch.stack([hi.to(torch.int64).sum(0), lo.to(torch.int64).sum(0)])


def clipped_delta_sum(rows: Tensor, base: Tensor, scale: Tensor) -> Tensor:
    L = base.numel()
    if rows.shape[0] == 0:
        return torch.zeros(L, dtype=torch.float64, device=base.device)
    return (scale.float().double()[:, None] * (rows.double() - base.double()[None])).sum(0)


PAIRWISE_CHUNK = 1 << 18


def pairwise_sq_dists(buf: Tensor, row_idx=None) -> Tensor:
    assert buf.dim() == 2
    idx = None
    if row_idx is not None:
        idx = torch.as_tensor(row_idx, dtype=torch.int64, device=buf.device).reshape(-1)
    n = buf.shape[0] if idx is None else idx.numel()
    L = buf.shape[1]
    D = torch.zeros(n, n, dtype=torch.float64, device=buf.device)
    if n < 2:
        return D
    for c0 in range(0, L, PAIRWISE_CHUNK):
        x = buf[:, c0:c0 + PAIRWISE_CHUNK]
        x = (x if idx is None else x.index_select(0, idx)).double()
        for i in range(n - 1):
            d = x[i + 1:] - x[i][None]
            D[i, i + 1:] += (d * d).sum(1)
    return D + D.t()


TRIM_CHUNK = 1 << 18


def check_trim(n: int, k: int) -> int:
    if isinstance(k, bool) or not isinstance(k, int) or k < 0 or (2 * k + 1 > n and not (n == 0 and k == 0)):
        raise ValueError(f"trimmed_delta_sum: k = {k!r} needs 0 <= k <= (n - 1) // 2 (n = {n})")
    return k


def trimmed_delta_sum(buf: Tensor, base: Tensor, k: int, row_idx=None) -> Tuple[Tensor, Tensor, Tensor]:
    assert buf.dim() == 2
    idx = None
    if row_idx is not None:
        idx = torch.as_tensor(row_idx, dtype=torch.int64, device=buf.device).reshape(-1)
    n = buf.shape[0] if idx is None else idx.numel()
    L = buf.shape[1]
    k = check_trim(n, k)
    total = torch.zeros(L, dtype=torch.float64, device=buf.device)
    kept = torch.zeros(n, dtype=torch.int64, device=buf.device)
    high = torch.zeros(n, dtype=torch.int64, device=buf.device)
    if n == 0:
        return total, kept, high
    b = base.double()
    for c0 in range(0, L, TRIM_CHUNK):
        x = buf[:, c0:c0 + TRIM_CHUNK]
        x = x if idx is None else x.index_select(0, idx)
        s = torch.sort(x, dim=0).values
        bc = b[c0:c0 + TRIM_CHUNK]
        t = s[k].double() - bc
        for r in range(k + 1, n - k):
            t = t + (s[r].double() - bc)
        total[c0:c0 + TRIM_CHUNK] = t
        lo, hi = s[k][None], s[n - 1 - k][None]
        is_low = x < lo
        is_high = (x > hi) | (x.isnan() & ~hi.isnan())
        kept += (~is_low & ~is_high).sum(1)
        high += is_high.sum(1)
    return total, kept, high


RLR_CHUNK = 1 << 18


def _rlr_rows(rows: Tensor, base: Tensor) -> Tuple[int, int]:
    assert rows.dim() == 2 and rows.dtype == torch.float32 and base.dtype == torch.float32
    assert rows.shape[1] == base.numel(), (tuple(rows.shape), base.numel())
    return rows.shape[0], rows.shape[1]


def delta_sum_votes(rows: Tensor, base: Tensor) -> Tuple[Tensor, Tensor]:
    n, L = _rlr_rows(rows, base)
    total = torch.zeros(L, dtype=torch.float64, device=base.device)
    votes = torch.zeros(L, dtype=torch.int32, device=base.device)
    for c0 in range(0, L if n else 0, RLR_CHUNK):
        b = base[c0:c0 + RLR_CHUNK]
        bd = b.double()
        t = total[c0:c0 + RLR_CHUNK]
        v = votes[c0:c0 + RLR_CHUNK]
        for i in range(n):
            x = rows[i, c0:c0 + RLR_CHUNK]
            t += x.double() - bd
            v += (x > b).to(torch.int32) - (x < b).to(torch.int32)
    return total, votes


def vote_agreement(rows: Tensor, base: Tensor, votes: Tensor, theta: int) -> Tensor:
    n, L = _rlr_rows(rows, base)
    assert votes.numel() == L
    votes = votes.reshape(-1)
    counts = torch.zeros(n, 2, dtype=torch.int64, device=base.device)
    for c0 in range(0, L if n else 0, RLR_CHUNK):
        b = base[c0:c0 + RLR_CHUNK][None]
        x = rows[:, c0:c0 + RLR_CHUNK]
        V = votes[c0:c0 + RLR_CHUNK].to(torch.int64)
        s = (x > b).to(torch.int64) - (x < b).to(torch.int64)
        m = torch.sign(V)[None]
        live = ((V.abs() >= int(theta))[None]) & (s != 0)
        counts[:, 0] += (live & (s == m)).sum(1)
        counts[:, 1] += (live & (s == -m)).sum(1)
    return counts


def rlr_apply(dst: Tensor, total: Tensor, votes: Tensor, theta: int, coef: float, sigma: float, seed: int,
              noise: bool) -> Tensor:
    L = dst.numel()
    assert dst.dim() == 1 and total.numel() == L and votes.numel() == L and total.dtype == torch.float64
    total, votes = total.reshape(-1), votes.reshape(-1)
    flipped = torch.zeros((), dtype=torch.int64, device=dst.device)
    cpos = torch.tensor(float(coef), dtype=torch.float64, device=dst.device)
    for c0 in range(0, L, RLR_CHUNK):
        t = total[c0:c0 + RLR_CHUNK]
        kept = votes[c0:c0 + RLR_CHUNK].to(torch.int64).abs() >= int(theta)
        u = (t * torch.where(kept, cpos, -cpos)).to(dst.dtype)
        if noise:
            ctr = torch.arange(c0, c0 + u.numel(), dtype=torch.int64, device=u.device)
            u = u + sigma * rng.normal(seed, ctr)
        dst[c0:c0 + RLR_CHUNK] += u
        flipped += (~kept).sum()
    return flipped


def gram(feats: Tensor) -> Tensor:
    f = feats.double()
    return f @ f.t()
```

Before: 3.855.

## Add dedicated stride-2 3x3 conv kernel with fused 1x1 shortcut for eval

Adds a specialized stride-2 3x3 convolution kernel (xs2) for two fixed shapes. It stages the input patch in shared memory as split half planes and streams fragment-ordered weights through a register ring. For the downsampling block entry in eval mode, it also computes the 1x1 shortcut conv from the same staged patch, so the input is read once instead of twice and a launch is saved. Weight fragment prep is extended to 1x1 kernels to support this. The cost is a large amount of new hand-tuned code limited to specific shapes, with fallbacks to the old path elsewhere.

```diff
diff --git a/csrc/kernels/xaux.hip b/csrc/kernels/xaux.hip
--- a/csrc/kernels/xaux.hip
+++ b/csrc/kernels/xaux.hip
@@ -49,7 +49,7 @@
 }
 
 struct XFDesc {
-  long long planes, out, ncol, cs, boff;
+  long long planes, out, ncol, cs, taps, boff;
 };
 struct XFBatch {
   XFDesc d[kXSBatch];
@@ -59,13 +59,13 @@
   int i = 0;
   while (i + 1 < b.n && (long long)blockIdx.x >= b.d[i + 1].boff) ++i;
   const XFDesc& d = b.d[i];
-  const int Cs = (int)d.cs, K = 9 * Cs, NK = K / 32;
+  const int Cs = (int)d.cs, taps = (int)d.taps, K = taps * Cs, NK = K / 32;
   const long long per = d.ncol * K;
   const long long idx = ((long long)blockIdx.x - d.boff) * 256 + threadIdx.x;
   if (idx >= per / 4) return;
   const int l = (int)(idx & 63), f = (int)(idx >> 6) & 3, p = f & 1, kk = f >> 1;
   const long long tt = idx >> 8;
-  const int t = (int)(tt % NK), nt = (int)(tt / NK), cc = t / 9, tap = t - cc * 9;
+  const int t = (int)(tt % NK), nt = (int)(tt / NK), cc = t / taps, tap = t - cc * taps;
   const long long e = (long long)(nt * 32 + (l & 31)) * K + tap * Cs + cc * 32 + (kk * 2 + (l >> 5)) * 8;
   const uint16_t* __restrict__ src = (const uint16_t*)d.planes + ((long long)blockIdx.y * 2 + p) * per;
   uint16_t* __restrict__ dst = (uint16_t*)d.out + (long long)blockIdx.y * 2 * per;
@@ -164,10 +164,11 @@
     long long nb = 0;
     for (int i = 0; i < b.n; ++i) {
       b.d[i] = ds[i0 + i];
-      if (b.d[i].ncol <= 0 || b.d[i].cs <= 0 || b.d[i].ncol % 32 || b.d[i].cs % 32 || ((b.d[i].planes | b.d[i].out) & 15))
+      if (b.d[i].ncol <= 0 || b.d[i].cs <= 0 || b.d[i].ncol % 32 || b.d[i].cs % 32 || ((b.d[i].planes | b.d[i].out) & 15) ||
+          (b.d[i].taps != 9 && b.d[i].taps != 1))
         return -105;
       b.d[i].boff = nb;
-      nb += b.d[i].ncol * 9 * b.d[i].cs / 1024;
+      nb += b.d[i].ncol * b.d[i].taps * b.d[i].cs / 1024;
     }
     hipLaunchKernelGGL(xfrag_w_kernel, dim3((unsigned)nb, slots), dim3(256), 0, (hipStream_t)stream, b);
     const int rc = (int)hipGetLastError();
diff --git a/csrc/kernels/xconv_fwd.hip b/csrc/kernels/xconv_fwd.hip
--- a/csrc/kernels/xconv_fwd.hip
+++ b/csrc/kernels/xconv_fwd.hip
@@ -1,4 +1,5 @@
 #include "xhalo.hpp"
+#include "xconv_s2.hpp"
 
 namespace xg {
 SplitPolicy& split_policy() {
@@ -550,6 +551,40 @@
   DBA_LAUNCH_CHECK();
 }
 
+int xs2_kslab(long long M, int G, int Ncol, int K, bool have_ws, const int* sk_cnt, long long sk_cnt_n) {
+  const int s = xsplitk(M, G, Ncol, K);
+  if (s == 1) return 1;
+  if (have_ws && sk_ok(sk_cnt, sk_cnt_n, M, Ncol, G, 1, s)) return -1;
+  if (s <= split_policy().kslab_max && Ncol > 64) return s;
+  return have_ws ? -1 : 1;
+}
+int xs2_run(xg::XS2Args& b, int G, int W, int Cin, int Cout, const float* ws, long long ws_floats, const int* sk_cnt,
+            long long sk_cnt_n, hipStream_t st) {
+  const int form = (W == 32 && Cin == 32 && Cout == 64) ? 0 : (W == 16 && Cin == 64 && Cout == 128) ? 1 : -1;
+  const bool entry = b.sc_out != nullptr;
+  const int mode = xg::xs2_mode();
+  if (form < 0 || (entry && form != 1)) return -100;
+  if (!(mode == 3 || (mode == 1 && xg::xs2_default(form, entry)))) return -100;
+  if ((long long)b.N * W * W * Cin >= (1LL << 29)) return -100;
+  if (!b.amax_src || !b.amax_w || !b.wf || !b.out) return -100;
+  if (!aligned16(b.src) || b.src_gstride % 4) return -100;
+  if (((uintptr_t)b.wf & 15) || b.wf_sstride % 8 || b.wf_sstride < 2LL * Cout * 9 * Cin) return -100;
+  const long long M = (long long)b.N * (W / 2) * (W / 2);
+  const int K = 9 * Cin;
+  const int s = xsplitk(M, G, Cout, K);
+  const bool have_ws = s > 1 && ws != nullptr && ws_floats >= (long long)s * G * M * Cout;
+  b.kslab = xs2_kslab(M, G, Cout, K, have_ws, sk_cnt, sk_cnt_n);
+  if (b.kslab < 1) return -100;
+  b.amax_bm = b.kslab > 1 ? 64 : xconv_bm(M, Cout, G, 1, 1);
+  if (entry) {
+    if (!b.sc_wf || !b.sc_amax_w) return -100;
+    if (((uintptr_t)b.sc_wf & 15) || b.sc_wf_sstride % 8 || b.sc_wf_sstride < 2LL * Cout * Cin) return -100;
+    if (xsplitk(M, G, Cout, Cin) != 1) return -100;
+    b.sc_amax_bm = xconv_bm(M, Cout, G, 1, 1);
+  }
+  return xg::xs2_launch(b, form, G, st);
+}
+
 int& ximg_on() {
   static int on = 1;
   return on;
@@ -597,6 +632,34 @@
   const int prev = xg::xstage_mode();
   if (on >= 1 && on <= 3) xg::xstage_mode() = on;
   return prev;
+}
+
+DBA_EXPORT int dba_xs2_set(int on) {
+  const int prev = xg::xs2_mode();
+  if (on >= 1 && on <= 3) xg::xs2_mode() = on;
+  return prev;
+}
+
+DBA_EXPORT int dba_xs2_entry_fwd(const float* x, long long x_gstride, const int* wsel, const int* nvalid, int G, int N,
+                                 int W, int Cin, int Cout, const int* amax_x, int amax_x_ld, const uint16_t* w1f,
+                                 long long w1f_sstride, const int* amax_w1, int amax_w1_ld, const float* b1,
+                                 long long b1_sstride, float* a_out, long long a_gstride, int* amax_a, int amax_a_ld,
+                                 const uint16_t* wscf, long long wscf_sstride, const int* amax_wsc, int amax_wsc_ld,
+                                 const float* bsc, long long bsc_sstride, float* sc_out, long long sc_gstride,
+                                 int* amax_sc, int amax_sc_ld, void* stream) {
+  if (!x || !w1f || !wscf || !a_out || !sc_out || !amax_x || !amax_w1 || !amax_wsc) return -109;
+  if (G < 1 || N < 1 || W < 2 || (W & 1)) return -100;
+  xg::XS2Args b{};
+  b.src = x; b.src_gstride = x_gstride; b.wsel = wsel; b.nvalid = nvalid; b.N = N;
+  b.amax_src = amax_x; b.amax_src_ld = amax_x_ld;
+  b.wf = w1f; b.wf_sstride = w1f_sstride; b.amax_w = amax_w1; b.amax_w_ld = amax_w1_ld;
+  b.bias = b1; b.b_sstride = b1_sstride; b.out = a_out; b.out_gstride = a_gstride;
+  b.amax_out = amax_a; b.amax_out_ld = amax_a_ld; b.relu = 1;
+  b.sc_wf = wscf; b.sc_wf_sstride = wscf_sstride; b.sc_amax_w = amax_wsc; b.sc_amax_w_ld = amax_wsc_ld;
+  b.sc_bias = bsc; b.sc_b_sstride = bsc_sstride; b.sc_out = sc_out; b.sc_out_gstride = sc_gstride;
+  b.sc_amax_out = amax_sc; b.sc_amax_out_ld = amax_sc_ld;
+  static const float kWs = 0.f;
+  return xs2_run(b, G, W, Cin, Cout, &kWs, 1LL << 62, nullptr, 0, (hipStream_t)stream);
 }
 
 
@@ -654,6 +717,17 @@
     if (rc == -100) rc = xhalo_try(a, G, KH, KW, st);
     if (rc != -100) return fin(rc);
   }
+  if (stride == 2 && KH == 3 && KW == 3 && pad == 1 && H == W && !(W & 1) && Ho == H / 2 && Wo == W / 2 && !bnf &&
+      !lz_coef && !res && wp && wf) {
+    xg::XS2Args b{};
+    b.src = x; b.src_gstride = x_gstride; b.wsel = wsel; b.nvalid = nvalid; b.N = N;
+    b.amax_src = amax_x; b.amax_src_ld = amax_x_ld;
+    b.wf = wf; b.wf_sstride = wf_sstride; b.amax_w = amax_w; b.amax_w_ld = amax_w_ld;
+    b.bias = bias; b.b_sstride = b_sstride; b.out = out; b.out_gstride = out_gstride;
+    b.amax_out = amax_out; b.amax_out_ld = amax_out_ld; b.relu = relu;
+    const int rc = xs2_run(b, G, W, Cin, Cout, ws, ws_floats, sk_cnt, sk_cnt_n, st);
+    if (rc != -100) return rc;
+  }
   const int s = xsplitk(M, G, Cout, K);
   const bool ws_ok = s > 1 && ws != nullptr && ws_floats >= (long long)s * G * M * Cout;
   if (s > 1 && !(ws_ok && sk_ok(sk_cnt, sk_cnt_n, M, Cout, G, 1, s))) {
diff --git a/csrc/kernels/xconv_s2.hip b/csrc/kernels/xconv_s2.hip
--- /dev/null
+++ b/csrc/kernels/xconv_s2.hip
@@ -0,0 +1,310 @@
+#include "xconv_s2.hpp"
+#include "xmfma.hpp"
+#include "xs2_geom.hpp"
+#include <algorithm>
+
+namespace xg {
+int& xs2_mode() {
+  static int mode = 1;
+  return mode;
+}
+bool xs2_default(int form, bool entry) {
+  constexpr bool kA = true, kB = true, kBEntry = true;
+  return form == 0 ? kA : entry ? kBEntry : kB;
+}
+}
+
+namespace {
+
+using xg::XS2Args;
+
+template <class GE, int BN, int RING, bool SC, bool KS>
+__global__ __launch_bounds__(256, 2) void xs2_kernel(const XS2Args a) {
+  constexpr int P = 2, NT = 256;
+  constexpr int CB = GE::CB, PATCH = GE::PATCH, WO = GE::WO, BM = GE::BM;
+  constexpr int WIN = GE::WIN, CIN = GE::CIN;
+  constexpr int WN = BN / 32, WM = (NT / 64) / WN, TM = BM / WM, MI = TM / 32;
+  static_assert(WM * WN == NT / 64 && MI >= 1 && TM % 32 == 0, "wave tiling");
+  static_assert(!(SC && KS), "no instantiation: see xs2_launch");
+  constexpr int NK = 9 * CB;
+  extern __shared__ __attribute__((aligned(16))) uint4 xs2_patch[];
+  __shared__ float xs2_red[(NT / 64) * MI];
+
+  const int tid = threadIdx.x, lane = tid & 63, wid = tid >> 6;
+  const int wm = wid / WN, wn = wid % WN;
+  const int fr = lane & 31, hf = lane >> 5;
+
+  const int tiles_g = a.N * GE::HT, total = a.G * tiles_g;
+  struct Tile { int g, img, oy0; };
+  auto tile_at = [&](int T) __attribute__((always_inline)) {
+    Tile t;
+    t.g = T / tiles_g;
+    const int r = T - t.g * tiles_g;
+    t.img = r / GE::HT;
+    t.oy0 = (r - t.img * GE::HT) * GE::TR;
+    return t;
+  };
+  auto next_valid = [&](int T) __attribute__((always_inline)) {
+    for (; T < total; T += gridDim.x) {
+      const Tile t = tile_at(T);
+      if (t.img < min(valid_rows(a.nvalid, t.g, a.N), a.N)) break;
+    }
+    return T;
+  };
+
+  constexpr int NE = GE::PR;
+  static_assert(GE::FILL_THREADS == NT, "fill mapping");
+  float4 pv[NE];
+  auto pload = [&](const Tile& t) __attribute__((always_inline)) {
+    const __amdgpu_buffer_rsrc_t rA =
+        rsrc(a.src + (long long)t.g * a.src_gstride, (long long)a.N * WIN * WIN * CIN * 4);
+    const int h0 = 2 * t.oy0 - 1;
+    const int gbase = ((t.img * WIN + h0) * WIN + GE::fill_pc(tid) - 1) * CIN + GE::fill_q(tid) * 4;
+#pragma unroll
+    for (int u = 0; u < NE; ++u) {
+      const bool ok = (unsigned)(h0 + u) < (unsigned)WIN;
+      pv[u] = bload4(rA, ok ? (gbase + u * WIN * CIN) * 4 : kOOB);
+    }
+  };
+
+  int T = next_valid(blockIdx.x);
+  if (T >= total) return;
+  pload(tile_at(T));
+  if (tid < GE::ZUNITS) {
+    const int o = GE::zero_unit(tid);
+#pragma unroll
+    for (int p = 0; p < P; ++p) xs2_patch[p * PATCH + o] = make_uint4(0u, 0u, 0u, 0u);
+  }
+
+  int aoy[MI], aox[MI];
+#pragma unroll
+  for (int i = 0; i < MI; ++i) {
+    const int m = wm * TM + i * 32 + fr;
+    aoy[i] = GE::row_oy(m);
+    aox[i] = GE::row_ox(m);
+  }
+  auto afrag = [&](int ki, int kj, int cb, int kk, uint4 (&af)[P][MI]) __attribute__((always_inline)) {
+#pragma unroll
+    for (int i = 0; i < MI; ++i) {
+      const int o = GE::frag_unit(aoy[i], aox[i], ki, kj, cb * 4 + kk * 2 + hf);
+#pragma unroll
+      for (int p = 0; p < P; ++p) af[p][i] = xs2_patch[p * PATCH + o];
+    }
+  };
+
+  int g_cur = -1, slot = 0;
+  HScale hs;
+  [[maybe_unused]] HScale hs2;
+
+  while (T < total) {
+    const Tile tl = tile_at(T);
+    const int g = tl.g;
+    if (g != g_cur) {
+      g_cur = g;
+      slot = a.wsel ? a.wsel[g] : g;
+      const int ma = amax_read(a.amax_src, a.amax_src_ld, g);
+      hs.init(ma, amax_read(a.amax_w, a.amax_w_ld, slot));
+      if constexpr (SC) hs2.init(ma, amax_read(a.sc_amax_w, a.sc_amax_w_ld, slot));
+    }
+
+    if constexpr (SC || KS) {
+#pragma unroll
+      for (int i = 0; i < MI; ++i) asm volatile("" : "+v"(aoy[i]), "+v"(aox[i]));
+    }
+    const __amdgpu_buffer_rsrc_t rF = rsrc(a.wf + (long long)slot * a.wf_sstride, (long long)BN * 9 * CIN * 4);
+    const int wbase = wn * NK * 4096 + lane * 16;
+    uint4 wb[RING][4];
+    auto gw = [&](auto TT, int s, int f) __attribute__((always_inline)) {
+      constexpr int t = decltype(TT)::value;
+      if constexpr (t < NK) {
+        constexpr int plane = (t % CB) * 9 + t / CB;
+        wb[s][f] = __builtin_bit_cast(uint4, bload4(rF, wbase + plane * 4096 + f * 1024));
+      }
+    };
+    sfor<RING - 1>([&](auto TT) __attribute__((always_inline)) {
+#pragma unroll
+      for (int f = 0; f < 4; ++f) gw(TT, decltype(TT)::value, f);
+    });
+
+#pragma unroll
+    for (int u = 0; u < NE; ++u) {
+      uint2 sp[P];
+      split4h(pv[u].x, pv[u].y, pv[u].z, pv[u].w, hs.ma, sp);
+      const int o = GE::fill_half(tid, u);
+#pragma unroll
+      for (int p = 0; p < P; ++p) ((uint2*)&xs2_patch[p * PATCH])[o] = sp[p];
+    }
+    __syncthreads();
+    const int Tn = next_valid(T + gridDim.x);
+    if (Tn < total) pload(tile_at(Tn));
+
+    f32x16_t acc[MI][1];
+#pragma unroll
+    for (int i = 0; i < MI; ++i)
+#pragma unroll
+      for (int r = 0; r < 16; ++r) acc[i][0][r] = 0.f;
+    [[maybe_unused]] f32x16_t ssum[KS ? MI : 1][1];
+    [[maybe_unused]] int zs = 1, kb_next = KS ? (int)((long long)NK / a.kslab) : 0;
+
+    sfor<NK>([&](auto TT) __attribute__((always_inline)) {
+      constexpr int t = decltype(TT)::value, tap = t / CB, cb = t % CB, ki = tap / 3, kj = tap - ki * 3;
+      constexpr int s = t % RING, s2 = (t + RING - 1) % RING;
+      __builtin_amdgcn_sched_barrier(0x786);
+      sfor<2>([&](auto KK) __attribute__((always_inline)) {
+        constexpr int kk = decltype(KK)::value;
+        uint4 af[P][MI], bfr[P][1];
+        afrag(ki, kj, cb, kk, af);
+#pragma unroll
+        for (int p = 0; p < P; ++p) bfr[p][0] = wb[s][kk * 2 + p];
+        mma_half<MI, 1, P, true, 4, kk>(af, bfr, acc, [&](int q) __attribute__((always_inline)) {
+          gw(std::integral_constant<int, t + RING - 1>{}, s2, q);
+        });
+      });
+      if constexpr (KS) {
+        if (t + 1 == kb_next) {
+          hs.finish(acc);
+#pragma unroll
+          for (int i = 0; i < MI; ++i)
+#pragma unroll
+            for (int r = 0; r < 16; ++r) {
+              ssum[i][0][r] = zs == 1 ? acc[i][0][r] : ssum[i][0][r] + acc[i][0][r];
+              acc[i][0][r] = 0.f;
+            }
+          ++zs;
+          kb_next = (int)((long long)NK * zs / a.kslab);
+        }
+      }
+    });
+    if constexpr (KS) {
+#pragma unroll
+      for (int i = 0; i < MI; ++i) acc[i][0] = ssum[i][0];
+    } else {
+      hs.finish(acc);
+    }
+
+    [[maybe_unused]] uint4 sw[SC ? CB : 1][4];
+    if constexpr (SC) {
+      const __amdgpu_buffer_rsrc_t rS =
+          rsrc(a.sc_wf + (long long)slot * a.sc_wf_sstride, (long long)BN * CIN * 4);
+      const int sbase = wn * CB * 4096 + lane * 16;
+#pragma unroll
+      for (int cb = 0; cb < CB; ++cb)
+#pragma unroll
+        for (int f = 0; f < 4; ++f) sw[cb][f] = __builtin_bit_cast(uint4, bload4(rS, sbase + cb * 4096 + f * 1024));
+    }
+
+    const long long row0 = (long long)tl.img * WO * WO + tl.oy0 * WO;
+    auto epilogue = [&](float* outp, long long gstride, const float* biasp, long long bstride, bool relu, int* amax,
+                        int amax_ld, int amax_bm) __attribute__((always_inline)) {
+      float* out = outp + (long long)g * gstride;
+      const float* bias = biasp ? biasp + (long long)slot * bstride : nullptr;
+      const int n = wn * 32 + fr;
+      const float bv = bias ? bias[n] : 0.f;
+      float vmax[MI];
+#pragma unroll
+      for (int i = 0; i < MI; ++i) {
+        vmax[i] = 0.f;
+#pragma unroll
+        for (int r = 0; r < 16; ++r) {
+          const int m = wm * TM + i * 32 + (r & 3) + 8 * (r >> 2) + 4 * hf;
+          float v = acc[i][0][r];
+          if (bias) v += bv;
+          if (relu) v = fmaxf(v, 0.f);
+          vmax[i] = fmaxf(vmax[i], fabsf(v));
+          out[(row0 + m) * BN + n] = v;
+        }
+      }
+      if (!amax) return;
+      __syncthreads();
+#pragma unroll
+      for (int i = 0; i < MI; ++i) {
+        const float x = wave_max(vmax[i]);
+        if (lane == 0) xs2_red[wid * MI + i] = x;
+      }
+      __syncthreads();
+      if (tid == 0) {
+        long long cur = -1;
+        float b = 0.f;
+        for (int q = 0; q <= BM / 32; ++q) {
+          const long long tile = q < BM / 32 ? (row0 + q * 32) / amax_bm : -2;
+          if (tile != cur) {
+            if (cur >= 0 && b > 0.f) atomicMax(amax + (int)(cur % kAmaxSub) * amax_ld + g, __float_as_int(b));
+            cur = tile;
+            b = 0.f;
+          }
+          if (q < BM / 32) {
+            const int qm = (q * 32) / TM, qi = (q * 32 - qm * TM) / 32;
+            for (int c = 0; c < WN; ++c) b = fmaxf(b, xs2_red[(qm * WN + c) * MI + qi]);
+          }
+        }
+      }
+    };
+    epilogue(a.out, a.out_gstride, a.bias, a.b_sstride, a.relu != 0, a.amax_out, a.amax_out_ld, a.amax_bm);
+
+    if constexpr (SC) {
+#pragma unroll
+      for (int i = 0; i < MI; ++i)
+#pragma unroll
+        for (int r = 0; r < 16; ++r) acc[i][0][r] = 0.f;
+      sfor<CB>([&](auto C) __attribute__((always_inline)) {
+        constexpr int cb = decltype(C)::value;
+        sfor<2>([&](auto KK) __attribute__((always_inline)) {
+          constexpr int kk = decltype(KK)::value;
+          uint4 af[P][MI], bfr[P][1];
+          afrag(1, 1, cb, kk, af);
+#pragma unroll
+          for (int p = 0; p < P; ++p) bfr[p][0] = sw[cb][kk * 2 + p];
+          mma_half<MI, 1, P, true, 0, kk>(af, bfr, acc, [](int) {});
+        });
+      });
+      hs2.finish(acc);
+      epilogue(a.sc_out, a.sc_out_gstride, a.sc_bias, a.sc_b_sstride, false, a.sc_amax_out, a.sc_amax_out_ld,
+               a.sc_amax_bm);
+    }
+    __syncthreads();
+    T = Tn;
+  }
+}
+
+constexpr int kRingA = 3, kRingB = 3;
+
+template <class GE, int BN, int RING, bool SC, bool KS>
+int xs2_go(const XS2Args& a, int G, hipStream_t st) {
+  static unsigned long long attr_set = 0ull;
+  int dev = 0;
+  if (hipGetDevice(&dev) != hipSuccess || dev < 0 || dev >= 64) return -100;
+  if (!(attr_set >> dev & 1ull)) {
+    if (hipFuncSetAttribute((const void*)xs2_kernel<GE, BN, RING, SC, KS>, hipFuncAttributeMaxDynamicSharedMemorySize,
+                            GE::LDS_BYTES) != hipSuccess)
+      return -100;
+    attr_set |= 1ull << dev;
+  }
+  static int cus[64] = {0};
+  if (cus[dev] <= 0 && (hipDeviceGetAttribute(&cus[dev], hipDeviceAttributeMultiprocessorCount, dev) != hipSuccess ||
+                        cus[dev] <= 0))
+    return -100;
+  XS2Args b = a;
+  b.G = G;
+  const long long tiles = (long long)G * a.N * GE::HT;
+  if (tiles >= (1LL << 30)) return -100;
+  const dim3 grid((unsigned)std::min<long long>(tiles, 2LL * cus[dev]), 1, 1);
+  hipLaunchKernelGGL((xs2_kernel<GE, BN, RING, SC, KS>), grid, dim3(256), GE::LDS_BYTES, st, b);
+  DBA_LAUNCH_CHECK();
+}
+
+}
+
+int xg::xs2_launch(const XS2Args& a, int form, int G, hipStream_t st) {
+  const bool sc = a.sc_out != nullptr, ks = a.kslab > 1;
+  if (a.kslab < 1 || a.kslab > 9 || a.amax_bm < 32 || a.amax_bm % 32 || (sc && (a.sc_amax_bm < 32 || a.sc_amax_bm % 32)))
+    return -100;
+  if (form == 0) {
+    if (sc || ks) return -100;
+    return xs2_go<XS2GeomA, 64, kRingA, false, false>(a, G, st);
+  }
+  if (form == 1) {
+    if (sc) return ks ? -100 : xs2_go<XS2GeomB, 128, kRingB, true, false>(a, G, st);
+    return ks ? xs2_go<XS2GeomB, 128, kRingB, false, true>(a, G, st) : xs2_go<XS2GeomB, 128, kRingB, false, false>(a, G, st);
+  }
+  return -100;
+}
diff --git a/csrc/kernels/xconv_s2.hpp b/csrc/kernels/xconv_s2.hpp
--- /dev/null
+++ b/csrc/kernels/xconv_s2.hpp
@@ -0,0 +1,33 @@
+#pragma once
+#include <hip/hip_runtime.h>
+#include <stdint.h>
+
+namespace xg {
+
+struct XS2Args {
+  const float* src; long long src_gstride;
+  const int* wsel;
+  const int* nvalid;
+  int N, G;
+  const int* amax_src; int amax_src_ld;
+  const uint16_t* wf; long long wf_sstride;
+  const int* amax_w; int amax_w_ld;
+  const float* bias; long long b_sstride;
+  float* out; long long out_gstride;
+  int* amax_out; int amax_out_ld;
+  int relu;
+  int kslab;
+  int amax_bm;
+  const uint16_t* sc_wf; long long sc_wf_sstride;
+  const int* sc_amax_w; int sc_amax_w_ld;
+  const float* sc_bias; long long sc_b_sstride;
+  float* sc_out; long long sc_out_gstride;
+  int* sc_amax_out; int sc_amax_out_ld;
+  int sc_amax_bm;
+};
+
+int xs2_launch(const XS2Args& a, int form, int G, hipStream_t st);
+int& xs2_mode();
+bool xs2_default(int form, bool entry);
+
+}
diff --git a/csrc/kernels/xs2_geom.hpp b/csrc/kernels/xs2_geom.hpp
--- /dev/null
+++ b/csrc/kernels/xs2_geom.hpp
@@ -0,0 +1,45 @@
+#pragma once
+
+#if defined(__HIPCC__)
+#define XS2_HD __host__ __device__ __forceinline__
+#else
+#define XS2_HD inline
+#endif
+
+template <int WIN_, int CIN_, int TR_, int PITCH_>
+struct XS2Geom {
+  static constexpr int WIN = WIN_, CIN = CIN_, TR = TR_, PITCH = PITCH_;
+  static constexpr int WO = WIN / 2, BM = TR * WO, HT = WO / TR;
+  static constexpr int PR = 2 * TR + 1, PC = WIN + 1;
+  static constexpr int EV = WIN / 2 + 1;
+  static constexpr int CH = CIN / 8, Q4 = CIN / 4, CB = CIN / 32;
+  static constexpr int PATCH = PR * PITCH * CH;
+  static constexpr int LDS_BYTES = 2 * PATCH * 16;
+  static_assert(WIN % 2 == 0 && WO % TR == 0 && BM % 32 == 0 && CIN % 32 == 0 && PITCH >= PC, "tile");
+  static_assert((CH == 4 && PITCH % 4 == 2) || (CH == 8 && PITCH % 2 == 1), "pitch / swizzle pairing");
+
+  static constexpr XS2_HD int pcol(int pc) { return (pc & 1) ? EV + (pc >> 1) : (pc >> 1); }
+  static constexpr XS2_HD int skew(int pr) { return CH == 4 ? 2 * (pr & 1) : 4 * pr + (pr & 1); }
+  static constexpr XS2_HD int key(int pr, int pcl) {
+    return CH == 4 ? ((pcl + skew(pr)) >> 2) & 3 : ((pcl + skew(pr)) >> 1) & 7;
+  }
+  static constexpr XS2_HD int unit(int pr, int pcl, int u) { return (pr * PITCH + pcl) * CH + (u ^ key(pr, pcl)); }
+  static constexpr XS2_HD int frag_unit(int oyl, int ox, int ki, int kj, int u) {
+    return unit(2 * oyl + ki, ox + pcol(kj), u);
+  }
+  static constexpr int FILL_THREADS = 256;
+  static_assert(WIN * Q4 == FILL_THREADS, "one fill piece per thread per patch row");
+  static constexpr XS2_HD int fill_pc(int tid) { return tid / Q4 + 1; }
+  static constexpr XS2_HD int fill_q(int tid) { return tid % Q4; }
+  static constexpr XS2_HD int fill_half(int tid, int pr) {
+    return unit(pr, pcol(fill_pc(tid)), fill_q(tid) >> 1) * 2 + (fill_q(tid) & 1);
+  }
+  static constexpr int ZUNITS = PR * CH;
+  static_assert(ZUNITS <= FILL_THREADS, "one zero unit per thread");
+  static constexpr XS2_HD int zero_unit(int z) { return unit(z / CH, 0, z % CH); }
+  static constexpr XS2_HD int row_oy(int m) { return m / WO; }
+  static constexpr XS2_HD int row_ox(int m) { return m % WO; }
+};
+
+using XS2GeomA = XS2Geom<32, 32, 8, 34>;
+using XS2GeomB = XS2Geom<16, 64, 8, 17>;
diff --git a/dba_mod_amd/models/program.py b/dba_mod_amd/models/program.py
--- a/dba_mod_amd/models/program.py
+++ b/dba_mod_amd/models/program.py
@@ -166,6 +166,15 @@
         r = ops.conv2d(x, wsc, self.wsel, 2, 0, bias=bsc, nvalid=self.nvalid)
         return ops.conv2d(a, w2, self.wsel, 1, 1, bias=b2, residual=r, relu=True, nvalid=self.nvalid)
 
+    def down_entry(self, x: Tensor, pre: str, sc: str) -> Optional[Tensor]:
+        w1, b1 = self.folded[pre + "conv1.weight"]
+        wsc, bsc = self.folded[sc + ".0.weight"]
+        if not ops.down_entry_ok(x, w1, wsc):
+            return None
+        w2, b2 = self.folded[pre + "conv2.weight"]
+        a, r = ops.down_entry_eval(x, w1, b1, wsc, bsc, self.wsel, self.nvalid)
+        return ops.conv2d(a, w2, self.wsel, 1, 1, bias=b2, residual=r, relu=True, nvalid=self.nvalid)
+
     def stem_block(self, x: Tensor, stem: str, pre: str) -> Optional[Tensor]:
         w0, b0 = self.folded[stem]
         w1, b1 = self.folded[pre + "conv1.weight"]
@@ -370,6 +379,11 @@
                 a = ctx.bn_conv(a, pre + "conv2.weight", pre + "bn2", stride, 1, relu=True)
                 last, p = "3", 0
             else:
+                if not ctx.train and stride == 2 and cin != w:
+                    y = ctx.down_entry(out, pre, pre + "shortcut")
+                    if y is not None:
+                        out, cin = y, w
+                        continue
                 a = ctx.bn_conv(out, pre + "conv1.weight", pre + "bn1", stride, 1, relu=True)
                 last, p = "2", 1
                 if not ctx.train and stride == 2 and cin != w:
@@ -400,6 +414,10 @@
             stride = 2 if (li > 0 and bi == 0) else 1
             pre = f"layer{li + 1}.{bi}."
             if not ctx.train and stride == 2 and cin != w:
+                y = ctx.down_entry(out, pre, pre + "downsample")
+                if y is not None:
+                    out, cin = y, w
+                    continue
                 a = ctx.bn_conv(out, pre + "conv1.weight", pre + "bn1", stride, 1, relu=True)
                 out, cin = ctx.down_block(a, out, pre, pre + "downsample"), w
                 continue
diff --git a/dba_mod_amd/ops/__init__.py b/dba_mod_amd/ops/__init__.py
--- a/dba_mod_amd/ops/__init__.py
+++ b/dba_mod_amd/ops/__init__.py
@@ -45,7 +45,7 @@
         "clipped_delta_sum", "pairwise_sq_dists", "trimmed_delta_sum", "delta_sum_votes",
         "vote_agreement", "rlr_apply", "gram", "prepare_dgrad_weights", "wgrad_flush",
         "wgrad_prepare", "conv_bn_stats", "bn_apply", "bn_finish", "basic_block_ok", "basic_block_eval",
-        "stem_block_ok", "stem_block_eval", "down_block_ok", "down_block_eval"]
+        "stem_block_ok", "stem_block_eval", "down_block_ok", "down_block_eval", "down_entry_ok", "down_entry_eval"]
 
 for _n in _OPS:
     globals()[_n] = _dispatch(_n)
diff --git a/dba_mod_amd/ops/branches.py b/dba_mod_amd/ops/branches.py
--- a/dba_mod_amd/ops/branches.py
+++ b/dba_mod_amd/ops/branches.py
@@ -58,7 +58,8 @@
             return False
         return {"conv2d": conv2d, "maxpool2d": maxpool2d, "conv_bn_stats": conv_bn_stats, "bn_apply": bn_apply,
                 "basic_block_ok": basic_block_ok, "stem_block_ok": lambda x, w0, w1, w2: False,
-                "down_block_ok": lambda a, w2, x2, wsc: False}
+                "down_block_ok": lambda a, w2, x2, wsc: False,
+                "down_entry_ok": lambda x, w1, wsc: False}
 
     def _valid(self, t):
         v = torch.zeros(t.shape[:2], dtype=torch.bool)
diff --git a/dba_mod_amd/ops/build.py b/dba_mod_amd/ops/build.py
--- a/dba_mod_amd/ops/build.py
+++ b/dba_mod_amd/ops/build.py
@@ -58,7 +58,8 @@
     return out
 
 
-_EXTRA = {n: ["-fno-slp-vectorize"] for n in ("xconv_fwd.hip", "xconv_dgrad.hip", "xwgrad.hip", "xaux.hip", "xbn.hip")}
+_EXTRA = {n: ["-fno-slp-vectorize"] for n in ("xconv_fwd.hip", "xconv_dgrad.hip", "xwgrad.hip", "xaux.hip", "xbn.hip",
+                                                "xconv_s2.hip")}
 _THIS_MTIME = os.path.getmtime(os.path.abspath(__file__))
 
 
diff --git a/dba_mod_amd/ops/hip.py b/dba_mod_amd/ops/hip.py
--- a/dba_mod_amd/ops/hip.py
+++ b/dba_mod_amd/ops/hip.py
@@ -93,6 +93,9 @@
     "dba_bnx_dy": [_P, _P, _P, _P, _LL, _P, _I, _I, _I, _I, _P, _I, _P],
     "dba_xwgrad_reduce_batch": [_P, _I, _I, _LL, _P],
     "dba_xstage_set": [_I],
+    "dba_xs2_set": [_I],
+    "dba_xs2_entry_fwd": [_P, _LL, _P, _P] + [_I] * 5 + [_P, _I] + [_P, _LL, _P, _I, _P, _LL, _P, _LL, _P, _I] * 2
+    + [_P],
     "dba_xblock_fwd": [_P, _LL, _P, _LL, _P, _P, _P, _LL, _P, _P, _LL, _P, _P, _LL, _P] + [_I] * 6
     + [_P, _I, _P, _P, _I, _P, _I, _P],
     "dba_xblock_stem_fwd": [_P, _LL, _P, _LL, _P, _P, _LL, _P, _LL, _P, _P, _LL, _P, _P, _LL, _P, _P, _LL, _P]
@@ -257,6 +260,10 @@
     return int(_L.dba_xstage_set(int(on)))
 
 
+def set_xs2(mode: int) -> int:
+    return int(_L.dba_xs2_set(int(mode)))
+
+
 def set_wgrad_halo(on: int) -> int:
     return int(_L.dba_xwgrad_halo_set(int(on)))
 
@@ -401,11 +408,12 @@
     desc, outs = [], []
     for w in ws:
         p = getattr(w, "_dba_planes", None)
-        if (p is None or w.dim() != 5 or tuple(w.shape[2:4]) != (3, 3) or w.shape[1] % 32 or w.shape[4] % 32
+        if (p is None or w.dim() != 5 or tuple(w.shape[2:4]) not in ((3, 3), (1, 1)) or w.shape[1] % 32 or w.shape[4] % 32
+                or (w.shape[2] == 1 and w.shape[4] < 64)
                 or not p.is_contiguous() or p.shape[2] != w[0].numel()):
             continue
         out = torch.empty(p.shape[0], 2 * p.shape[2], dtype=torch.int16, device=p.device)
-        desc.append([p.data_ptr(), out.data_ptr(), w.shape[1], w.shape[4], 0])
+        desc.append([p.data_ptr(), out.data_ptr(), w.shape[1], w.shape[4], w.shape[2] * w.shape[3], 0])
         outs.append((w, out))
     if not desc:
         return
@@ -611,6 +619,52 @@
 _EVAL_DOWN = os.environ.get("DBA_EVAL_DOWN", "1") != "0"
 
 
+def down_entry_ok(x, w1, wsc) -> bool:
+    if not (x.dtype == _F32 and x.dim() == 5 and w1.dim() == 5 and wsc.dim() == 5):
+        return False
+    if any(getattr(t, k, None) is None for t in (w1, wsc) for k in ("_dba_planes", "_dba_fplanes")):
+        return False
+    H, W, C = x.shape[2:]
+    Co = w1.shape[1]
+    if tuple(w1.shape[1:]) != (Co, 3, 3, C) or tuple(wsc.shape[1:]) != (Co, 1, 1, C) or w1.shape[0] != wsc.shape[0]:
+        return False
+    return (H, W, C, Co) == (16, 16, 64, 128)
+
+
+def down_entry_eval(x, w1, b1, wsc, bsc, wsel=None, nvalid=None):
+    x = _act(x, _F32, "conv input")
+    G, N, H, W, Cin = x.shape
+    Cout, Ho, Wo = w1.shape[1], H // 2, W // 2
+
+    def two():
+        return (conv2d(x, w1, wsel, 2, 1, bias=b1, relu=True, nvalid=nvalid),
+                conv2d(x, wsc, wsel, 2, 0, bias=bsc, nvalid=nvalid))
+
+    ar = _ARENA[-1] if _ARENA else None
+    if ar is not None and int(_L.dba_xconv_ws_floats(G, N, Ho, Wo, Cin, Cout, 3, 3)) > 0:
+        ncnt = int(_L.dba_xconv_sk_ints(G, N, Ho, Wo, Cin, Cout, 3, 3))
+        if ncnt > 0 and x.device == ar.cnt.device and ar.cnt_next + ncnt <= ar.cnt.numel():
+            return two()
+    (_, ws1), (_, wss) = _check_w(w1), _check_w(wsc)
+    aw1, awsc = _amax_w(w1, ws1, Cout * 9 * Cin), _amax_w(wsc, wss, Cout * Cin)
+    (b1c, bs1), (bscc, bss) = _rowview(b1), _rowview(bsc)
+    f1, fsc = w1._dba_fplanes, wsc._dba_fplanes
+    ax = _amax_act(x, nvalid)
+    a = torch.empty(G, N, Ho, Wo, Cout, dtype=_F32, device=x.device)
+    sc = torch.empty_like(a)
+    mark = (ar.next if ar is not None else 0)
+    aa, asc = _amax_out(a), _amax_out(sc)
+    rc = _call("dba_xs2_entry_fwd", x.data_ptr(), x.stride(0), _ptr(_i32(wsel)), _ptr(_i32(nvalid)), G, N, W, Cin,
+               Cout, *_aptr(ax), f1.data_ptr(), f1.stride(0), *_aptr(aw1), b1c.data_ptr(), bs1, a.data_ptr(),
+               a.stride(0), *_aptr(aa), fsc.data_ptr(), fsc.stride(0), *_aptr(awsc), bscc.data_ptr(), bss,
+               sc.data_ptr(), sc.stride(0), *_aptr(asc), _stream())
+    if rc == NOT_HANDLED:
+        if ar is not None and ar.next == mark + 2:
+            ar.next = mark
+        return two()
+    return a, sc
+
+
 def conv2d(x, w, wsel, stride, pad, bias=None, residual=None, relu=False, nvalid=None, out_dtype=None,
            bn_stats=False):
     return _xconv_fwd(_act(x, _F32, "conv input"), w, wsel, stride, pad, bias, residual, relu, nvalid, out_dtype)
diff --git a/dba_mod_amd/ops/reference.py b/dba_mod_amd/ops/reference.py
--- a/dba_mod_amd/ops/reference.py
+++ b/dba_mod_amd/ops/reference.py
@@ -138,6 +138,16 @@
                     wsel: Optional[Tensor] = None, nvalid: Optional[Tensor] = None) -> Tensor:
     sc = conv2d(x2, wsc, wsel, 2, 0, bias=bsc, nvalid=nvalid)
     return conv2d(a, w2, wsel, 1, 1, bias=b2, residual=sc, relu=True, nvalid=nvalid)
+
+
+def down_entry_ok(x: Tensor, w1: Tensor, wsc: Tensor) -> bool:
+    return False
+
+
+def down_entry_eval(x: Tensor, w1: Tensor, b1: Tensor, wsc: Tensor, bsc: Tensor, wsel: Optional[Tensor] = None,
+                    nvalid: Optional[Tensor] = None) -> Tuple[Tensor, Tensor]:
+    return (conv2d(x, w1, wsel, 2, 1, bias=b1, relu=True, nvalid=nvalid),
+            conv2d(x, wsc, wsel, 2, 0, bias=bsc, nvalid=nvalid))
 
 
 def _valid_mask(t: Tensor, nvalid: Optional[Tensor]) -> Tensor:
```

Result: no change. 3.892 (median of 3 runs) (+1.0%).
